# hjanime/recoup

Hardware: NVIDIA B200
Metric: reads/s through coverage + profileMatrix (reads -> per-base coverage -> regions x bins) (higher is better)
Workload: dtype int32 coverage / f64 matrix

## Files before the change

include/recoup_b200.h:

```cpp
#ifndef RECOUP_B200_H
#define RECOUP_B200_H

#include <stdint.h>

#ifdef __cplusplus
extern "C" {
#endif

#define RCP_ABI_VERSION 1

enum {
    RCP_OK = 0,
    RCP_ERR_CUDA = 1,
    RCP_ERR_ARG = 2,
    RCP_ERR_HANDLE = 3,
    RCP_ERR_NOGPU = 4,
    RCP_ERR_UNSUPPORTED = 5,
    RCP_ERR_DATA = 6
};

#define RCP_MEM_HOST 0
#define RCP_MEM_DEVICE 1

#define RCP_STRAND_ANY 2
// ... 35 lines not shown
#define RCP_PATH_BUCKETS 2
#define RCP_PATH_BLOCKS 3
#define RCP_PATH_SPLIT 4
int rcp_set_coverage_path(int path);
int rcp_coverage_path_info(int cov, int* path, int64_t* candidates);

int rcp_set_deferred_validation(int on);

int rcp_r_sample(int n, int k, int seed, int sample_kind, int* out );
int rcp_r_rank_table(int n, int seed, int sample_kind, int* rank_out );

int rcp_reads_load(int64_t n, const int32_t* chrom, const int32_t* start, const int32_t* end,
                   const int8_t* strand, int n_chrom, const int64_t* chrom_len, int frag_len,
                   int mem, int* reads_out);
int rcp_reads_load_rle(int64_t n, int64_t n_runs, const int32_t* run_chrom, const int32_t* run_len,
                       const int32_t* start, const int32_t* end, const int8_t* strand, int n_chrom,
                       const int64_t* chrom_len, int frag_len, int mem, int* reads_out);
int rcp_reads_load_width(int64_t n, const int32_t* chrom, int64_t n_runs, const int32_t* run_chrom,
                         const int32_t* run_len, const int32_t* start, int width, const int8_t* strand,
                         int n_chrom, const int64_t* chrom_len, int frag_len, int mem, int* reads_out);
int rcp_reads_width_quantile(int64_t n, const int32_t* start, const int32_t* end, double prob, int mem,
                             double* quantile_out , int64_t* n_le_out );
int rcp_r_sample_sorted(int seed, int sample_kind, int n_calls, const int64_t* n, const int64_t* k,
                        int32_t* out );
int rcp_reads_load_select(int64_t n, const int32_t* chrom, const int32_t* start, const int32_t* end,
                          const int8_t* strand, double max_width, int64_t k, const int32_t* idx,
                          int n_chrom, const int64_t* chrom_len, int frag_len, int mem,
                          int64_t* n_kept_out, int* reads_out);
int rcp_bgzf_size(const uint8_t* data , int64_t n_bytes, int64_t* inflated_bytes, int64_t* n_blocks);
int rcp_bgzf_inflate(const uint8_t* data , int64_t n_bytes, uint8_t* out , int64_t capacity,
                     int n_threads);
int rcp_bam_index(const uint8_t* rec , int64_t n_bytes, int64_t* n_records_out,
                  int64_t* offsets_out , int64_t capacity);
int rcp_bam_decode(const uint8_t* rec, int64_t n_bytes, const int64_t* offsets, int64_t n_records,
                   int n_ref, const int64_t* ref_len , int splice_split, int mem,
                   int* decoded_out, int64_t* n_out);
int rcp_bam_decode_param(const uint8_t* rec, int64_t n_bytes, const int64_t* offsets, int64_t n_records,
                         int n_ref, const int64_t* ref_len , int splice_split, int mem,
                         const int32_t* flag , int mapq_min , int simple_cigar,
                         int n_which, const int32_t* which_ref, const int32_t* which_start,
                         const int32_t* which_end, int n_tags, const char* tag_names, const int32_t* tag_ptr,
                         const int32_t* tag_type , const int64_t* int_values,
                         const char* const* str_values, int* decoded_out, int64_t* n_out);
int rcp_bed_decode(const char* text, int64_t n_bytes, int n_names, const char* const* names ,
                   int mem, int* decoded_out, int64_t* n_out);
int rcp_decoded_fetch(int decoded, int32_t* chrom, int32_t* start, int32_t* end, int8_t* strand,
                      int64_t capacity);
int rcp_decoded_free(int decoded);
int rcp_reads_load_decoded(int decoded, int n_chrom, const int64_t* chrom_len, int frag_len,
                           int* reads_out);
int rcp_decoded_width_quantile(int decoded, double prob, double* quantile_out, int64_t* n_le_out);
int rcp_reads_load_decoded_select(int decoded, double max_width, int64_t k, const int32_t* idx ,
                                  int n_chrom, const int64_t* chrom_len, int frag_len,
                                  int64_t* n_kept_out, int* reads_out);
int rcp_reads_info(int reads, int64_t* n, int* n_chrom, int64_t* device_bytes);
int rcp_reads_free(int reads);

int rcp_coverage(int reads, int64_t n_regions, const int32_t* chrom, const int32_t* start,
                 const int32_t* end, const int8_t* strand, int ignore_strand, int strand_filter,
                 int mem, int* cov_out);
int rcp_coverage_list(int reads, int64_t n_elements, const int64_t* ptr, const int32_t* chrom,
                      const int32_t* start, const int32_t* end, const int8_t* strand,
                      int ignore_strand, int strand_filter, int mem, int* cov_out);
int rcp_coverage_concat3(int left, int center, int right, int* cov_out);
int rcp_coverage_set_scale(int cov, double factor);
int rcp_coverage_info(int cov, int64_t* n_regions, int64_t* total_len, int64_t* n_null,
                      double* scale);
int rcp_coverage_lengths(int cov, int32_t* len_out );
int rcp_coverage_fetch(int cov, int64_t first, int64_t count, int32_t* out, int64_t capacity);
int rcp_coverage_rle(int cov, int64_t first, int64_t count, int64_t* run_ptr_out,
                     int32_t* values_out, int32_t* lengths_out, int64_t capacity);
int rcp_coverage_free(int cov);

#define RCP_VALUE_INT32 0
#define RCP_VALUE_FLOAT32 1
int rcp_bigwig_load(const uint8_t* data , int64_t n_bytes, int n_threads, int* signal_out);
int rcp_signal_info(int signal, int* n_chrom, int64_t* n_items, int64_t* names_bytes);
int rcp_signal_chroms(int signal, char* names , int64_t* chrom_len);
int rcp_signal_fetch(int signal, int32_t* chrom, int32_t* start, int32_t* end, float* value, int64_t capacity);
int rcp_signal_free(int signal);
int rcp_signal_coverage(int signal, int64_t n_elements, const int64_t* ptr, const int32_t* chrom,
                        const int32_t* start, const int32_t* end, const int8_t* strand, int mem, int* cov_out);
int rcp_coverage_value_type(int cov, int* type);
int rcp_coverage_fetch_f32(int cov, int64_t first, int64_t count, float* out, int64_t capacity);
int rcp_coverage_rle_f32(int cov, int64_t first, int64_t count, int64_t* run_ptr_out,
                         float* values_out, int32_t* lengths_out, int64_t capacity);

int rcp_bin_matrix(int cov, int where, int f1, int f2, int n_bins, int stat, int interp,
                   int seed, int sample_kind, double* out, int64_t ld, int mem);
int rcp_base_matrix(int cov, int where, int f1, int f2, int64_t n_cols, double* out, int64_t ld,
                    int mem);
int rcp_profile_ncols(int cov, int equal_lengths, int f1, int f2, int flank_bin_size,
                      int region_bin_size, int64_t* ncols_out);
int rcp_profile_matrix(int cov, int equal_lengths, int f1, int f2, int flank_bin_size,
                       int region_bin_size, int stat, int interp, int seed, int sample_kind,
                       double* out, int64_t ld, int mem);

int rcp_coverage_profile(int reads, int64_t n_regions, const int32_t* chrom,
                         const int32_t* start, const int32_t* end, const int8_t* strand,
                         int ignore_strand, int strand_filter, int n_bins, int seed,
                         int sample_kind, double scale, double* out, int64_t ld,
                         uint8_t* is_null_out, int mem);

int rcp_sort_keys_u32(uint32_t* keys, int64_t n, int key_bits, int mem);

#define RCP_ROW_SUM 0
#define RCP_ROW_MAX 1
#define RCP_ROW_MEAN 2
int rcp_matrix_col_profile(const double* m, int64_t n_rows, int64_t n_cols, int64_t ld, int stat,
                           int log2_scale, int mem, double* center ,
                           double* spread );
int rcp_matrix_row_stat(const double* m, int64_t n_rows, int64_t n_cols, int64_t ld, int what, int mem,
                        double* out );
int rcp_order(const double* v, int64_t n, int decreasing, int mem, int32_t* ix , int64_t* n_out);
int rcp_matrix_quantile(const double* m, int64_t n_rows, int64_t n_cols, int64_t ld, const double* probs,
                        int k, int mem, double* out );

int rcp_rows_scatter(const double* src, int64_t ld_src, int64_t n_rows, int64_t n_cols,
                     const int64_t* row_index, double* dst, int64_t ld_dst);

int rcp_rows_put(const double* src, int64_t ld_src, int64_t n_rows, int64_t n_cols, double* dst,
                 int64_t ld_dst, void* stream);

int rcp_reads_route_count(int64_t n, const int32_t* chrom, const int32_t* start, const int32_t* end, int world,
                          int n_chrom, const int32_t* spans, int64_t* counts_out );
int rcp_reads_route_pack(int64_t n, const int32_t* chrom, const int32_t* start, const int32_t* end,
                         const int8_t* strand, int world, int n_chrom, const int32_t* spans,
                         const int64_t* offsets , int32_t* chrom_out, int32_t* start_out,
                         int32_t* end_out, int8_t* strand_out);

#define RCP_IPC_HANDLE_BYTES 64
int rcp_shared_alloc(int64_t bytes, void** ptr_out, unsigned char* handle_out );
int rcp_shared_open(const unsigned char* handle , void** ptr_out);
int rcp_shared_close(void* ptr);
int rcp_shared_free(void* ptr);

#ifdef __cplusplus
}
#endif
#endif
```

recoup_b200/_lib.py:

```python
import ctypes as C
import os

_HERE = os.path.dirname(os.path.abspath(__file__))
LIB_PATH = os.environ.get("RCP_LIB_PATH") or os.path.join(_HERE, "librecoup_b200.so")

RCP_OK, RCP_ERR_CUDA, RCP_ERR_ARG, RCP_ERR_HANDLE, RCP_ERR_NOGPU, RCP_ERR_UNSUPPORTED, RCP_ERR_DATA = range(7)
MEM_HOST, MEM_DEVICE = 0, 1
STRAND_ANY = 2
WHERE = {"whole": 0, "center": 1, "upstream": 2, "downstream": 3}
STAT = {"mean": 0, "median": 1}
INTERP = {"auto": 0, "spline": 1, "linear": 2, "neighborhood": 3}
SAMPLE_KIND = {"Rejection": 0, "Rounding": 1}
COVERAGE_PATH = {"auto": 0, "index": 1, "buckets": 2, "blocks": 3, "split": 4}
VALUE_INT32, VALUE_FLOAT32 = 0, 1

_i32p = C.POINTER(C.c_int32)
_i64p = C.POINTER(C.c_int64)
_i8p = C.POINTER(C.c_int8)
_u8p = C.POINTER(C.c_uint8)
_f64p = C.POINTER(C.c_double)
_ip = C.POINTER(C.c_int)
_vp = C.c_void_p

SIGNATURES = {
    "rcp_last_error": (C.c_char_p, []),
    "rcp_abi_version": (C.c_int, []),
    "rcp_init": (C.c_int, [C.c_int]),
    "rcp_shutdown": (C.c_int, []),
    "rcp_device_info": (C.c_int, [_ip, _ip, _ip, _ip, _i64p]),
    "rcp_stream": (C.c_void_p, []),
    "rcp_sync": (C.c_int, []),
    "rcp_launch_count": (C.c_int64, [C.c_int]),
    "rcp_set_coverage_path": (C.c_int, [C.c_int]),
    "rcp_set_deferred_validation": (C.c_int, [C.c_int]),
    "rcp_host_alloc": (C.c_int, [C.c_int64, C.POINTER(C.c_void_p)]),
    "rcp_host_free": (C.c_int, [C.c_void_p]),
    "rcp_timing_enable": (C.c_int, [C.c_int]),
    "rcp_timing_read": (C.c_int, [C.c_int, C.c_int, _f64p, _i64p]),
    "rcp_timing_stage_name": (C.c_char_p, [C.c_int]),
    "rcp_r_sample": (C.c_int, [C.c_int, C.c_int, C.c_int, C.c_int, _ip]),
    "rcp_r_rank_table": (C.c_int, [C.c_int, C.c_int, C.c_int, _ip]),
    "rcp_reads_load": (C.c_int, [C.c_int64, _vp, _vp, _vp, _vp, C.c_int, _i64p, C.c_int, C.c_int, _ip]),
    "rcp_matrix_col_profile": (C.c_int, [_vp, C.c_int64, C.c_int64, C.c_int64, C.c_int, C.c_int, C.c_int,
                                         _vp, _vp]),
    "rcp_matrix_row_stat": (C.c_int, [_vp, C.c_int64, C.c_int64, C.c_int64, C.c_int, C.c_int, _vp]),
    "rcp_order": (C.c_int, [_vp, C.c_int64, C.c_int, C.c_int, _vp, _i64p]),
    "rcp_matrix_quantile": (C.c_int, [_vp, C.c_int64, C.c_int64, C.c_int64, _vp, C.c_int, C.c_int, _vp]),
    "rcp_reads_width_quantile": (C.c_int, [C.c_int64, _vp, _vp, C.c_double, C.c_int, _f64p, _i64p]),
    "rcp_r_sample_sorted": (C.c_int, [C.c_int, C.c_int, C.c_int, _i64p, _i64p, _vp]),
    "rcp_reads_load_select": (C.c_int, [C.c_int64, _vp, _vp, _vp, _vp, C.c_double, C.c_int64, _vp, C.c_int,
                                        _i64p, C.c_int, C.c_int, _i64p, _ip]),
    "rcp_coverage_path_info": (C.c_int, [C.c_int, _ip, _i64p]),
    "rcp_rows_put": (C.c_int, [_vp, C.c_int64, C.c_int64, C.c_int64, _vp, C.c_int64, _vp]),
    "rcp_reads_route_count": (C.c_int, [C.c_int64, _vp, _vp, _vp, C.c_int, C.c_int, _i32p, _i64p]),
    "rcp_reads_route_pack": (C.c_int, [C.c_int64, _vp, _vp, _vp, _vp, C.c_int, C.c_int, _i32p, _i64p, _vp, _vp, _vp,
                                       _vp]),
    "rcp_reads_load_width": (C.c_int, [C.c_int64, _vp, C.c_int64, _vp, _vp, _vp, C.c_int, _vp, C.c_int, _i64p,
                                       C.c_int, C.c_int, _ip]),
    "rcp_reads_load_rle": (C.c_int, [C.c_int64, C.c_int64, _vp, _vp, _vp, _vp, _vp, C.c_int, _i64p,
                                     C.c_int, C.c_int, _ip]),
    "rcp_bgzf_size": (C.c_int, [_vp, C.c_int64, _i64p, _i64p]),
    "rcp_bgzf_inflate": (C.c_int, [_vp, C.c_int64, _vp, C.c_int64, C.c_int]),
    "rcp_bam_index": (C.c_int, [_vp, C.c_int64, _i64p, _vp, C.c_int64]),
    "rcp_bam_decode": (C.c_int, [_vp, C.c_int64, _vp, C.c_int64, C.c_int, _i64p, C.c_int, C.c_int, _ip, _i64p]),
    "rcp_bam_decode_param": (C.c_int, [_vp, C.c_int64, _vp, C.c_int64, C.c_int, _i64p, C.c_int, C.c_int, _i32p,
                                       C.c_int, C.c_int, C.c_int, _i32p, _i32p, _i32p, C.c_int, C.c_char_p, _i32p,
                                       _i32p, _i64p, C.POINTER(C.c_char_p), _ip, _i64p]),
    "rcp_bed_decode": (C.c_int, [_vp, C.c_int64, C.c_int, C.POINTER(C.c_char_p), C.c_int, _ip, _i64p]),
    "rcp_decoded_fetch": (C.c_int, [C.c_int, _vp, _vp, _vp, _vp, C.c_int64]),
    "rcp_decoded_free": (C.c_int, [C.c_int]),
    "rcp_reads_load_decoded": (C.c_int, [C.c_int, C.c_int, _i64p, C.c_int, _ip]),
    "rcp_decoded_width_quantile": (C.c_int, [C.c_int, C.c_double, _f64p, _i64p]),
    "rcp_reads_load_decoded_select": (C.c_int, [C.c_int, C.c_double, C.c_int64, _vp, C.c_int, _i64p, C.c_int,
                                                _i64p, _ip]),
    "rcp_reads_info": (C.c_int, [C.c_int, _i64p, _ip, _i64p]),
    "rcp_reads_free": (C.c_int, [C.c_int]),
    "rcp_coverage": (C.c_int, [C.c_int, C.c_int64, _vp, _vp, _vp, _vp, C.c_int, C.c_int, C.c_int, _ip]),
    "rcp_coverage_list": (C.c_int, [C.c_int, C.c_int64, _i64p, _vp, _vp, _vp, _vp, C.c_int, C.c_int,
                                    C.c_int, _ip]),
    "rcp_coverage_concat3": (C.c_int, [C.c_int, C.c_int, C.c_int, _ip]),
    "rcp_coverage_set_scale": (C.c_int, [C.c_int, C.c_double]),
    "rcp_coverage_info": (C.c_int, [C.c_int, _i64p, _i64p, _i64p, _f64p]),
    "rcp_coverage_lengths": (C.c_int, [C.c_int, _i32p]),
    "rcp_coverage_fetch": (C.c_int, [C.c_int, C.c_int64, C.c_int64, _i32p, C.c_int64]),
    "rcp_coverage_rle": (C.c_int, [C.c_int, C.c_int64, C.c_int64, _i64p, _i32p, _i32p, C.c_int64]),
    "rcp_coverage_free": (C.c_int, [C.c_int]),
    "rcp_bigwig_load": (C.c_int, [_vp, C.c_int64, C.c_int, _ip]),
    "rcp_signal_info": (C.c_int, [C.c_int, _ip, _i64p, _i64p]),
    "rcp_signal_chroms": (C.c_int, [C.c_int, C.c_char_p, _i64p]),
    "rcp_signal_fetch": (C.c_int, [C.c_int, _vp, _vp, _vp, _vp, C.c_int64]),
    "rcp_signal_free": (C.c_int, [C.c_int]),
    "rcp_signal_coverage": (C.c_int, [C.c_int, C.c_int64, _i64p, _vp, _vp, _vp, _vp, C.c_int, _ip]),
    "rcp_coverage_value_type": (C.c_int, [C.c_int, _ip]),
    "rcp_coverage_fetch_f32": (C.c_int, [C.c_int, C.c_int64, C.c_int64, _vp, C.c_int64]),
    "rcp_coverage_rle_f32": (C.c_int, [C.c_int, C.c_int64, C.c_int64, _i64p, _vp, _i32p, C.c_int64]),
    "rcp_bin_matrix": (C.c_int, [C.c_int, C.c_int, C.c_int, C.c_int, C.c_int, C.c_int, C.c_int, C.c_int,
                                 C.c_int, _vp, C.c_int64, C.c_int]),
    "rcp_base_matrix": (C.c_int, [C.c_int, C.c_int, C.c_int, C.c_int, C.c_int64, _vp, C.c_int64, C.c_int]),
    "rcp_profile_ncols": (C.c_int, [C.c_int, C.c_int, C.c_int, C.c_int, C.c_int, C.c_int, _i64p]),
    "rcp_profile_matrix": (C.c_int, [C.c_int, C.c_int, C.c_int, C.c_int, C.c_int, C.c_int, C.c_int,
                                     C.c_int, C.c_int, C.c_int, _vp, C.c_int64, C.c_int]),
    "rcp_coverage_profile": (C.c_int, [C.c_int, C.c_int64, _vp, _vp, _vp, _vp, C.c_int, C.c_int, C.c_int,
                                       C.c_int, C.c_int, C.c_double, _vp, C.c_int64, _vp, C.c_int]),
    "rcp_sort_keys_u32": (C.c_int, [_vp, C.c_int64, C.c_int, C.c_int]),
    "rcp_shared_alloc": (C.c_int, [C.c_int64, C.POINTER(C.c_void_p), C.POINTER(C.c_ubyte)]),
    "rcp_shared_open": (C.c_int, [C.POINTER(C.c_ubyte), C.POINTER(C.c_void_p)]),
    "rcp_shared_close": (C.c_int, [C.c_void_p]),
    "rcp_shared_free": (C.c_int, [C.c_void_p]),
    "rcp_rows_scatter": (C.c_int, [_vp, C.c_int64, C.c_int64, C.c_int64, _vp, _vp, C.c_int64]),
}


class RecoupError(RuntimeError):
    def __init__(self, code, message):
        super().__init__("librecoup_b200 error %d: %s" % (code, message))
        self.code = code


def _load():
    if not os.path.exists(LIB_PATH):
        raise ImportError(
            "%s is missing: build it with `python -c 'import __graft_entry__ as g; g.build()'` "
            "(nvcc, sm_100a). recoup_b200 has no CPU fallback." % LIB_PATH)
    lib = C.CDLL(LIB_PATH)
    for name, (res, args) in SIGNATURES.items():
        fn = getattr(lib, name)
        fn.restype = res
        fn.argtypes = args
    return lib


lib = _load()
_initialised_device = None


def check(rc):
    if rc != RCP_OK:
        raise RecoupError(rc, lib.rcp_last_error().decode("utf-8", "replace"))


def init(device=None):
    global _initialised_device
    if device is None:
        device = int(os.environ.get("LOCAL_RANK", "0"))
    if _initialised_device == device:
        return
    check(lib.rcp_init(int(device)))
    _initialised_device = device


def shutdown():
    global _initialised_device
    lib.rcp_shutdown()
    _initialised_device = None


def set_coverage_path(path):
    ensure_init()
    check(lib.rcp_set_coverage_path(COVERAGE_PATH[path]))


def ensure_init():
    if _initialised_device is None:
        init()
```

recoup_b200/csrc/api.cu:

```cuda
#include <climits>
#include <algorithm>
#include <cstdarg>
#include <cstdio>
#include <cstdlib>
#include <cstring>
#include <map>
#include <memory>

#include "r_rng.cuh"
#include "rcp_internal.cuh"

namespace rcp {

Ctx g_ctx;
static thread_local std::string g_error;
static std::map<int, std::unique_ptr<ReadsIdx>> g_reads;
static std::map<int, std::unique_ptr<Coverage>> g_covs;
static int g_next_handle = 1;

int fail(int code, const char* fmt, ...) {
    char buf[1024];
    va_list ap;
    va_start(ap, fmt);
    vsnprintf(buf, sizeof(buf), fmt, ap);
// ... 912 lines not shown
    Coverage *a = get_coverage(left), *b = get_coverage(center), *c = get_coverage(right);
    if (!a || !b || !c) return fail(RCP_ERR_HANDLE, "unknown coverage handle");
    if (cov_out == nullptr) return fail(RCP_ERR_ARG, "cov_out is NULL");
    if (a->value_type != b->value_type || b->value_type != c->value_type)
        return fail(RCP_ERR_ARG, "concat3: the three coverages have different value types");
    Coverage* cv;
    int h;
    RCP_TRY(new_coverage(&cv, &h));
    cv->value_type = b->value_type;
    int rc = coverage_concat3(*a, *b, *c, cv);
    if (rc != RCP_OK) {
        drop_coverage(h);
        return rc;
    }
    cv->scale = b->scale;
    *cov_out = h;
    return RCP_OK;
}

int rcp_coverage_set_scale(int cov, double factor) {
    Coverage* cv = get_coverage(cov);
    if (!cv) return fail(RCP_ERR_HANDLE, "unknown coverage handle %d", cov);
    cv->scale = factor;
    return RCP_OK;
}

int rcp_coverage_info(int cov, int64_t* n_regions, int64_t* total_len, int64_t* n_null,
                      double* scale) {
    Coverage* cv = get_coverage(cov);
    if (!cv) return fail(RCP_ERR_HANDLE, "unknown coverage handle %d", cov);
    if (total_len || n_null) RCP_TRY(coverage_resolve_stats(*cv));
    if (n_regions) *n_regions = cv->n_regions;
    if (total_len) *total_len = cv->total_len;
    if (n_null) *n_null = cv->n_null;
    if (scale) *scale = cv->scale;
    return RCP_OK;
}

int rcp_coverage_path_info(int cov, int* path, int64_t* candidates) {
    Coverage* cv = get_coverage(cov);
    if (!cv) return fail(RCP_ERR_HANDLE, "unknown coverage handle %d", cov);
    if (candidates) RCP_TRY(coverage_resolve_stats(*cv));
    if (path) *path = cv->path;
    if (candidates) *candidates = cv->candidates;
    return RCP_OK;
}

int rcp_coverage_lengths(int cov, int32_t* len_out) {
    RCP_TRY(require_ready());
    Coverage* cv = get_coverage(cov);
    if (!cv) return fail(RCP_ERR_HANDLE, "unknown coverage handle %d", cov);
    if (cv->n_regions == 0) return RCP_OK;
    if (!len_out) return fail(RCP_ERR_ARG, "len_out is NULL");
    RCP_CUDA(cudaMemcpyAsync(len_out, cv->len, (size_t)cv->n_regions * 4, cudaMemcpyDeviceToHost,
                             g_ctx.stream));
    RCP_CUDA(cudaStreamSynchronize(g_ctx.stream));
    return RCP_OK;
}

int rcp_coverage_fetch(int cov, int64_t first, int64_t count, int32_t* out, int64_t capacity) {
    RCP_TRY(require_ready());
    Coverage* cv = get_coverage(cov);
    if (!cv) return fail(RCP_ERR_HANDLE, "unknown coverage handle %d", cov);
    if (cv->value_type != RCP_VALUE_INT32) return fail(RCP_ERR_ARG, "rcp_coverage_fetch: a FLOAT32 coverage (use _f32)");
    return coverage_fetch(*cv, first, count, out, capacity);
}

int rcp_coverage_fetch_f32(int cov, int64_t first, int64_t count, float* out, int64_t capacity) {
    RCP_TRY(require_ready());
    Coverage* cv = get_coverage(cov);
    if (!cv) return fail(RCP_ERR_HANDLE, "unknown coverage handle %d", cov);
    if (cv->value_type != RCP_VALUE_FLOAT32) return fail(RCP_ERR_ARG, "rcp_coverage_fetch_f32: an INT32 coverage");
    return coverage_fetch(*cv, first, count, reinterpret_cast<int32_t*>(out), capacity);
}

int rcp_coverage_value_type(int cov, int* type) {
    Coverage* cv = get_coverage(cov);
    if (!cv) return fail(RCP_ERR_HANDLE, "unknown coverage handle %d", cov);
    if (type == nullptr) return fail(RCP_ERR_ARG, "type is NULL");
    *type = cv->value_type;
    return RCP_OK;
}

int rcp_coverage_rle(int cov, int64_t first, int64_t count, int64_t* run_ptr_out,
                     int32_t* values_out, int32_t* lengths_out, int64_t capacity) {
    RCP_TRY(require_ready());
    Coverage* cv = get_coverage(cov);
    if (!cv) return fail(RCP_ERR_HANDLE, "unknown coverage handle %d", cov);
    if (cv->value_type != RCP_VALUE_INT32) return fail(RCP_ERR_ARG, "rcp_coverage_rle: a FLOAT32 coverage (use _f32)");
    return coverage_rle(*cv, first, count, run_ptr_out, values_out, lengths_out, capacity);
}

int rcp_coverage_rle_f32(int cov, int64_t first, int64_t count, int64_t* run_ptr_out, float* values_out,
                         int32_t* lengths_out, int64_t capacity) {
    RCP_TRY(require_ready());
    Coverage* cv = get_coverage(cov);
    if (!cv) return fail(RCP_ERR_HANDLE, "unknown coverage handle %d", cov);
    if (cv->value_type != RCP_VALUE_FLOAT32) return fail(RCP_ERR_ARG, "rcp_coverage_rle_f32: an INT32 coverage");
    return coverage_rle(*cv, first, count, run_ptr_out, reinterpret_cast<int32_t*>(values_out), lengths_out,
                        capacity);
}

int rcp_coverage_free(int cov) {
    if (!get_coverage(cov)) return fail(RCP_ERR_HANDLE, "unknown coverage handle %d", cov);
    drop_coverage(cov);
    return RCP_OK;
}

int rcp_bin_matrix(int cov, int where, int f1, int f2, int n_bins, int stat, int interp, int seed,
                   int sample_kind, double* out, int64_t ld, int mem) {
    RCP_TRY(require_ready());
    Coverage* cv = get_coverage(cov);
    if (!cv) return fail(RCP_ERR_HANDLE, "unknown coverage handle %d", cov);
    RCP_TRY(check_bins(n_bins, stat, interp));
    if (where < RCP_WHERE_WHOLE || where > RCP_WHERE_DOWNSTREAM) return fail(RCP_ERR_ARG, "bad where");
    if (f1 < 0 || f2 < 0) return fail(RCP_ERR_ARG, "negative flank");
    if (ld < cv->n_regions || out == nullptr) return fail(RCP_ERR_ARG, "bad output matrix");
    MatrixOut m;
    RCP_TRY(m.init(out, ld, cv->n_regions, n_bins, mem));
    RCP_TRY(bin_matrix_device(*cv, where, f1, f2, n_bins, stat, interp, seed, sample_kind, m.dev,
                              m.ld_dev));
    return m.finish(out, ld, cv->n_regions, n_bins);
}

int rcp_base_matrix(int cov, int where, int f1, int f2, int64_t n_cols, double* out, int64_t ld,
                    int mem) {
    RCP_TRY(require_ready());
    Coverage* cv = get_coverage(cov);
    if (!cv) return fail(RCP_ERR_HANDLE, "unknown coverage handle %d", cov);
    if (where < RCP_WHERE_WHOLE || where > RCP_WHERE_DOWNSTREAM || where == RCP_WHERE_CENTER)
        return fail(RCP_ERR_ARG, "baseCoverageMatrix takes where = whole / upstream / downstream");
    if (f1 < 0 || f2 < 0 || n_cols < 0) return fail(RCP_ERR_ARG, "negative size");
    if (where == RCP_WHERE_UPSTREAM && n_cols != f1) return fail(RCP_ERR_ARG, "n_cols must equal flank[1]");
    if (where == RCP_WHERE_DOWNSTREAM && n_cols != f2) return fail(RCP_ERR_ARG, "n_cols must equal flank[2]");
    if (ld < cv->n_regions || out == nullptr) return fail(RCP_ERR_ARG, "bad output matrix");
    MatrixOut m;
    RCP_TRY(m.init(out, ld, cv->n_regions, n_cols, mem));
    RCP_TRY(base_matrix_device(*cv, where, f1, f2, n_cols, m.dev, m.ld_dev));
    return m.finish(out, ld, cv->n_regions, n_cols);
}

int rcp_profile_ncols(int cov, int equal_lengths, int f1, int f2, int flank_bin_size,
                      int region_bin_size, int64_t* ncols_out) {
    RCP_TRY(require_ready());
    Coverage* cv = get_coverage(cov);
    if (!cv) return fail(RCP_ERR_HANDLE, "unknown coverage handle %d", cov);
    int64_t common = 0;
    if (equal_lengths && region_bin_size == 0) RCP_TRY(common_length(*cv, &common));
    Blocks b;
    RCP_TRY(profile_blocks(*cv, equal_lengths, f1, f2, flank_bin_size, region_bin_size, common, &b));
    *ncols_out = b.left + b.center + b.right;
    return RCP_OK;
}

int rcp_profile_matrix(int cov, int equal_lengths, int f1, int f2, int flank_bin_size,
                       int region_bin_size, int stat, int interp, int seed, int sample_kind,
                       double* out, int64_t ld, int mem) {
    RCP_TRY(require_ready());
    Coverage* cv = get_coverage(cov);
    if (!cv) return fail(RCP_ERR_HANDLE, "unknown coverage handle %d", cov);
    if (ld < cv->n_regions || out == nullptr) return fail(RCP_ERR_ARG, "bad output matrix");
    int64_t common = 0;
    if (equal_lengths && region_bin_size == 0) RCP_TRY(common_length(*cv, &common));
    Blocks b;
    RCP_TRY(profile_blocks(*cv, equal_lengths, f1, f2, flank_bin_size, region_bin_size, common, &b));
    const int64_t ncols = b.left + b.center + b.right;
// ... 260 lines not shown
```

recoup_b200/csrc/coverage.cu:

```cuda
#include "cov_common.cuh"
#include "rcp_internal.cuh"

namespace rcp {

using namespace covk;

namespace {

template <int NS>
struct Sources {
    const uint32_t* xs[NS];
    const uint32_t* ye[NS];
    uint32_t n[NS];
    uint32_t yshift[NS];
    uint8_t cls_bit[NS];
    uint8_t corr[NS];
};

struct RegionArrays {
    uint32_t* gs;
    int32_t* len;
    uint8_t* flags;
    uint8_t* is_null;
    uint32_t* ix0;
// ... 381 lines not shown
                int32_t* __restrict__ cov) {
    __shared__ __align__(16) int diff[TILE];
    __shared__ int rowpre[MAX_ROWS + 1];
    const int tid = threadIdx.x;
    const int64_t g = tile_region[blockIdx.x];
    const int j = (int)((int64_t)blockIdx.x - tile_off[g]);
    const int L = la.len[g];
    const int m = (L + TILE - 1) / TILE;
    const int tile_len = (((L + m - 1) / m) + ROW - 1) / ROW * ROW;
    const int o_lo = j * tile_len;
    const int tlen = min(tile_len, L - o_lo);
    const bool rev = (la.flags[g] & 1u) != 0;
    const int t0 = rev ? (L - o_lo - tlen) : o_lo;
    const int t1 = t0 + tlen - 1;
    const int nrows = (tlen + ROW - 1) / ROW;
    for (int i = tid; i < nrows * (ROW / 4); i += CTA)
        reinterpret_cast<int4*>(diff)[i] = make_int4(0, 0, 0, 0);
    __syncthreads();
    const int64_t a = ptr[g], b = ptr[g + 1];
    const uint32_t clo = la.clo[g], chi = la.chi[g], span_lo = la.span_lo[g];
    for (uint32_t i = clo + tid; i < chi; i += CTA) {
        const uint32_t rs = __ldg(xs + i), re1 = __ldg(p_end1 + i);
        if (re1 <= span_lo) continue;
        const int rst = p_strand ? (int)__ldg(p_strand + i) : 0;
        if (strand_filter != RCP_STRAND_ANY && rst != strand_filter) continue;
        int mult = 0;
        for (int64_t q = a; q < b; q++) {
            const uint32_t s = __ldg(la.xgs + q), e = __ldg(la.xge + q);
            if (e + 1u == s) continue;
            if (rs <= e && re1 > s &&
                strand_ok(rst, strand ? (int)__ldg(strand + q) : 0, ignore_strand, strand_filter))
                mult++;
        }
        if (mult == 0) continue;
        for (int64_t q = a; q < b; q++) {
            const uint32_t s = __ldg(la.xgs + q), e = __ldg(la.xge + q);
            if (e + 1u == s) continue;
            if (!(rs <= e && re1 > s)) continue;
            const int xo = __ldg(la.xoff + q);
            const int pa = xo + (int)(max(rs, s) - s);
            const int pb = xo + (int)(min(re1 - 1u, e) - s);
            if (pb < t0 || pa > t1) continue;
            const int ka = max(pa, t0) - t0, kb1 = pb + 1 - t0;
            if (!rev) {
                atomicAdd(diff + ka, mult);
                if (kb1 < tlen) atomicSub(diff + kb1, mult);
            } else {
                atomicAdd(diff + (tlen - 1 - ka), mult);
                if (kb1 < tlen) atomicSub(diff + (tlen - 1 - kb1), mult);
            }
        }
    }
    __syncthreads();
    block_scan_store(diff, tlen, 0, rev, rowpre, cov + off[g] + o_lo);
}

__global__ void __launch_bounds__(CTA)
concat_plan_kernel(int64_t R, const uint8_t* __restrict__ n0, const uint8_t* __restrict__ n1,
                   const uint8_t* __restrict__ n2, const int32_t* __restrict__ l0,
                   const int32_t* __restrict__ l1, const int32_t* __restrict__ l2,
                   int32_t* __restrict__ len, uint8_t* __restrict__ is_null,
                   int64_t* __restrict__ padded, unsigned long long* __restrict__ stats) {
    const int64_t r = (int64_t)blockIdx.x * CTA + threadIdx.x;
    if (r >= R) return;
    const bool null = n0[r] || n1[r] || n2[r];
    const int64_t L = null ? 0 : (int64_t)l0[r] + l1[r] + l2[r];
    len[r] = (int32_t)L;
    is_null[r] = null ? 1 : 0;
    padded[r] = (L + PAD - 1) / PAD * PAD;
    if (null) {
        atomicAdd(&stats[0], 1ull);
    } else {
        atomicAdd(&stats[1], (unsigned long long)L);
        atomicMax(&stats[2], (unsigned long long)L);
    }
}

__global__ void __launch_bounds__(CTA)
concat_copy_kernel(const int32_t* __restrict__ c0, const int64_t* __restrict__ o0,
                   const int32_t* __restrict__ l0, const int32_t* __restrict__ c1,
                   const int64_t* __restrict__ o1, const int32_t* __restrict__ l1,
                   const int32_t* __restrict__ c2, const int64_t* __restrict__ o2,
                   const int32_t* __restrict__ l2, const int32_t* __restrict__ len,
                   const int64_t* __restrict__ off, int32_t* __restrict__ cov) {
    const int64_t r = blockIdx.x;
    if (len[r] == 0) return;
    int32_t* dst = cov + off[r];
    const int a = l0[r], b = l1[r], c = l2[r];
    for (int i = threadIdx.x; i < a; i += CTA) dst[i] = c0[o0[r] + i];
    for (int i = threadIdx.x; i < b; i += CTA) dst[a + i] = c1[o1[r] + i];
    for (int i = threadIdx.x; i < c; i += CTA) dst[a + b + i] = c2[o2[r] + i];
}

__global__ void __launch_bounds__(CTA)
pack_kernel(const int32_t* __restrict__ cov, const int64_t* __restrict__ off,
            const int32_t* __restrict__ len, const int64_t* __restrict__ packed_off,
            int64_t first, int32_t* __restrict__ out) {
    const int64_t r = first + blockIdx.x;
    const int L = len[r];
    const int32_t* src = cov + off[r];
    int32_t* dst = out + packed_off[blockIdx.x];
    for (int i = threadIdx.x; i < L; i += CTA) dst[i] = src[i];
}

__global__ void __launch_bounds__(CTA)
len_to_i64_kernel(int64_t n, const int32_t* __restrict__ len, int64_t* __restrict__ out) {
    const int64_t i = (int64_t)blockIdx.x * CTA + threadIdx.x;
    if (i < n) out[i] = len[i];
}


__global__ void __launch_bounds__(CTA)
rle_count_kernel(const int32_t* __restrict__ cov, const int64_t* __restrict__ off,
                 const int32_t* __restrict__ len, int64_t first, int64_t* __restrict__ n_runs) {
    __shared__ int wsum[WARPS];
    const int64_t r = first + blockIdx.x;
    const int L = len[r];
    const int32_t* x = cov + off[r];
    int c = 0;
    for (int i = threadIdx.x; i < L; i += CTA) c += (i == 0) || (x[i] != x[i - 1]);
    for (int d = 16; d > 0; d >>= 1) c += __shfl_xor_sync(0xffffffffu, c, d);
    if ((threadIdx.x & 31) == 0) wsum[threadIdx.x >> 5] = c;
    __syncthreads();
    if (threadIdx.x == 0) {
        int t = 0;
        for (int w = 0; w < WARPS; w++) t += wsum[w];
        n_runs[blockIdx.x] = t;
    }
}

__global__ void __launch_bounds__(CTA)
rle_write_kernel(const int32_t* __restrict__ cov, const int64_t* __restrict__ off,
                 const int32_t* __restrict__ len, int64_t first,
                 const int64_t* __restrict__ run_ptr, int32_t* __restrict__ values,
                 int32_t* __restrict__ starts) {
    __shared__ int wsum[WARPS];
    __shared__ int carry_s;
    const int64_t r = first + blockIdx.x;
    const int L = len[r];
    const int32_t* x = cov + off[r];
    const int64_t base = run_ptr[blockIdx.x];
    const int lane = threadIdx.x & 31, warp = threadIdx.x >> 5;
    if (threadIdx.x == 0) carry_s = 0;
    __syncthreads();
    for (int i0 = 0; i0 < L; i0 += CTA) {
        const int i = i0 + threadIdx.x;
        int v = 0;
        bool head = false;
        if (i < L) {
            v = x[i];
            head = (i == 0) || (v != x[i - 1]);
        }
        const unsigned bal = __ballot_sync(0xffffffffu, head);
        if (lane == 0) wsum[warp] = __popc(bal);
        __syncthreads();
        int pre = carry_s;
        for (int w = 0; w < warp; w++) pre += wsum[w];
        if (head) {
            const int64_t o = base + pre + __popc(bal & ((1u << lane) - 1u));
            values[o] = v;
            starts[o] = i;
        }
        __syncthreads();
        if (threadIdx.x == CTA - 1) carry_s = pre + __popc(bal);
        __syncthreads();
    }
}

__global__ void __launch_bounds__(CTA)
rle_lengths_kernel(const int32_t* __restrict__ len, int64_t first,
                   const int64_t* __restrict__ run_ptr, const int32_t* __restrict__ starts,
                   int32_t* __restrict__ lengths) {
    const int64_t r = first + blockIdx.x;
    const int L = len[r];
    const int64_t a = run_ptr[blockIdx.x], b = run_ptr[blockIdx.x + 1];
    for (int64_t j = a + threadIdx.x; j < b; j += CTA)
        lengths[j] = (j + 1 < b ? starts[j + 1] : L) - starts[j];
}

int alloc_coverage_arrays(Coverage* cv, int64_t R) {
    cv->n_regions = R;
    RCP_TRY(dalloc(&cv->off, (size_t)R + 1));
    RCP_TRY(dalloc(&cv->len, (size_t)R));
    RCP_TRY(dalloc(&cv->is_null, (size_t)R));
    return RCP_OK;
}

template <int NS>
int coverage_ranges_impl(ReadsIdx& rd, Sources<NS> src, int64_t R, const int32_t* chrom,
                         const int32_t* start, const int32_t* end, const int8_t* strand,
                         int ignore_strand, int strand_filter, Coverage* cv) {
    RCP_TRY(alloc_coverage_arrays(cv, R));
    RegionArrays ra;
    RCP_TRY(dalloc(&ra.gs, (size_t)R));
    ra.len = cv->len;
    RCP_TRY(dalloc(&ra.flags, (size_t)R));
    ra.is_null = cv->is_null;
    RCP_TRY(dalloc(&ra.ix0, (size_t)R * NS));
    RCP_TRY(dalloc(&ra.ix1, (size_t)R * NS));
    RCP_TRY(dalloc(&ra.iy0, (size_t)R * NS));
    RCP_TRY(dalloc(&ra.iy1, (size_t)R * NS));
    RCP_TRY(dalloc(&ra.padded, (size_t)R));
    RCP_TRY(dalloc(&ra.ntiles, (size_t)R));
    int64_t* tile_off = nullptr;
    RCP_TRY(dalloc(&tile_off, (size_t)R + 1));
    unsigned int* d_err = nullptr;
    unsigned long long* d_stats = nullptr;
    RCP_TRY(dalloc(&d_err, 1));
    RCP_TRY(dalloc(&d_stats, 3));
    RCP_CUDA(cudaMemsetAsync(d_err, 0, sizeof(unsigned int), g_ctx.stream));
    RCP_CUDA(cudaMemsetAsync(d_stats, 0, 3 * sizeof(unsigned long long), g_ctx.stream));

    struct Host {
        int64_t total_padded, total_tiles;
        unsigned long long stats[3];
        unsigned int err;
    } h = {0, 0, {0, 0, 0}, 0};
    {
        StageTimer t(ST_COV_PLAN);
        if (R > 0) {
            region_plan_kernel<NS><<<blocks_for(R, CTA), CTA, 0, g_ctx.stream>>>(
                R, chrom, start, end, strand, rd.d_chrom_off, rd.d_chrom_len, rd.n_chrom, src,
                ignore_strand, strand_filter, ra, d_err, d_stats);
            RCP_LAUNCHED();
        }
        RCP_TRY(exclusive_scan2_i64(ra.padded, cv->off, cv->off + R, ra.ntiles, tile_off,
                                    tile_off + R, R));
    }
    {
        const FetchItem items[4] = {{cv->off + R, &h.total_padded, 8}, {tile_off + R, &h.total_tiles, 8},
                                    {d_stats, h.stats, 24}, {d_err, &h.err, 4}};
        RCP_TRY(fetch_and_sync(items, 4));
    }
    int rc = RCP_OK;
    if (h.err & 1u) rc = fail(RCP_ERR_DATA, "a region has a chromosome id outside [0, n_chrom)");
    else if (h.err & 2u) rc = fail(RCP_ERR_DATA, "a region has end < start - 1");
    if (rc == RCP_OK) {
        cv->path = RCP_PATH_INDEX;
        cv->total_padded = h.total_padded;
        cv->n_null = (int64_t)h.stats[0];
        cv->total_len = (int64_t)h.stats[1];
        cv->max_len = (int32_t)h.stats[2];
        rc = dalloc(&cv->cov, (size_t)h.total_padded);
    }
    int32_t* tile_region = nullptr;
    if (rc == RCP_OK && h.total_tiles > 0) {
        rc = dalloc(&tile_region, (size_t)h.total_tiles);
        if (rc == RCP_OK) {
            {
                StageTimer t(ST_COV_PLAN);
                fill_tiles_kernel<<<blocks_for(R, CTA), CTA, 0, g_ctx.stream>>>(R, ra.ntiles,
                                                                                tile_off, tile_region);
                g_ctx.launches++;
            }
            StageTimer t(ST_COV_TILE);
            cov_tile_kernel<NS><<<(unsigned)h.total_tiles, CTA, 0, g_ctx.stream>>>(
                tile_region, tile_off, ra, src, cv->off, cv->cov);
            g_ctx.launches++;
        }
    }
    if (rc == RCP_OK && R > 0) {
        StageTimer t(ST_COV_SMALL);
        cov_small_kernel<NS><<<blocks_for(R, WARPS), CTA, 0, g_ctx.stream>>>(R, ra, src, cv->off,
                                                                             cv->cov);
        g_ctx.launches++;
    }
    if (rc == RCP_OK && cudaGetLastError() != cudaSuccess)
        rc = fail(RCP_ERR_CUDA, "coverage kernel launch failed");
    dfree(tile_region);
    dfree(ra.gs);
    dfree(ra.flags);
    dfree(ra.ix0);
    dfree(ra.ix1);
    dfree(ra.iy0);
    dfree(ra.iy1);
    dfree(ra.padded);
    dfree(ra.ntiles);
    dfree(tile_off);
    dfree(d_err);
    dfree(d_stats);
    return rc;
}

}

void coverage_release(Coverage& c) {
    dfree(c.cov);
    dfree(c.off);
    dfree(c.len);
    dfree(c.is_null);
    dfree(c.d_stats);
    c.stats_pending = false;
}

namespace {
__global__ void __launch_bounds__(CTA)
na_rule_kernel(int64_t R, const int32_t* __restrict__ chrom, const int8_t* __restrict__ strand,
               const uint8_t* __restrict__ len_na, int n_chrom, const int64_t* __restrict__ off,
               int32_t* __restrict__ len, uint8_t* __restrict__ is_null, const int32_t* __restrict__ cov,
               const int64_t* __restrict__ end_pos) {
    const int64_t r = (int64_t)blockIdx.x * CTA + threadIdx.x;
    if (r >= R) return;
    const int32_t L = len[r];
    const int c = chrom[r];
    if (L <= 0 || c < 0 || c >= n_chrom || !len_na[c]) return;
    const int64_t idx = end_pos ? end_pos[r] : ((strand && strand[r] < 0) ? 0 : (int64_t)L - 1);
    if (idx < 0 || idx >= L || cov[off[r] + idx] == 0) {
        len[r] = 0;
        is_null[r] = 1;
    }
}

__global__ void __launch_bounds__(CTA)
len_stats_kernel(int64_t R, const int32_t* __restrict__ len, unsigned long long* __restrict__ stats) {
    const int64_t r = (int64_t)blockIdx.x * CTA + threadIdx.x;
    unsigned long long my_null = 0, my_len = 0;
    if (r < R) {
        my_len = (unsigned long long)len[r];
        my_null = my_len == 0 ? 1 : 0;
    }
    unsigned long long my_max = my_len;
    for (int d = 16; d > 0; d >>= 1) {
        my_null += __shfl_xor_sync(0xffffffffu, my_null, d);
        my_len += __shfl_xor_sync(0xffffffffu, my_len, d);
        my_max = max(my_max, __shfl_xor_sync(0xffffffffu, my_max, d));
    }
    if ((threadIdx.x & 31) == 0) {
        if (my_null) atomicAdd(&stats[0], my_null);
        if (my_len) atomicAdd(&stats[1], my_len);
        if (my_max) atomicMax(&stats[2], my_max);
    }
}
}

int coverage_na_rule(const ReadsIdx& rd, Coverage& cv, int64_t R, const int32_t* d_chrom, const int8_t* d_strand,
                     const int64_t* d_end_pos) {
    if (!rd.any_na || R <= 0) return RCP_OK;
    RCP_TRY(coverage_resolve_stats(cv));
    if (!cv.d_stats) RCP_TRY(dalloc(&cv.d_stats, 4));
    const unsigned long long h[4] = {0ull, 0ull, 0ull, (unsigned long long)cv.candidates};
    RCP_CUDA(cudaMemcpyAsync(cv.d_stats, h, 32, cudaMemcpyHostToDevice, g_ctx.stream));
    na_rule_kernel<<<blocks_for(R, CTA), CTA, 0, g_ctx.stream>>>(R, d_chrom, d_strand, rd.d_len_na, rd.n_chrom, cv.off,
                                                               cv.len, cv.is_null, cv.cov, d_end_pos);
    RCP_LAUNCHED();
    len_stats_kernel<<<blocks_for(R, CTA), CTA, 0, g_ctx.stream>>>(R, cv.len, cv.d_stats);
    RCP_LAUNCHED();
    cv.stats_pending = true;
    return coverage_resolve_stats(cv);
}

int coverage_resolve_stats(Coverage& c) {
    if (!c.stats_pending) return RCP_OK;
    unsigned long long h[4] = {0, 0, 0, 0};
    const FetchItem items[1] = {{c.d_stats, h, 32}};
    RCP_TRY(fetch_and_sync(items, 1));
    c.n_null = (int64_t)h[0];
    c.total_len = (int64_t)h[1];
    c.max_len = (int32_t)h[2];
    c.candidates = (int64_t)h[3];
    c.stats_pending = false;
    return RCP_OK;
}

int coverage_ranges(ReadsIdx& rd, int64_t R, const int32_t* chrom, const int32_t* start,
                    const int32_t* end, const int8_t* strand, int ignore_strand,
                    int strand_filter, int mem, Coverage* cv) {
    DevIn<int32_t> d_chrom, d_start, d_end;
    DevIn<int8_t> d_strand;
    RCP_TRY(d_chrom.init(chrom, (size_t)R, mem));
    RCP_TRY(d_start.init(start, (size_t)R, mem));
    RCP_TRY(d_end.init(end, (size_t)R, mem));
    RCP_TRY(d_strand.init(strand, (size_t)R, mem));
    const bool unstranded = (strand_filter == RCP_STRAND_ANY) && (ignore_strand || strand == nullptr);
    const bool uni = rd.uniform_w != 0;
    auto fill = [&](auto& src, int slot, int cls, int bit) {
        const SortedClass& sc = rd.cls[cls];
        src.xs[slot] = sc.xs;
        src.ye[slot] = uni ? sc.xs : sc.ye;
        src.yshift[slot] = rd.uniform_w;
        src.n[slot] = (uint32_t)sc.n;
        src.cls_bit[slot] = (uint8_t)bit;
        src.corr[slot] = 0;
    };
    auto fill_corr = [&](auto& src, int slot, int cls, int bit) {
        const SortedClass& sc = rd.cls[cls];
        src.xs[slot] = sc.cxs;
        src.ye[slot] = sc.cye;
        src.yshift[slot] = 0;
        src.n[slot] = (uint32_t)sc.cn;
        src.cls_bit[slot] = (uint8_t)bit;
        src.corr[slot] = 1;
    };
    if (unstranded) {
        RCP_TRY(reads_build_class(rd, CLS_ALL));
        if (!uni) {
            Sources<1> src;
            fill(src, 0, CLS_ALL, 0);
            return coverage_ranges_impl<1>(rd, src, R, d_chrom.ptr, d_start.ptr, d_end.ptr,
                                           d_strand.ptr, ignore_strand, strand_filter, cv);
        }
        Sources<2> src;
        fill(src, 0, CLS_ALL, 0);
        fill_corr(src, 1, CLS_ALL, 0);
        return coverage_ranges_impl<2>(rd, src, R, d_chrom.ptr, d_start.ptr, d_end.ptr,
                                       d_strand.ptr, ignore_strand, strand_filter, cv);
    }
    for (int k = 0; k < 3; k++) RCP_TRY(reads_build_class(rd, CLS_PLUS + k));
    if (!uni) {
        Sources<3> src;
        for (int k = 0; k < 3; k++) fill(src, k, CLS_PLUS + k, k);
        return coverage_ranges_impl<3>(rd, src, R, d_chrom.ptr, d_start.ptr, d_end.ptr,
                                       d_strand.ptr, ignore_strand, strand_filter, cv);
    }
    Sources<6> src;
    for (int k = 0; k < 3; k++) {
        fill(src, k, CLS_PLUS + k, k);
        fill_corr(src, 3 + k, CLS_PLUS + k, k);
    }
    return coverage_ranges_impl<6>(rd, src, R, d_chrom.ptr, d_start.ptr, d_end.ptr, d_strand.ptr,
                                   ignore_strand, strand_filter, cv);
}

int coverage_list(ReadsIdx& rd, int64_t G, const int64_t* ptr, const int64_t n_ranges,
                  const int32_t* chrom, const int32_t* start, const int32_t* end,
                  const int8_t* strand, int ignore_strand, int strand_filter, int mem,
                  Coverage* cv) {
// ... 41 lines not shown
        RCP_LAUNCHED();
    }
    RCP_TRY(exclusive_scan2_i64(la.padded, cv->off, cv->off + G, la.ntiles, tile_off,
                                tile_off + G, G));
    {
        const FetchItem items[4] = {{cv->off + G, &h.total_padded, 8}, {tile_off + G, &h.total_tiles, 8},
                                    {d_stats, h.stats, 24}, {d_err, &h.err, 4}};
        RCP_TRY(fetch_and_sync(items, 4));
    }
    int rc = RCP_OK;
    if (h.err & 1u) rc = fail(RCP_ERR_DATA, "a range has a chromosome id outside [0, n_chrom)");
    else if (h.err & 2u) rc = fail(RCP_ERR_DATA, "a range has end < start - 1");
    else if (h.err & 4u)
        rc = fail(RCP_ERR_DATA, "the ranges of one list element lie on different chromosomes");
    if (rc == RCP_OK) {
        cv->total_padded = h.total_padded;
        cv->n_null = (int64_t)h.stats[0];
        cv->total_len = (int64_t)h.stats[1];
        cv->max_len = (int32_t)h.stats[2];
        rc = dalloc(&cv->cov, (size_t)h.total_padded);
    }
    int32_t* tile_region = nullptr;
    if (rc == RCP_OK && h.total_tiles > 0) {
        rc = dalloc(&tile_region, (size_t)h.total_tiles);
        if (rc == RCP_OK) {
            fill_tiles_kernel<<<blocks_for(G, CTA), CTA, 0, g_ctx.stream>>>(G, la.ntiles, tile_off,
                                                                            tile_region);
            g_ctx.launches++;
            cov_list_kernel<<<(unsigned)h.total_tiles, CTA, 0, g_ctx.stream>>>(
                tile_region, tile_off, d_ptr.ptr, d_strand.ptr, la, rd.cls[CLS_ALL].xs, rd.p_end1,
                rd.p_strand, ignore_strand, strand_filter, cv->off, cv->cov);
            g_ctx.launches++;
            if (cudaGetLastError() != cudaSuccess)
                rc = fail(RCP_ERR_CUDA, "list coverage kernel launch failed");
        }
    }
    dfree(tile_region);
    dfree(la.xgs);
    dfree(la.xge);
    dfree(la.xoff);
    dfree(la.flags);
    dfree(la.clo);
    dfree(la.chi);
    dfree(la.span_lo);
    dfree(la.padded);
    dfree(la.ntiles);
    dfree(tile_off);
    dfree(d_err);
    dfree(d_stats);
    return rc;
}

int coverage_concat3(const Coverage& a, const Coverage& b, const Coverage& c, Coverage* cv) {
    const int64_t R = a.n_regions;
    if (b.n_regions != R || c.n_regions != R)
        return fail(RCP_ERR_ARG, "concat3: the three coverages have different lengths");
    RCP_TRY(alloc_coverage_arrays(cv, R));
    int64_t* padded = nullptr;
    unsigned long long* d_stats = nullptr;
    RCP_TRY(dalloc(&padded, (size_t)R));
    RCP_TRY(dalloc(&d_stats, 3));
    RCP_CUDA(cudaMemsetAsync(d_stats, 0, 24, g_ctx.stream));
    if (R > 0) {
        concat_plan_kernel<<<blocks_for(R, CTA), CTA, 0, g_ctx.stream>>>(
            R, a.is_null, b.is_null, c.is_null, a.len, b.len, c.len, cv->len, cv->is_null, padded,
            d_stats);
        RCP_LAUNCHED();
    }
    RCP_TRY(exclusive_scan_i64(padded, cv->off, R, cv->off + R));
    int64_t total = 0;
    unsigned long long stats[3] = {0, 0, 0};
    StageTimer concat_timer(ST_COV_CONCAT);
    RCP_CUDA(cudaMemcpyAsync(&total, cv->off + R, 8, cudaMemcpyDeviceToHost, g_ctx.stream));
    RCP_CUDA(cudaMemcpyAsync(stats, d_stats, 24, cudaMemcpyDeviceToHost, g_ctx.stream));
    RCP_CUDA(cudaStreamSynchronize(g_ctx.stream));
    cv->total_padded = total;
    cv->n_null = (int64_t)stats[0];
    cv->total_len = (int64_t)stats[1];
    cv->max_len = (int32_t)stats[2];
    RCP_TRY(dalloc(&cv->cov, (size_t)total));
    if (R > 0) {
        concat_copy_kernel<<<(unsigned)R, CTA, 0, g_ctx.stream>>>(a.cov, a.off, a.len, b.cov, b.off,
                                                                 b.len, c.cov, c.off, c.len,
                                                                 cv->len, cv->off, cv->cov);
        RCP_LAUNCHED();
    }
    dfree(padded);
    dfree(d_stats);
    return RCP_OK;
}

int coverage_fetch(const Coverage& cv, int64_t first, int64_t count, int32_t* out,
                   int64_t capacity) {
    if (first < 0 || count < 0 || first + count > cv.n_regions)
        return fail(RCP_ERR_ARG, "fetch: region range [%lld, %lld) outside [0, %lld)",
                    (long long)first, (long long)(first + count), (long long)cv.n_regions);
    if (count == 0) return RCP_OK;
    int64_t *len64 = nullptr, *poff = nullptr;
    RCP_TRY(dalloc(&len64, (size_t)count));
    RCP_TRY(dalloc(&poff, (size_t)count + 1));
    len_to_i64_kernel<<<blocks_for(count, CTA), CTA, 0, g_ctx.stream>>>(count, cv.len + first, len64);
    RCP_LAUNCHED();
    RCP_TRY(exclusive_scan_i64(len64, poff, count, poff + count));
    int64_t total = 0;
    RCP_CUDA(cudaMemcpyAsync(&total, poff + count, 8, cudaMemcpyDeviceToHost, g_ctx.stream));
    RCP_CUDA(cudaStreamSynchronize(g_ctx.stream));
    int rc = RCP_OK;
    if (total > capacity) {
        rc = fail(RCP_ERR_ARG, "fetch: %lld ints needed, capacity %lld", (long long)total,
                  (long long)capacity);
    } else if (total > 0) {
        int32_t* packed = nullptr;
        rc = dalloc(&packed, (size_t)total);
        if (rc == RCP_OK) {
            pack_kernel<<<(unsigned)count, CTA, 0, g_ctx.stream>>>(cv.cov, cv.off, cv.len, poff,
                                                                  first, packed);
            g_ctx.launches++;
            cudaError_t e = cudaMemcpyAsync(out, packed, (size_t)total * 4, cudaMemcpyDeviceToHost,
                                            g_ctx.stream);
            if (e == cudaSuccess) e = cudaStreamSynchronize(g_ctx.stream);
            if (e != cudaSuccess) rc = fail(RCP_ERR_CUDA, "fetch copy failed: %s", cudaGetErrorString(e));
            dfree(packed);
        }
    }
    dfree(len64);
    dfree(poff);
    return rc;
}

int coverage_rle(const Coverage& cv, int64_t first, int64_t count, int64_t* run_ptr,
                 int32_t* values, int32_t* lengths, int64_t capacity) {
    if (first < 0 || count < 0 || first + count > cv.n_regions)
        return fail(RCP_ERR_ARG, "rle: region range [%lld, %lld) outside [0, %lld)", (long long)first,
                    (long long)(first + count), (long long)cv.n_regions);
    if (run_ptr == nullptr) return fail(RCP_ERR_ARG, "rle: run_ptr is NULL");
    run_ptr[0] = 0;
    if (count == 0) return RCP_OK;
    int64_t *n_runs = nullptr, *d_ptr = nullptr;
    RCP_TRY(dalloc(&n_runs, (size_t)count));
    RCP_TRY(dalloc(&d_ptr, (size_t)count + 1));
    rle_count_kernel<<<(unsigned)count, CTA, 0, g_ctx.stream>>>(cv.cov, cv.off, cv.len, first, n_runs);
    RCP_LAUNCHED();
    RCP_TRY(exclusive_scan_i64(n_runs, d_ptr, count, d_ptr + count));
    RCP_CUDA(cudaMemcpyAsync(run_ptr, d_ptr, ((size_t)count + 1) * 8, cudaMemcpyDeviceToHost,
                             g_ctx.stream));
    RCP_CUDA(cudaStreamSynchronize(g_ctx.stream));
    const int64_t total = run_ptr[count];
    int rc = RCP_OK;
    if (values != nullptr || lengths != nullptr) {
        if (values == nullptr || lengths == nullptr)
            rc = fail(RCP_ERR_ARG, "rle: values and lengths must be given together");
        else if (total > capacity)
            rc = fail(RCP_ERR_ARG, "rle: %lld runs, capacity %lld", (long long)total, (long long)capacity);
        else if (total > 0) {
            int32_t *d_val = nullptr, *d_start = nullptr, *d_len = nullptr;
            rc = dalloc(&d_val, (size_t)total);
            if (rc == RCP_OK) rc = dalloc(&d_start, (size_t)total);
            if (rc == RCP_OK) rc = dalloc(&d_len, (size_t)total);
            if (rc == RCP_OK) {
                rle_write_kernel<<<(unsigned)count, CTA, 0, g_ctx.stream>>>(cv.cov, cv.off, cv.len, first,
                                                                           d_ptr, d_val, d_start);
                g_ctx.launches++;
                rle_lengths_kernel<<<(unsigned)count, CTA, 0, g_ctx.stream>>>(cv.len, first, d_ptr,
                                                                             d_start, d_len);
                g_ctx.launches++;
                cudaError_t e = cudaMemcpyAsync(values, d_val, (size_t)total * 4, cudaMemcpyDeviceToHost,
                                                g_ctx.stream);
                if (e == cudaSuccess)
                    e = cudaMemcpyAsync(lengths, d_len, (size_t)total * 4, cudaMemcpyDeviceToHost,
                                        g_ctx.stream);
                if (e == cudaSuccess) e = cudaStreamSynchronize(g_ctx.stream);
                if (e != cudaSuccess) rc = fail(RCP_ERR_CUDA, "rle copy failed: %s", cudaGetErrorString(e));
            }
            dfree(d_val);
            dfree(d_start);
            dfree(d_len);
        }
    }
    dfree(n_runs);
    dfree(d_ptr);
    return rc;
}

}
```

recoup_b200/csrc/coverage_split.cu:

```cuda
#include <algorithm>
#include <cstdlib>
#include <chrono>
#include <cstdio>

#include <type_traits>
#include <vector>

#include <cooperative_groups.h>

#include "cov_common.cuh"
#include "r_rng.cuh"
#include "rcp_internal.cuh"

namespace rcp {

using namespace covk;

namespace {

constexpr int BLK_SHIFT = 14;
#ifndef RCP_SUB_SHIFT
#define RCP_SUB_SHIFT 10
#endif
constexpr int SUB_SHIFT = RCP_SUB_SHIFT;
constexpr int NG = 1024;
constexpr int RING = 32;
constexpr int CH = 16;
#ifndef RCP_SPLIT_ST
#define RCP_SPLIT_ST 1024
#endif
constexpr int ST = RCP_SPLIT_ST;
constexpr int ROUND_VEC = 2048;
constexpr int VPT = ROUND_VEC / ST;
constexpr int SLAB = 64;
constexpr int MIN_P = 16, MAX_P = 22;
constexpr int GT = 1024;
constexpr int CS = 1024;
constexpr int WT = 7 * ROW;
constexpr int WT_ONE = SMALL_MAX;
static_assert(NG % ST == 0 && ROUND_VEC % ST == 0, "the flush phase maps thread t to the groups t, t + ST, ...");
static_assert(RING == 2 * CH, "a ring holds two chunks");
static_assert(SLAB >= 64, "one flush phase of a warp needs up to 64 chunks");

__device__ __forceinline__ void sp_mark_block(uint32_t* __restrict__ tab, uint32_t b) {
    atomicOr(tab + (b >> 4), 1u << (b & 15u));
    if (b > 0) atomicOr(tab + ((b - 1u) >> 4), 0x10000u << ((b - 1u) & 15u));
}

__global__ void __launch_bounds__(CTA)
sp_plan_kernel(int64_t R, const int32_t* __restrict__ chrom, const int32_t* __restrict__ start,
               const int32_t* __restrict__ end, const int8_t* __restrict__ strand,
               const uint32_t* __restrict__ chrom_off, const int64_t* __restrict__ chrom_len,
               int n_chrom, int ignore_strand, int strand_filter, uint32_t* __restrict__ gs_out,
               int32_t* __restrict__ plen, uint8_t* __restrict__ flags, int64_t* __restrict__ ntile,
               int64_t* __restrict__ padded, uint32_t* __restrict__ tab, unsigned int* __restrict__ err,
               unsigned long long* __restrict__ pstats ,
               unsigned long long* __restrict__ zero4 ) {
    const int64_t r = (int64_t)blockIdx.x * CTA + threadIdx.x;
    if (r < 4) zero4[r] = 0ull;
    unsigned long long my_len = 0;
    if (r < R) {
        const int st = strand ? (int)strand[r] : 0;
        uint32_t gs;
        int64_t L;
        const bool null = window_geometry(chrom[r], start[r], end[r], n_chrom, chrom_off, chrom_len,
                                          err, &gs, &L);
        const int32_t len = null ? 0 : (int32_t)L;
        gs_out[r] = gs;
        plen[r] = len;
        flags[r] = (uint8_t)((st < 0 ? 1u : 0u) | (class_mask(st, ignore_strand, strand_filter) << 1));
        ntile[r] = len > WT_ONE ? ((int64_t)len + WT - 1) / WT : (len > 0 ? 1 : 0);
        padded[r] = ((int64_t)len + PAD - 1) / PAD * PAD;
        my_len = (unsigned long long)len;
        if (len > 0) {
            const uint32_t b1 = (gs + (uint32_t)len - 1u) >> BLK_SHIFT;
            for (uint32_t b = gs >> BLK_SHIFT; b <= b1; b++) sp_mark_block(tab, b);
        }
    }
    unsigned long long my_max = my_len, my_inv = my_len ? 0x100000000ull - my_len : 0ull;
    for (int d = 16; d > 0; d >>= 1) {
        my_len += __shfl_xor_sync(0xffffffffu, my_len, d);
        my_max = max(my_max, __shfl_xor_sync(0xffffffffu, my_max, d));
        my_inv = max(my_inv, __shfl_xor_sync(0xffffffffu, my_inv, d));
    }
    if ((threadIdx.x & 31) == 0 && my_len) {
        atomicAdd(&pstats[0], my_len);
        atomicMax(&pstats[1], my_max);
        atomicMax(&pstats[2], my_inv);
    }
}

__device__ __forceinline__ int64_t sp_owner_of(const int64_t* __restrict__ off, int64_t R, int64_t t) {
    int64_t lo = 0, hi = R;
    while (hi - lo > 1) {
        const int64_t mid = lo + ((hi - lo) >> 1);
        if (__ldg(off + mid) <= t) lo = mid;
        else hi = mid;
    }
    return lo;
}

struct __align__(16) SpDesc {
    int64_t out;
    uint32_t c0;
    uint32_t n;
    int32_t tlen;
    uint32_t cts;
    uint32_t flags;
    uint32_t region;
};

__global__ void __launch_bounds__(CTA)
sp_tiles_kernel(int64_t R, int64_t T, const int64_t* __restrict__ off_tile, const uint32_t* __restrict__ gs,
                const int32_t* __restrict__ plen, const uint8_t* __restrict__ flags,
                const int64_t* __restrict__ cov_off ,
                const int32_t* __restrict__ edge, int n_bins,
                uint32_t max_w, uint32_t pmask, const uint32_t* __restrict__ boff, SpDesc* __restrict__ desc,
                uint32_t* __restrict__ tabs,
                const uint32_t* __restrict__ lxs, const uint32_t* __restrict__ lmax, uint32_t ln,
                uint2* __restrict__ lrange) {
    const int64_t t = (int64_t)blockIdx.x * CTA + threadIdx.x;
    if (t >= T) return;
    const int64_t r = sp_owner_of(off_tile, R, t);
    const int L = plen[r];
    uint32_t o_lo = 0, tlen = (uint32_t)L;
    if (L > WT_ONE) {
        o_lo = (uint32_t)(t - off_tile[r]) * WT;
        tlen = (uint32_t)min(WT, L - (int)o_lo);
    }
    const uint32_t q0 = (flags[r] & 1u) ? (uint32_t)L - o_lo - tlen : o_lo;
    const uint32_t tstart = gs[r] + q0;
    const uint32_t first = tstart >= max_w ? tstart - max_w + 1u : 0u;
    SpDesc d;
    d.out = cov_off ? cov_off[r] + o_lo : (int64_t)o_lo;
    if (!cov_off) {
        int a = 0, b = n_bins;
        while (b - a > 1) {
            const int mid = (a + b) >> 1;
            if (__ldg(edge + mid) <= (int)o_lo) a = mid;
            else b = mid;
        }
        d.out |= (int64_t)a << 32;
    }
    d.c0 = __ldg(boff + (first >> SUB_SHIFT));
    d.n = __ldg(boff + ((tstart + tlen - 1u) >> SUB_SHIFT) + 1u) - d.c0;
    d.tlen = (int32_t)tlen;
    d.cts = tstart & pmask;
    d.flags = flags[r];
    d.region = (uint32_t)r;
    desc[t] = d;
    if (ln) {
        tabs[t] = tstart;
        const uint32_t hi = tstart + tlen - 1u;
        uint32_t a = 0, b = ln;
        while (a < b) {
            const uint32_t mid = a + ((b - a) >> 1);
            if (__ldg(lxs + mid) < hi + 1u) a = mid + 1;
            else b = mid;
        }
        const uint32_t c1 = a;
        a = 0;
        b = c1;
        while (a < b) {
            const uint32_t mid = a + ((b - a) >> 1);
            if (__ldg(lmax + mid) < tstart + 1u) a = mid + 1;
            else b = mid;
        }
        lrange[t] = make_uint2(a, c1);
    }
}

__device__ __forceinline__ uint2 lds64(uint32_t a) {
    uint2 v;
    asm volatile("ld.shared.v2.u32 {%0, %1}, [%2];" : "=r"(v.x), "=r"(v.y) : "r"(a));
    return v;
}
__device__ __forceinline__ uint32_t lds32(uint32_t a) {
    uint32_t v;
    asm volatile("ld.shared.u32 %0, [%1];" : "=r"(v) : "r"(a));
    return v;
}
__device__ __forceinline__ uint4 lds128(uint32_t a) {
    uint4 v;
    asm volatile("ld.shared.v4.u32 {%0, %1, %2, %3}, [%4];" : "=r"(v.x), "=r"(v.y), "=r"(v.z), "=r"(v.w) : "r"(a));
    return v;
}
__device__ __forceinline__ void sts32(uint32_t a, uint32_t v) {
    asm volatile("st.shared.u32 [%0], %1;" ::"r"(a), "r"(v) : "memory");
}
__device__ __forceinline__ void sts64(uint32_t a, uint32_t x, uint32_t y) {
    asm volatile("st.shared.v2.u32 [%0], {%1, %2};" ::"r"(a), "r"(x), "r"(y) : "memory");
}
__device__ __forceinline__ int lds_s8(uint32_t a) {
    int v;
    asm volatile("ld.shared.s8 %0, [%1];" : "=r"(v) : "r"(a));
    return v;
}
__device__ __forceinline__ void sts8(uint32_t a, int v) {
    asm volatile("st.shared.u8 [%0], %1;" ::"r"(a), "r"(v) : "memory");
}
__device__ __forceinline__ uint32_t atoms_add(uint32_t a, uint32_t v) {
    uint32_t old;
    asm volatile("atom.shared.add.u32 %0, [%1], %2;" : "=r"(old) : "r"(a), "r"(v) : "memory");
    return old;
}

struct SplitOut {
    uint32_t* pool;
    uint16_t* meta;
    uint32_t* pool_next;
};

constexpr size_t sp_split_smem(int words) {
    return (size_t)NG * RING * 4 + (size_t)NG * 4 + (size_t)words * 4;
}
constexpr size_t SP_SMEM_MAX = 232448;

template <bool STRANDED>
__global__ void __launch_bounds__(ST, 1)
sp_split_kernel(int64_t n, const uint32_t* __restrict__ g_start, const uint32_t* __restrict__ g_end1,
                const int8_t* __restrict__ strand, const uint32_t* __restrict__ tab_g, int words, int P,
                uint32_t max_pack_w, SplitOut out) {
    extern __shared__ __align__(16) unsigned char sp_smem[];
    const int tid = threadIdx.x;
    const unsigned lane = tid & 31, lt = (1u << lane) - 1u;
    const uint32_t ring_a = (uint32_t)__cvta_generic_to_shared(sp_smem);
    const uint32_t cnt_a = ring_a + NG * RING * 4;
    const uint32_t tab_a = cnt_a + NG * 4;
    for (int i = tid; i < words; i += ST) sts32(tab_a + i * 4, tab_g[i]);
    for (int i = tid; i < NG; i += ST) sts32(cnt_a + i * 4, 0u);
    __syncthreads();
    const uint32_t pmask = (1u << P) - 1u;
    const int wsh = STRANDED ? P + 2 : P;
    uint32_t slab_next = 0, slab_end = 0;
    uint32_t spare = 0;
    bool have_spare = false;
    bool hot = false;

    uint32_t a_rem = 0, a_old = 0, a_new = 0;
    auto alloc = [&](uint32_t total) {
        a_rem = slab_end - slab_next;
        a_old = slab_next;
        a_new = 0;
        if (total > a_rem) {
            if (!have_spare && lane == 0) spare = atomicAdd(out.pool_next, (uint32_t)SLAB);
            a_new = __shfl_sync(0xffffffffu, spare, 0);
            have_spare = false;
            slab_next = a_new + (total - a_rem);
            slab_end = a_new + SLAB;
        } else {
            slab_next += total;
// ... 361 lines not shown
            keys[k] = s[i];
            idx[k] = (uint32_t)i;
        }
    }
}

__global__ void __launch_bounds__(CTA)
sp_long_gather_kernel(uint32_t n, const uint32_t* __restrict__ idx, const uint32_t* __restrict__ e1,
                      const int8_t* __restrict__ st, uint32_t* __restrict__ o_e1, int8_t* __restrict__ o_st) {
    const uint32_t i = blockIdx.x * CTA + threadIdx.x;
    if (i >= n) return;
    o_e1[i] = e1[idx[i]];
    if (st) o_st[i] = st[idx[i]];
}

__device__ __forceinline__ uint32_t sp_lower_bound(const uint32_t* __restrict__ a, uint32_t lo, uint32_t hi, uint32_t v) {
    while (lo < hi) {
        const uint32_t mid = lo + ((hi - lo) >> 1);
        if (__ldg(a + mid) < v) lo = mid + 1;
        else hi = mid;
    }
    return lo;
}
__device__ __forceinline__ uint2 sp_long_range(const LongIdx& lg, uint32_t lo, uint32_t hi) {
    const uint32_t c1 = sp_lower_bound(lg.xs, 0, lg.n, hi + 1u);
    const uint32_t c0 = sp_lower_bound(lg.maxe1, 0, c1, lo + 1u);
    return make_uint2(c0, c1);
}

__device__ __forceinline__ SpDesc sp_load_desc(const SpDesc* __restrict__ p) {
    const int4 a = __ldg(reinterpret_cast<const int4*>(p));
    const int4 b = __ldg(reinterpret_cast<const int4*>(p) + 1);
    SpDesc d;
    d.out = (int64_t)(((uint64_t)(uint32_t)a.y << 32) | (uint32_t)a.x);
    d.c0 = (uint32_t)a.z;
    d.n = (uint32_t)a.w;
    d.tlen = b.x;
    d.cts = (uint32_t)b.y;
    d.flags = (uint32_t)b.z;
    d.region = (uint32_t)b.w;
    return d;
}

template <bool STRANDED>
__device__ __forceinline__ bool sp_apply(uint32_t e, const SpDesc& d, int P, int* diff) {
    const int sh = 32 - P;
    const int rel = ((int)((e - d.cts) << sh)) >> sh;
    uint32_t w = e >> (STRANDED ? P + 2 : P);
    if (STRANDED && !((d.flags >> (1u + ((e >> P) & 3u))) & 1u)) w = 0;
    int lo = max(rel, 0), hi = min(rel + (int)w, d.tlen);
    if (lo >= hi) return false;
    if (d.flags & 1u) {
        const int l2 = d.tlen - hi;
        hi = d.tlen - lo;
        lo = l2;
    }
    atomicAdd(diff + lo, 1);
    if (hi < d.tlen) atomicSub(diff + hi, 1);
    return true;
}

template <bool STRANDED, bool REV>
__device__ __forceinline__ bool sp_apply_fast(uint32_t e, uint32_t cts, int tlen, uint32_t cls, int P,
                                              uint32_t diff_a) {
    const int sh = 32 - P;
    const int rel = ((int)((e - cts) << sh)) >> sh;
    int w = (int)(e >> (STRANDED ? P + 2 : P));
    if (STRANDED) w = ((cls >> ((e >> P) & 3u)) & 1u) ? w : 0;
    const int lo = max(rel, 0), hi = min(rel + w, tlen);
    const int a = REV ? tlen - hi : lo;
    const int b = REV ? tlen - lo : hi;
    asm volatile(
        "{\n\t"
        ".reg .pred p, q;\n\t"
        "setp.lt.s32 p, %0, %1;\n\t"
        "setp.lt.and.s32 q, %2, %3, p;\n\t"
        "@p red.shared.add.s32 [%4], 1;\n\t"
        "@q red.shared.add.s32 [%5], -1;\n\t"
        "}" ::"r"(lo), "r"(hi), "r"(b), "r"(tlen), "r"(diff_a + (uint32_t)a * 4u), "r"(diff_a + (uint32_t)b * 4u)
        : "memory");
    return lo < hi;
}

template <int RPW, bool STORE = true>
__device__ __forceinline__ void warp_scan_store_fwd(int* diff, int tlen, int32_t* __restrict__ dst) {
    const int lane = threadIdx.x & 31;
    int* mine = diff + lane * 4 * RPW;
    int4 v[RPW];
    int sum = 0;
#pragma unroll
    for (int k = 0; k < RPW; k++) {
        v[k] = *(reinterpret_cast<const int4*>(mine) + k);
        sum += (v[k].x + v[k].y) + (v[k].z + v[k].w);
    }
    const int inc = warp_inclusive_scan(sum);
    int run = inc - sum;
#pragma unroll
    for (int k = 0; k < RPW; k++) {
        int4 o;
        o.x = (run += v[k].x);
        o.y = (run += v[k].y);
        o.z = (run += v[k].z);
        o.w = (run += v[k].w);
        *(reinterpret_cast<int4*>(mine) + k) = o;
    }
    __syncwarp();
    if (STORE && lane == 0) {
        fence_proxy_async_smem();
        tma_store_1d(dst, diff, (uint32_t)((tlen + 3) & ~3) * 4u);
        tma_store_commit();
    }
}

struct FusedBins {
    const int32_t* edge;
    int n;
    int64_t R;
    unsigned long long* acc;
};

template <int RPW>
__device__ __forceinline__ bool warp_scan_prefix2(int* diff) {
    const int lane = threadIdx.x & 31;
    int* mine = diff + lane * 4 * RPW;
    int4 v[RPW];
    int sum = 0;
#pragma unroll
    for (int k = 0; k < RPW; k++) {
        v[k] = *(reinterpret_cast<const int4*>(mine) + k);
        sum += (v[k].x + v[k].y) + (v[k].z + v[k].w);
    }
    const int inc = warp_inclusive_scan(sum);
    const int run0 = inc - sum;
    int run = run0, cmax = 0;
    uint32_t tot = 0;
#pragma unroll
    for (int k = 0; k < RPW; k++) {
        run += v[k].x; tot += (uint32_t)run; cmax = max(cmax, run);
        run += v[k].y; tot += (uint32_t)run; cmax = max(cmax, run);
        run += v[k].z; tot += (uint32_t)run; cmax = max(cmax, run);
        run += v[k].w; tot += (uint32_t)run; cmax = max(cmax, run);
    }
    const bool small = __reduce_max_sync(0xffffffffu, cmax) < (1 << 22);
    uint32_t acc = 0;
    if (small) {
        uint32_t incs = tot;
#pragma unroll
        for (int d = 1; d < 32; d <<= 1) {
            const uint32_t o = __shfl_up_sync(0xffffffffu, incs, d);
            if (lane >= d) incs += o;
        }
        acc = incs - tot;
    }
    run = run0;
#pragma unroll
    for (int k = 0; k < RPW; k++) {
        int4 o;
        run += v[k].x; acc += (uint32_t)run; o.x = small ? (int)acc : run;
        run += v[k].y; acc += (uint32_t)run; o.y = small ? (int)acc : run;
        run += v[k].z; acc += (uint32_t)run; o.z = small ? (int)acc : run;
        run += v[k].w; acc += (uint32_t)run; o.w = small ? (int)acc : run;
        *(reinterpret_cast<int4*>(mine) + k) = o;
    }
    __syncwarp();
    return small;
}

__device__ __forceinline__ void tile_to_bins(const int* tile, const SpDesc& d, const FusedBins& fb, bool prefixed) {
    const int lane = threadIdx.x & 31;
    const int o_lo = (int)(uint32_t)d.out, o_hi = o_lo + d.tlen;
    const int a = (int)(d.out >> 32);
    for (int i = a + lane; i < fb.n; i += 32) {
        const int e0 = __ldg(fb.edge + i);
        if (e0 >= o_hi) break;
        const int lo = max(e0, o_lo) - o_lo, hi = min(__ldg(fb.edge + i + 1), o_hi) - o_lo;
        unsigned long long s = 0;
        if (prefixed) {
            if (hi > lo) s = (uint32_t)tile[hi - 1] - (lo > 0 ? (uint32_t)tile[lo - 1] : 0u);
        } else {
            for (int k = lo; k < hi; k++) s += (unsigned long long)(unsigned int)tile[k];
        }
        if (s) atomicAdd(fb.acc + (size_t)i * fb.R + d.region, s);
    }
}

__global__ void __launch_bounds__(CTA)
sp_bins_finish_kernel(FusedBins fb, const int32_t* __restrict__ plen, const uint8_t* __restrict__ region_hit,
                      double scale, double* __restrict__ out, int64_t ld, uint8_t* __restrict__ is_null) {
    const int64_t r = (int64_t)blockIdx.x * CTA + threadIdx.x;
    if (r >= fb.R) return;
    const int i = blockIdx.y;
    const bool null = plen[r] == 0 || region_hit[r] == 0;
    double v = 0.0;
    if (!null) {
        const int w = __ldg(fb.edge + i + 1) - __ldg(fb.edge + i);
        v = scale * ((double)(long long)fb.acc[(size_t)i * fb.R + r] / (double)w);
    }
    out[(size_t)i * ld + r] = v;
    if (i == 0 && is_null) is_null[r] = null ? 1 : 0;
}

__device__ __forceinline__ void cp_async16(uint32_t smem_dst, const void* gmem_src) {
    asm volatile("cp.async.cg.shared.global [%0], [%1], 16;" ::"r"(smem_dst), "l"(gmem_src) : "memory");
}
__device__ __forceinline__ void cp_async_commit() { asm volatile("cp.async.commit_group;" ::: "memory"); }
template <int N>
__device__ __forceinline__ void cp_async_wait() { asm volatile("cp.async.wait_group %0;" ::"n"(N) : "memory"); }

#ifndef RCP_WTILE_OCC
#define RCP_WTILE_OCC 4
#endif
constexpr int CBUF = 256;
constexpr size_t WTILE_SMEM = (size_t)WARPS * (WT_ONE * 4 + 2 * CBUF * 4 + 4 * sizeof(SpDesc));
template <bool STRANDED, bool FUSED>
__global__ void __launch_bounds__(CTA, RCP_WTILE_OCC)
sp_wtile_kernel(int64_t T, const SpDesc* __restrict__ desc, const uint32_t* __restrict__ cand, int P,
                int32_t* __restrict__ cov, uint8_t* __restrict__ region_hit, FusedBins fb, LongIdx lg,
                const uint32_t* __restrict__ tabs, const uint2* __restrict__ lrange) {
    extern __shared__ __align__(16) unsigned char wt_smem[];
    const int warp = threadIdx.x >> 5;
    const uint32_t lane = threadIdx.x & 31;
    int* diff = reinterpret_cast<int*>(wt_smem) + warp * WT_ONE;
    const uint32_t* cs = reinterpret_cast<const uint32_t*>(wt_smem + (size_t)WARPS * WT_ONE * 4) + warp * 2 * CBUF;
    const SpDesc* ring = reinterpret_cast<const SpDesc*>(wt_smem + (size_t)WARPS * (WT_ONE * 4 + 2 * CBUF * 4)) + warp * 4;
    const uint32_t cs_a = (uint32_t)__cvta_generic_to_shared(cs);
    const uint32_t ring_a = (uint32_t)__cvta_generic_to_shared(ring);
    const int64_t step = (int64_t)gridDim.x * WARPS;
    int64_t t = (int64_t)blockIdx.x * WARPS + warp;
    if (t >= T) return;
    auto stage_desc = [&](int64_t tile, int j) {
        if (lane < 2 && tile < T)
            cp_async16(ring_a + (uint32_t)(j & 3) * (uint32_t)sizeof(SpDesc) + lane * 16u,
                       reinterpret_cast<const int4*>(desc + tile) + lane);
    };
    auto stage_cands = [&](uint32_t c0, uint32_t n, int buf) {
        const uint32_t a0 = c0 & ~3u;
        const uint32_t units = min(((c0 - a0) + n + 3u) >> 2, (uint32_t)(CBUF / 4));
#pragma unroll
        for (int k = 0; k < CBUF / 128; k++) {
            const uint32_t u = (uint32_t)k * 32u + lane;
            if (u < units) cp_async16(cs_a + (uint32_t)buf * (CBUF * 4) + u * 16u, cand + a0 + u * 4u);
        }
    };
    stage_desc(t, 0);
    stage_desc(t + step, 1);
    cp_async_commit();
    cp_async_wait<0>();
    __syncwarp();
    stage_cands(ring[0].c0, ring[0].n, 0);
    cp_async_commit();
    int buf = 0;
    constexpr int B = 4;
    for (int j = 0;; j++) {
        cp_async_wait<0>();
        __syncwarp();
        const SpDesc d = ring[j & 3];
        const bool more = t + step < T;
        if (more) {
            const SpDesc* nx = ring + ((j + 1) & 3);
            stage_cands(nx->c0, nx->n, buf ^ 1);
        }
        stage_desc(t + 2 * step, j + 2);
        cp_async_commit();
        const int rows = (d.tlen + ROW - 1) / ROW;
        for (int k = 0; k < rows; k++) reinterpret_cast<int4*>(diff)[k * 32 + lane] = make_int4(0, 0, 0, 0);
        __syncwarp();
        bool hit = false;
        const uint32_t a0 = d.c0 & ~3u;
        const uint32_t words = (d.c0 - a0) + d.n;
        const uint32_t staged = min((words + 3u) & ~3u, (uint32_t)CBUF);
        const uint32_t mine_a = cs_a + (uint32_t)buf * (CBUF * 4) + lane * 4u;
        const uint32_t diff_a = (uint32_t)__cvta_generic_to_shared(diff);
        const uint32_t cls = d.flags >> 1;
        auto apply_all = [&](auto rev_tag) {
            constexpr bool REV = decltype(rev_tag)::value;
#pragma unroll 4
            for (uint32_t i = lane; i < staged; i += 32)
                hit |= sp_apply_fast<STRANDED, REV>(lds32(mine_a + (i - lane) * 4u), d.cts, d.tlen, cls, P, diff_a);
#if defined(RCP_EXP_MODE) && RCP_EXP_MODE == 2
            if (d.tlen >= 0) return;
#endif
            for (uint32_t i0 = CBUF; i0 < words; i0 += B * 32) {
                uint32_t e[B];
#pragma unroll
                for (int k = 0; k < B; k++) {
                    const uint32_t i = i0 + (uint32_t)k * 32u + lane;
                    e[k] = i < words ? __ldg(cand + a0 + i) : 0u;
                }
#pragma unroll
                for (int k = 0; k < B; k++) hit |= sp_apply_fast<STRANDED, REV>(e[k], d.cts, d.tlen, cls, P, diff_a);
            }
        };
#if defined(RCP_EXP_MODE) && RCP_EXP_MODE == 1
        if (d.tlen < 0) apply_all(std::true_type{});
#else
        if (d.flags & 1u) apply_all(std::true_type{});
        else apply_all(std::false_type{});
#endif
        if (lg.n) {
            const uint2 lr = lrange[t];
            const uint32_t ts = tabs[t];
            for (uint32_t i = lr.x + lane; i < lr.y; i += 32) {
                const uint32_t rs = __ldg(lg.xs + i), re1 = __ldg(lg.e1 + i);
                const int st = lg.st ? (int)__ldg(lg.st + i) : 0;
                const uint32_t cls = st > 0 ? 0u : (st < 0 ? 1u : 2u);
                if (!((d.flags >> (1u + cls)) & 1u)) continue;
                if (rs >= ts + (uint32_t)d.tlen || re1 <= ts) continue;
                int lo = (int)(max(rs, ts) - ts), hi = (int)(min(re1, ts + (uint32_t)d.tlen) - ts);
                if (d.flags & 1u) {
                    const int l2 = d.tlen - hi;
                    hi = d.tlen - lo;
                    lo = l2;
                }
                atomicAdd(diff + lo, 1);
                if (hi < d.tlen) atomicSub(diff + hi, 1);
                hit = true;
            }
        }
        hit = __any_sync(0xffffffffu, hit);
        __syncwarp();
        if (FUSED) {
            if (hit) {
                bool prefixed = false;
                switch (rows) {
                    case 1: prefixed = warp_scan_prefix2<1>(diff); break;
                    case 2: prefixed = warp_scan_prefix2<2>(diff); break;
                    case 3: prefixed = warp_scan_prefix2<3>(diff); break;
                    case 4: prefixed = warp_scan_prefix2<4>(diff); break;
                    case 5: prefixed = warp_scan_prefix2<5>(diff); break;
                    case 6: prefixed = warp_scan_prefix2<6>(diff); break;
                    case 7: prefixed = warp_scan_prefix2<7>(diff); break;
                    default: prefixed = warp_scan_prefix2<8>(diff); break;
                }
                tile_to_bins(diff, d, fb, prefixed);
            }
        } else {
            int32_t* dst = cov + d.out;
            switch (rows) {
                case 1: warp_scan_store_fwd<1>(diff, d.tlen, dst); break;
                case 2: warp_scan_store_fwd<2>(diff, d.tlen, dst); break;
                case 3: warp_scan_store_fwd<3>(diff, d.tlen, dst); break;
                case 4: warp_scan_store_fwd<4>(diff, d.tlen, dst); break;
                case 5: warp_scan_store_fwd<5>(diff, d.tlen, dst); break;
                case 6: warp_scan_store_fwd<6>(diff, d.tlen, dst); break;
                case 7: warp_scan_store_fwd<7>(diff, d.tlen, dst); break;
                default: {
                    int pre = 0;
                    for (int row = 0; row < rows; row++)
                        pre += warp_row_scan_store(diff + row * ROW, pre, 0, false, d.tlen - row * ROW, dst + row * ROW);
                }
            }
        }
        if (hit && lane == 0) region_hit[d.region] = 1;
        t += step;
        if (!FUSED && lane == 0) tma_store_wait_read();
        if (!more) break;
        __syncwarp();
        buf ^= 1;
    }
}

struct ListPlan {
    const int64_t* ptr;
    const int8_t* rstrand;
    uint32_t* xgs;
    uint32_t* xge;
    int32_t* xoff;
    uint2* lrange;
};

__global__ void __launch_bounds__(CTA)
sp_list_plan_kernel(int64_t G, ListPlan lp, const int32_t* __restrict__ chrom, const int32_t* __restrict__ start,
                    const int32_t* __restrict__ end, const uint32_t* __restrict__ chrom_off,
                    const int64_t* __restrict__ chrom_len, int n_chrom, int32_t* __restrict__ plen,
                    uint8_t* __restrict__ flags, int64_t* __restrict__ ntile, int64_t* __restrict__ padded,
                    unsigned int* __restrict__ err, unsigned long long* __restrict__ pstats, LongIdx lg) {
    const int64_t g = (int64_t)blockIdx.x * CTA + threadIdx.x;
    unsigned long long my_len = 0;
    if (g < G) {
        const int64_t a = lp.ptr[g], b = lp.ptr[g + 1];
        bool null = (b <= a);
        bool simple = true;
        int64_t L = 0;
        int st0 = 0;
        uint32_t lo = 0xffffffffu, hi = 0;
        if (!null) {
            const int c = chrom[a];
            st0 = lp.rstrand ? (int)lp.rstrand[a] : 0;
            if (c < 0 || c >= n_chrom) {
                atomicOr(err, 1u);
                null = true;
            } else {
                const int64_t clen = chrom_len[c];
                const uint32_t coff = chrom_off[c];
                int64_t prev_end = -1;
                for (int64_t i = a; i < b; i++) {
                    int64_t s = start[i], e = end[i];
                    if (s <= prev_end || e < s || (lp.rstrand && lp.rstrand[i] != lp.rstrand[a])) simple = false;
                    prev_end = e;
                    if (chrom[i] != c) atomicOr(err, 4u);
                    if (e < s - 1) { atomicOr(err, 2u); null = true; }
                    if (s < 0 || e > clen) null = true;
                    if (s == 0) s = 1;
                    int64_t w = e - s + 1;
                    if (w < 0) w = 0;
                    const uint32_t gs = coff + (uint32_t)(s > 0 ? s : 0);
                    lp.xgs[i] = gs;
                    lp.xge[i] = gs + (uint32_t)w - 1u;
                    lp.xoff[i] = (int32_t)L;
                    L += w;
                    if (w > 0) {
                        lo = min(lo, gs);
                        hi = max(hi, gs + (uint32_t)w - 1u);
                    }
                }
                if (L == 0 || L > 0x7fffffff) null = true;
            }
// ... 370 lines not shown
        RCP_TRY(sort_pairs_u32(rd.ln_xs, idx, (int64_t)n, rd.key_bits));
        dbg.lap("  long: sort");
        if (n > 0) {
            sp_long_gather_kernel<<<blocks_for((int64_t)n, CTA), CTA, 0, g_ctx.stream>>>((uint32_t)n, idx, rd.g_end1,
                                                                                        rd.d_strand, rd.ln_e1, rd.ln_st);
            RCP_LAUNCHED();
        }
        RCP_TRY(running_max_u32_device(rd.ln_e1, rd.ln_maxe1, (int64_t)n));
        rd.ln_n = (int64_t)n;
        dfree(idx);
        dbg.lap("binned: long-read list");
    }
    Arena K, B, Tb;
    RCP_TRY(Tb.reserve(Arena::pad((size_t)g.words * 4)));
    uint32_t* tab = Tb.take<uint32_t>((size_t)g.words);
    RCP_CUDA(cudaMemsetAsync(tab, 0xff, (size_t)g.words * 4, g_ctx.stream));
    SortedCands sc;
    RCP_TRY(split_and_sort(rd, tab, g.words, g.P, g.n_groups, stranded, stranded, max_pack_w, K, B, &sc));
    rd.bn_base = K.base;
    K.base = nullptr;
    rd.bn_cand = sc.cand;
    rd.bn_boff = sc.boff;
    rd.bn_cb = sc.cb;
    rd.bn_P = g.P;
    rd.bn_stranded = stranded;
    dbg.lap("binned: split + sort");
    return RCP_OK;
}

struct FusedReq {
    int n_bins, seed, sample_kind;
    double scale;
    double* d_out;
    int64_t ld;
    uint8_t* d_is_null;
};

static int split_impl(ReadsIdx& rd, int64_t R, const int32_t* chrom, const int32_t* start,
                      const int32_t* end, const int8_t* strand, int ignore_strand,
                      int strand_filter, int mem, Coverage* cv, const FusedReq* fz) {
    const bool stranded = !((strand_filter == RCP_STRAND_ANY) && (ignore_strand || strand == nullptr));
    const bool st_arr = stranded && rd.d_strand != nullptr;
    const int64_t span = (int64_t)rd.chrom_off[(size_t)rd.n_chrom];
    const int words = (int)((span >> (BLK_SHIFT + 4)) + 2);
    int P = MIN_P;
    while (P < MAX_P && ((span + (1ll << P) - 1) >> P) > NG) P++;
    const int n_groups = (int)std::max<int64_t>(1, (span + (1ll << P) - 1) >> P);
    const int wbits = 32 - P - (stranded ? 2 : 0);
    if (n_groups > NG || rd.n >= 0x7ffffff0ll || sp_split_smem(words) > SP_SMEM_MAX)
        return RCP_SPLIT_NOT_APPLICABLE;
    const bool have_index = rd.bn_cand && rd.bn_P == P && (rd.bn_stranded || !stranded);
    if (!have_index && !rd.pending && (rd.max_width > 8191u || rd.max_width >= (1u << wbits)))
        return RCP_SPLIT_NOT_APPLICABLE;
    const uint32_t pmask = (1u << P) - 1u;

    DevIn<int32_t> d_chrom, d_start, d_end;
    DevIn<int8_t> d_strand;
    RCP_TRY(d_chrom.init(chrom, (size_t)R, mem));
    RCP_TRY(d_start.init(start, (size_t)R, mem));
    RCP_TRY(d_end.init(end, (size_t)R, mem));
    RCP_TRY(d_strand.init(strand, (size_t)R, mem));

    Arena A;
    const size_t r = (size_t)R;
    RCP_TRY(A.reserve(Arena::pad(64) + Arena::pad((size_t)words * 4) + Arena::pad(r * 4) * 2 + Arena::pad(r) * 2 +
                      Arena::pad(r * 8) * 2 + Arena::pad((r + 1) * 8)));
    unsigned int* err = A.take<unsigned int>(16);
    unsigned long long* pstats = reinterpret_cast<unsigned long long*>(err + 4);
    uint32_t* tab = A.take<uint32_t>((size_t)words);
    uint8_t* region_hit = A.take<uint8_t>(r);
    const size_t zero_bytes = A.used;
    uint32_t* gs = A.take<uint32_t>(r);
    int32_t* plen = A.take<int32_t>(r);
    uint8_t* flags = A.take<uint8_t>(r);
    int64_t* ntile = A.take<int64_t>(r);
    int64_t* padded = A.take<int64_t>(r);
    int64_t* off_tile = A.take<int64_t>(r + 1);
    if (A.used > A.cap) return fail(RCP_ERR_CUDA, "internal: split plan arena overrun");

    cv->n_regions = R;
    RCP_TRY(dalloc(&cv->off, r + 1));
    RCP_TRY(dalloc(&cv->len, r));
    RCP_TRY(dalloc(&cv->is_null, r));
    RCP_TRY(dalloc(&cv->d_stats, 4));
    auto give_up = [&]() {
        dfree(cv->off);
        dfree(cv->len);
        dfree(cv->is_null);
        dfree(cv->d_stats);
        return RCP_SPLIT_NOT_APPLICABLE;
    };
    {
        StageTimer t(ST_SP_PLAN);
        RCP_CUDA(cudaMemsetAsync(A.base, 0, zero_bytes, g_ctx.stream));
        if (R == 0) RCP_CUDA(cudaMemsetAsync(cv->d_stats, 0, 32, g_ctx.stream));
        if (R > 0) {
            sp_plan_kernel<<<blocks_for(R, CTA), CTA, 0, g_ctx.stream>>>(
                R, d_chrom.ptr, d_start.ptr, d_end.ptr, d_strand.ptr, rd.d_chrom_off, rd.d_chrom_len,
                rd.n_chrom, ignore_strand, strand_filter, gs, plen, flags, ntile, padded, tab, err,
                pstats, cv->d_stats);
            RCP_LAUNCHED();
        }
        RCP_TRY(exclusive_scan2_i64(ntile, off_tile, off_tile + R, padded, cv->off, cv->off + R, R));
    }
    struct Host {
        int64_t T, total_padded;
        unsigned long long pstats[3];
        unsigned int err;
    } h = {0, 0, {0, 0, 0}, 0};
    Arena K, B;
    SortedCands sc;
    {
        FetchItem items[8] = {{off_tile + R, &h.T, 8}, {cv->off + R, &h.total_padded, 8}, {pstats, h.pstats, 24},
                              {err, &h.err, 4}};
        int n_items = 4;
        reads_pending_items(rd, items, &n_items);
        RCP_TRY(fetch_begin(items, n_items));
        if (!have_index) RCP_TRY(split_and_sort(rd, tab, words, P, n_groups, stranded, st_arr, 0xffffffffu, K, B, &sc));
        RCP_TRY(fetch_end(items, n_items));
        RCP_TRY(reads_finish(rd));
    }
    if (h.err & 1u) return fail(RCP_ERR_DATA, "a region has a chromosome id outside [0, n_chrom)");
    if (h.err & 2u) return fail(RCP_ERR_DATA, "a region has end < start - 1");
    const int64_t T = h.T;
    if (T > 0x7fffffff) return fail(RCP_ERR_UNSUPPORTED, "more than 2^31-1 coverage tiles");
    const uint32_t max_w = have_index ? std::max(1u, std::min(rd.max_width, rd.bn_max_pack_w))
                                      : (rd.max_width > 0 ? rd.max_width : 1u);
    if (!have_index && (max_w > 8191u || max_w >= (1u << wbits))) return give_up();

    FusedBins fb = {nullptr, 0, R, nullptr};
    Arena F;
    if (fz) {
        const int64_t max_len = (int64_t)h.pstats[1];
        const int64_t min_len = h.pstats[2] ? 0x100000000ll - (int64_t)h.pstats[2] : 0;
        const int n = fz->n_bins;
        if (max_len != min_len || (max_len > 0 && max_len < n)) return give_up();
        const int64_t Lc = max_len > 0 ? max_len : n;
        std::vector<int32_t> edge((size_t)n + 1);
        {
            std::vector<int> perm((size_t)n), scratch((size_t)n), rank((size_t)n);
            RRng* rng = new RRng;
            rng->seed((uint32_t)fz->seed, fz->sample_kind);
            rng->sample(n, n, scratch.data(), perm.data());
            delete rng;
            for (int pos = 0; pos < n; pos++) rank[(size_t)perm[(size_t)pos] - 1] = pos + 1;
            const int64_t b = Lc / n, d = Lc - b * n;
            int64_t at = 0;
            for (int i = 0; i < n; i++) {
                edge[(size_t)i] = (int32_t)at;
                at += b + (rank[(size_t)i] <= d ? 1 : 0);
            }
            edge[(size_t)n] = (int32_t)at;
        }
        RCP_TRY(F.reserve(Arena::pad(((size_t)n + 1) * 4) + Arena::pad((size_t)n * r * 8)));
        int32_t* d_edge = F.take<int32_t>((size_t)n + 1);
        fb.acc = F.take<unsigned long long>((size_t)n * r);
        RCP_CUDA(cudaMemcpyAsync(d_edge, edge.data(), ((size_t)n + 1) * 4, cudaMemcpyHostToDevice, g_ctx.stream));
        RCP_CUDA(cudaMemsetAsync(fb.acc, 0, (size_t)n * r * 8, g_ctx.stream));
        fb.edge = d_edge;
        fb.n = n;
    } else {
        cv->path = RCP_PATH_SPLIT;
        cv->total_padded = h.total_padded;
        cv->total_len = (int64_t)h.pstats[0];
        cv->max_len = (int32_t)h.pstats[1];
        cv->n_null = 0;
        cv->stats_pending = true;
        RCP_TRY(dalloc(&cv->cov, (size_t)h.total_padded));
    }

    bool words_stranded = stranded;
    if (have_index) {
        sc.cand = rd.bn_cand;
        sc.boff = rd.bn_boff;
        sc.cb = rd.bn_cb;
        words_stranded = rd.bn_stranded;
    }
    uint32_t* cand = sc.cand;
    uint32_t* boff = sc.boff;
    uint32_t* cb = sc.cb;
    LongIdx lg = long_index(rd);
    if (!have_index) lg.n = 0;
    Arena D;
    RCP_TRY(D.reserve(Arena::pad((size_t)(T + 1) * sizeof(SpDesc)) + (lg.n ? Arena::pad((size_t)(T + 1) * 4) +
                                                                            Arena::pad((size_t)(T + 1) * 8) : 0)));
    SpDesc* desc = D.take<SpDesc>((size_t)T + 1);
    uint32_t* tabs = lg.n ? D.take<uint32_t>((size_t)T + 1) : nullptr;
    uint2* lrange = lg.n ? D.take<uint2>((size_t)T + 1) : nullptr;
    if (T > 0) {
        StageTimer t(ST_SP_PLAN);
        sp_tiles_kernel<<<blocks_for(T, CTA), CTA, 0, g_ctx.stream>>>(R, T, off_tile, gs, plen, flags,
                                                                     fz ? nullptr : cv->off, fb.edge, fb.n, max_w, pmask, boff,
                                                                     desc, tabs,
                                                                     lg.xs, lg.maxe1, lg.n, lrange);
        RCP_LAUNCHED();
    }
    if (T > 0) {
        {
            StageTimer t(fz ? ST_FUSED : ST_SP_TILE);
            const int64_t want = blocks_for(T, WARPS);
            auto launch = [&](auto kern) -> int {
                int per_sm = 0;
                RCP_CUDA(cudaFuncSetAttribute(kern, cudaFuncAttributeMaxDynamicSharedMemorySize, (int)WTILE_SMEM));
                RCP_CUDA(cudaOccupancyMaxActiveBlocksPerMultiprocessor(&per_sm, kern, CTA, WTILE_SMEM));
                per_sm = std::max(per_sm, 1);
                kern<<<(unsigned)std::min<int64_t>(want, (int64_t)g_ctx.sm_count * per_sm), CTA, WTILE_SMEM,
                       g_ctx.stream>>>(
                    T, desc, cand, P, cv->cov, region_hit, fb, lg, tabs, lrange);
                RCP_LAUNCHED();
                return RCP_OK;
            };
            if (fz) RCP_TRY(words_stranded ? launch(sp_wtile_kernel<true, true>) : launch(sp_wtile_kernel<false, true>));
            else RCP_TRY(words_stranded ? launch(sp_wtile_kernel<true, false>) : launch(sp_wtile_kernel<false, false>));
        }
    }
    if (fz) {
        if (R > 0) {
            StageTimer t(ST_FUSED);
            sp_bins_finish_kernel<<<dim3(blocks_for(R, CTA), (unsigned)fb.n), CTA, 0, g_ctx.stream>>>(
                fb, plen, region_hit, fz->scale, fz->d_out, fz->ld, fz->d_is_null);
            RCP_LAUNCHED();
        }
        return RCP_OK;
    }
    if (R > 0) {
        StageTimer t(ST_SP_PLAN);
        sp_null_kernel<<<blocks_for(R, CTA), CTA, 0, g_ctx.stream>>>(R, plen, region_hit, cb, cv->len, cv->is_null,
                                                                    cv->d_stats);
        RCP_LAUNCHED();
    }
    return RCP_OK;
}

int coverage_ranges_split(ReadsIdx& rd, int64_t R, const int32_t* chrom, const int32_t* start,
                          const int32_t* end, const int8_t* strand, int ignore_strand,
                          int strand_filter, int mem, Coverage* cv) {
    return split_impl(rd, R, chrom, start, end, strand, ignore_strand, strand_filter, mem, cv, nullptr);
}

int coverage_profile_split(ReadsIdx& rd, int64_t R, const int32_t* chrom, const int32_t* start,
                           const int32_t* end, const int8_t* strand, int ignore_strand,
                           int strand_filter, int mem, int n_bins, int seed, int sample_kind,
                           double scale, double* d_out, int64_t ld, uint8_t* d_is_null) {
    if (n_bins < 1 || n_bins > 30000) return RCP_SPLIT_NOT_APPLICABLE;
    Coverage scratch;
    const FusedReq fz = {n_bins, seed, sample_kind, scale, d_out, ld, d_is_null};
    const int rc = split_impl(rd, R, chrom, start, end, strand, ignore_strand, strand_filter, mem, &scratch, &fz);
    coverage_release(scratch);
    return rc;
}

int coverage_list_split(ReadsIdx& rd, int64_t G, const int64_t* ptr, int64_t n_ranges, const int32_t* chrom,
                        const int32_t* start, const int32_t* end, const int8_t* strand, int ignore_strand,
                        int strand_filter, int mem, Coverage* cv) {
    DebugLap dbg;
    {
        const int rc = reads_build_binned(rd);
        if (rc != RCP_OK) return rc;
    }
    dbg.lap("list: binned index");
    const SplitGeom g = split_geometry(rd);
    const uint32_t max_w = std::max(1u, std::min(rd.max_width, rd.bn_max_pack_w));
    const LongIdx lg = long_index(rd);
    DevIn<int64_t> d_ptr;
    DevIn<int32_t> d_chrom, d_start, d_end;
    DevIn<int8_t> d_strand;
    RCP_TRY(d_ptr.init(ptr, (size_t)G + 1, mem));
    RCP_TRY(d_chrom.init(chrom, (size_t)n_ranges, mem));
    RCP_TRY(d_start.init(start, (size_t)n_ranges, mem));
    RCP_TRY(d_end.init(end, (size_t)n_ranges, mem));
    RCP_TRY(d_strand.init(strand, (size_t)n_ranges, mem));
    Arena A;
    const size_t r = (size_t)G, nr = (size_t)n_ranges;
    RCP_TRY(A.reserve(Arena::pad(64) + Arena::pad(r) * 2 + Arena::pad(r * 4) + Arena::pad(r * 8) * 3 +
                      Arena::pad((r + 1) * 8) + Arena::pad(nr * 4) * 3));
    unsigned int* err = A.take<unsigned int>(16);
    unsigned long long* pstats = reinterpret_cast<unsigned long long*>(err + 4);
    uint8_t* region_hit = A.take<uint8_t>(r);
    const size_t zero_bytes = A.used;
    uint8_t* flags = A.take<uint8_t>(r);
    int32_t* plen = A.take<int32_t>(r);
    int64_t* ntile = A.take<int64_t>(r);
    int64_t* padded = A.take<int64_t>(r);
    int64_t* off_tile = A.take<int64_t>(r + 1);
    ListPlan lp;
    lp.ptr = d_ptr.ptr;
    lp.rstrand = d_strand.ptr;
    lp.xgs = A.take<uint32_t>(nr);
    lp.xge = A.take<uint32_t>(nr);
    lp.xoff = A.take<int32_t>(nr);
    lp.lrange = A.take<uint2>(r);
// ... 66 lines not shown
```

recoup_b200/csrc/profile.cu:

```cuda

#include <algorithm>
#include <cstdlib>
#include <type_traits>

#include "r_rng.cuh"
#include "rcp_internal.cuh"

namespace rcp {

namespace {

constexpr int CTA = 256;
constexpr int WARPS = CTA / 32;

template <class V>
struct Val;
template <>
struct Val<int32_t> {
    using Sum = long long;
    using Key = int;
    static constexpr int KEY_MIN = -0x7fffffff - 1, KEY_MAX = 0x7fffffff;
};
template <>
struct Val<float> {
    using Sum = double;
    using Key = unsigned;
    static constexpr unsigned KEY_MIN = 0u, KEY_MAX = 0xffffffffu;
};
template <class V>
__device__ __forceinline__ typename Val<V>::Sum word_sum(uint32_t w) {
    if constexpr (std::is_same<V, float>::value) return (double)__uint_as_float(w);
    else return (long long)w;
}
template <class V>
__device__ __forceinline__ auto word_val(int w) {
    if constexpr (std::is_same<V, float>::value) return (double)__int_as_float(w);
    else return w;
}
template <class V>
__device__ __forceinline__ double word_double(int w) {
    if constexpr (std::is_same<V, float>::value) return (double)__int_as_float(w);
    else return (double)w;
}
template <class V>
__device__ __forceinline__ typename Val<V>::Key word_key(int w) {
    if constexpr (std::is_same<V, float>::value) {
        const unsigned u = (unsigned)w;
        return (u & 0x80000000u) ? ~u : (u | 0x80000000u);
    } else {
        return w;
    }
}
template <class V>
__device__ __forceinline__ double key_double(typename Val<V>::Key k) {
    if constexpr (std::is_same<V, float>::value)
        return (double)__uint_as_float((k & 0x80000000u) ? (k & 0x7fffffffu) : ~k);
    else return (double)k;
}

struct Seg {
    int a, b;
};

__device__ __forceinline__ Seg segment_of(int L, int where, int f1, int f2) {
    Seg s;
    switch (where) {
        case RCP_WHERE_CENTER: s.a = f1; s.b = L - f2; break;
        case RCP_WHERE_UPSTREAM: s.a = 0; s.b = f1; break;
        case RCP_WHERE_DOWNSTREAM: s.a = L - f2; s.b = L; break;
        default: s.a = 0; s.b = L; break;
    }
    if (s.a < 0) s.a = 0;
    if (s.b > L) s.b = L;
    if (s.b < s.a) s.b = s.a;
    return s;
}

struct BinArgs {
    const int32_t* cov;
    const int64_t* off;
    const int32_t* len;
    const uint8_t* is_null;
    const int* rank;
    int where, f1, f2, n;
    double scale;
    double* out;
    int64_t ld;
    int32_t* short_list;
    unsigned int* short_count;
};

constexpr int STAGE_INTS = 12288;
constexpr int STAGE_MAX_BIN = 128;
constexpr int LONG_REGION_MIN = 16384;

__device__ __forceinline__ long long warp_range_sum(const int32_t* __restrict__ src, int lo, int hi) {
    const int lane = threadIdx.x & 31;
    long long s = 0;
    const int a4 = (lo + 3) & ~3, b4 = hi & ~3;
    if (a4 >= b4) {
        for (int q = lo + lane; q < hi; q += 32) s += __ldg(src + q);
    } else {
        if (lo + lane < a4) s += __ldg(src + lo + lane);
        const int4* v = reinterpret_cast<const int4*>(src + a4);
        const int nv = (b4 - a4) >> 2;
        for (int q = lane; q < nv; q += 32) {
            const int4 x = __ldg(v + q);
            s += (long long)x.x + x.y + x.z + x.w;
        }
        if (b4 + lane < hi) s += __ldg(src + b4 + lane);
    }
#pragma unroll
    for (int d = 16; d > 0; d >>= 1) s += __shfl_xor_sync(0xffffffffu, s, d);
    return s;
}

template <class V>
__global__ void __launch_bounds__(CTA) bin_median_kernel(BinArgs p) {
    using K = typename Val<V>::Key;
    extern __shared__ __align__(16) int sh[];
    int* edges = sh;
    __shared__ int wcount[WARPS];
    __shared__ int chunk_carry;
    const int tid = threadIdx.x, warp = tid >> 5, lane = tid & 31;
    const int64_t r = blockIdx.x;
    const int n = p.n;
    double* out = p.out + r;
    if (p.is_null[r]) {
        for (int i = tid; i < n; i += CTA) out[(int64_t)i * p.ld] = 0.0;
        return;
    }
    const int L = p.len[r];
    const Seg sg = segment_of(L, p.where, p.f1, p.f2);
    const int Ls = sg.b - sg.a;
    if (Ls < n) {
        if (tid == 0) {
            if (Ls <= 0) {
                for (int i = 0; i < n; i++) out[(int64_t)i * p.ld] = 0.0;
            } else {
                p.short_list[atomicAdd(p.short_count, 1u)] = (int32_t)r;
            }
        }
        return;
    }
    const int bsz = Ls / n, dif = Ls - bsz * n;
    if (dif == 0) {
        for (int i = tid; i <= n; i += CTA) edges[i] = sg.a + i * bsz;
        __syncthreads();
    } else {
        if (tid == 0) chunk_carry = 0;
        __syncthreads();
        for (int c0 = 0; c0 < n; c0 += CTA) {
            const int i = c0 + tid;
            const bool extra = (i < n) && (p.rank[i] <= dif);
            const unsigned bal = __ballot_sync(0xffffffffu, extra);
            if (lane == 0) wcount[warp] = __popc(bal);
            __syncthreads();
            int pre = chunk_carry;
            for (int w = 0; w < warp; w++) pre += wcount[w];
            pre += __popc(bal & ((1u << lane) - 1u));
            if (i < n) edges[i] = sg.a + i * bsz + pre;
            __syncthreads();
            if (tid == CTA - 1) chunk_carry = pre + (extra ? 1 : 0);
            __syncthreads();
        }
        if (tid == 0) edges[n] = sg.b;
        __syncthreads();
    }
    const int32_t* src = p.cov + p.off[r];
    int g = 1;
    while (g < 32 && g < bsz) g <<= 1;
    const int per_warp = 32 / g;
    const int sub = lane / g, li = lane % g;
    for (int b0 = warp * per_warp; b0 < n; b0 += WARPS * per_warp) {
        const int i = b0 + sub;
        const bool ok = i < n;
        const int lo = ok ? edges[i] : 0, hi = ok ? edges[i + 1] : 0;
        const int cnt = hi - lo;
        K vmin = Val<V>::KEY_MAX, vmax = Val<V>::KEY_MIN;
        for (int q = lo + li; q < hi; q += g) {
            const K v = word_key<V>(__ldg(src + q));
            vmin = min(vmin, v);
            vmax = max(vmax, v);
        }
        for (int d = g >> 1; d > 0; d >>= 1) {
            vmin = min(vmin, __shfl_xor_sync(0xffffffffu, vmin, d));
            vmax = max(vmax, __shfl_xor_sync(0xffffffffu, vmax, d));
        }
        const int k1 = (cnt - 1) / 2, k2 = cnt / 2;
        K res[2];
#pragma unroll
        for (int t = 0; t < 2; t++) {
            const int k = t == 0 ? k1 : k2;
            K a = vmin, b = vmax;
            K span = ok ? (b - a) : 0;
            for (int d = 16; d > 0; d >>= 1) span = max(span, __shfl_xor_sync(0xffffffffu, span, d));
            while (span > 0) {
                const K mid = a + ((b - a) >> 1);
                int c = 0;
                for (int q = lo + li; q < hi; q += g) c += (word_key<V>(__ldg(src + q)) <= mid);
                for (int d = g >> 1; d > 0; d >>= 1) c += __shfl_xor_sync(0xffffffffu, c, d);
                if (a < b) {
                    if (c >= k + 1) b = mid;
                    else a = mid + 1;
                }
                span >>= 1;
            }
            res[t] = a;
        }
        if (ok && li == 0)
            out[(int64_t)i * p.ld] = p.scale * ((key_double<V>(res[0]) + key_double<V>(res[1])) * 0.5);
    }
}

__device__ __forceinline__ uint32_t smem_u32(const void* p) {
    return (uint32_t)__cvta_generic_to_shared(p);
}
__device__ __forceinline__ void mbar_init(uint64_t* bar, uint32_t count) {
    asm volatile("mbarrier.init.shared::cta.b64 [%0], %1;" ::"r"(smem_u32(bar)), "r"(count) : "memory");
}
__device__ __forceinline__ void mbar_arrive(uint64_t* bar) {
    asm volatile("mbarrier.arrive.shared::cta.b64 _, [%0];" ::"r"(smem_u32(bar)) : "memory");
}
__device__ __forceinline__ void mbar_arrive_expect_tx(uint64_t* bar, uint32_t bytes) {
    asm volatile("mbarrier.arrive.expect_tx.shared::cta.b64 _, [%0], %1;" ::"r"(smem_u32(bar)), "r"(bytes)
                 : "memory");
}
__device__ __forceinline__ void mbar_wait(uint64_t* bar, uint32_t parity) {
    asm volatile(
        "{\n\t"
        ".reg .pred P1;\n\t"
        "WAIT_LOOP:\n\t"
        "mbarrier.try_wait.parity.shared::cta.b64 P1, [%0], %1;\n\t"
        "@P1 bra WAIT_DONE;\n\t"
        "bra WAIT_LOOP;\n\t"
        "WAIT_DONE:\n\t"
        "}" ::"r"(smem_u32(bar)), "r"(parity)
        : "memory");
}
__device__ __forceinline__ void tma_load_1d(void* smem_dst, const void* gmem_src, uint32_t bytes,
                                            uint64_t* bar) {
    asm volatile("cp.async.bulk.shared::cluster.global.mbarrier::complete_tx::bytes [%0], [%1], %2, [%3];"
                 ::"r"(smem_u32(smem_dst)), "l"(gmem_src), "r"(bytes), "r"(smem_u32(bar))
                 : "memory");
}
__device__ __forceinline__ void fence_proxy_async() {
    asm volatile("fence.proxy.async.shared::cta;" ::: "memory");
}

struct __align__(16) BinDesc {
    int off_lo, off_hi, a, b;
    int bsz, dif, lo_al, nvec;
};

constexpr int BT = 256;
constexpr int BWARPS = BT / 32;

__global__ void __launch_bounds__(CTA)
bin_desc_kernel(int64_t R, const int64_t* __restrict__ off, const int32_t* __restrict__ len,
                const uint8_t* __restrict__ is_null, int where, int f1, int f2, int n,
                int buf_ints, BinDesc* __restrict__ desc, int32_t* __restrict__ long_list,
                unsigned int* __restrict__ long_count) {
    const int64_t r = (int64_t)blockIdx.x * CTA + threadIdx.x;
    if (r >= R) return;
    Seg sg;
    sg.a = sg.b = 0;
    if (!is_null[r]) sg = segment_of(len[r], where, f1, f2);
    const uint64_t o = (uint64_t)off[r];
    BinDesc d;
    d.off_lo = (int)(uint32_t)o;
    d.off_hi = (int)(uint32_t)(o >> 32);
    d.a = sg.a;
    d.b = sg.b;
    const int Ls = sg.b - sg.a;
    d.bsz = Ls >= n ? Ls / n : 0;
    d.dif = Ls >= n ? Ls - d.bsz * n : 0;
    d.lo_al = sg.a & ~3;
    d.nvec = 0;
    if (d.bsz > 0 && d.bsz < STAGE_MAX_BIN) {
        const int nvec = (sg.b - d.lo_al + 3) >> 2;
        if (nvec * 4 <= buf_ints) d.nvec = nvec;
    }
    if (d.bsz >= STAGE_MAX_BIN && Ls >= LONG_REGION_MIN) {
        d.nvec = -1;
        long_list[atomicAdd(long_count, 1u)] = (int32_t)r;
    }
    desc[r] = d;
}

__device__ __forceinline__ BinDesc load_bin_desc(const BinDesc* __restrict__ p) {
    const int4 u = __ldg(reinterpret_cast<const int4*>(p));
    const int4 v = __ldg(reinterpret_cast<const int4*>(p) + 1);
    BinDesc d;
    d.off_lo = u.x; d.off_hi = u.y; d.a = u.z; d.b = u.w;
    d.bsz = v.x; d.dif = v.y; d.lo_al = v.z; d.nvec = v.w;
    return d;
}

constexpr int NBUF_MAX = 8;

template <class V>
__global__ void __launch_bounds__(BT)
bin_mean_kernel(BinArgs p, const BinDesc* __restrict__ desc, int64_t R, int buf_ints, int nbuf) {
    using S = typename Val<V>::Sum;
    extern __shared__ __align__(16) int sh[];
    int* edges = sh;
    uint32_t* bufs = reinterpret_cast<uint32_t*>(sh + ((p.n + 1 + 3) & ~3));
    __shared__ int wcount[BWARPS];
    __shared__ int chunk_carry;
    __shared__ __align__(8) uint64_t full_bar[NBUF_MAX];
    __shared__ BinDesc ring[NBUF_MAX];
    const int tid = threadIdx.x, warp = tid >> 5, lane = tid & 31;
    const int n = p.n;
    const int64_t step = gridDim.x;
    int64_t r = blockIdx.x;
    if (r >= R) return;
    if (tid == 0) {
        for (int k = 0; k < nbuf; k++) mbar_init(&full_bar[k], 1);
        fence_proxy_async();
    }
    __syncthreads();
    BinDesc none;
    none.off_lo = none.off_hi = none.a = none.b = none.bsz = none.dif = none.lo_al = none.nvec = 0;

    auto src_of = [&](const BinDesc& d) {
        return p.cov + (int64_t)(((uint64_t)(uint32_t)d.off_hi << 32) | (uint32_t)d.off_lo);
    };
    auto issue = [&](const BinDesc& d, int which) {
        if (tid != 0) return;
        ring[which] = d;
        uint64_t* bar = &full_bar[which];
        if (d.nvec > 0) {
            const uint32_t bytes = (uint32_t)d.nvec * 16u;
            fence_proxy_async();
            mbar_arrive_expect_tx(bar, bytes);
            tma_load_1d(bufs + (size_t)which * buf_ints, src_of(d) + d.lo_al, bytes, bar);
        } else {
            mbar_arrive(bar);
        }
    };

    auto desc_at = [&](int64_t k) {
        const int64_t rr = blockIdx.x + k * step;
        return rr < R ? load_bin_desc(desc + rr) : none;
    };
    for (int k = 0; k < nbuf - 1; k++) issue(desc_at(k), k);
    BinDesc dq = desc_at(nbuf - 1);
    uint32_t parity = 0;
    for (int64_t it = 0;; it++) {
        const int cur = (int)(it % nbuf);
        issue(dq, (int)((it + nbuf - 1) % nbuf));
        dq = desc_at(it + nbuf);
        uint32_t* stage = bufs + (size_t)cur * buf_ints;
        mbar_wait(&full_bar[cur], (parity >> cur) & 1u);
        parity ^= 1u << cur;
        const BinDesc d = ring[cur];
        double* out = p.out + r;
        const int Ls = d.b - d.a;
        if (Ls <= 0) {
            for (int i = tid; i < n; i += BT) out[(int64_t)i * p.ld] = 0.0;
        } else if (d.bsz == 0) {
            if (tid == 0) p.short_list[atomicAdd(p.short_count, 1u)] = (int32_t)r;
        } else if (d.nvec < 0) {
        } else {
            const int bsz = d.bsz, dif = d.dif;
            const bool equal = dif == 0;
            if (!equal) {
                if (tid == 0) chunk_carry = 0;
                __syncthreads();
                for (int c0 = 0; c0 < n; c0 += BT) {
                    const int i = c0 + tid;
                    const bool extra = (i < n) && (p.rank[i] <= dif);
                    const unsigned bal = __ballot_sync(0xffffffffu, extra);
                    if (lane == 0) wcount[warp] = __popc(bal);
                    __syncthreads();
                    int pre = chunk_carry;
                    for (int w = 0; w < warp; w++) pre += wcount[w];
                    pre += __popc(bal & ((1u << lane) - 1u));
                    if (i < n) edges[i] = d.a + i * bsz + pre;
                    __syncthreads();
                    if (tid == BT - 1) chunk_carry = pre + (extra ? 1 : 0);
                    __syncthreads();
                }
                if (tid == 0) edges[n] = d.b;
                __syncthreads();
            }
            auto edge = [&](int i) { return equal ? d.a + i * bsz : edges[i]; };
            const int32_t* src = src_of(d);
            if (bsz < STAGE_MAX_BIN) {
                const bool preloaded = d.nvec > 0;
                const int bins_per_chunk = preloaded ? n : max(1, (buf_ints - 4) / (bsz + 1));
                for (int bin0 = 0; bin0 < n; bin0 += bins_per_chunk) {
                    const int bin1 = min(n, bin0 + bins_per_chunk);
                    const int lo_al = preloaded ? d.lo_al : (edge(bin0) & ~3);
                    const int nvec = preloaded ? d.nvec : ((edge(bin1) - lo_al + 3) >> 2);
                    if (!preloaded) {
                        __syncthreads();
                        const int4* gsrc = reinterpret_cast<const int4*>(src + lo_al);
                        for (int i = tid; i < nvec; i += BT)
                            reinterpret_cast<int4*>(stage)[i] = __ldg(gsrc + i);
                        __syncthreads();
                    }
                    const int nb = bin1 - bin0;
                    int g = 1;
                    while (g < 32 && 2 * g * nb <= BT) g <<= 1;
                    const int part = tid & (g - 1);
                    for (int b0 = bin0; b0 < bin1; b0 += BT / g) {
                        const int b = b0 + tid / g;
                        S s64 = 0;
                        int eb0 = 0, eb1 = 1;
                        if (b < bin1) {
                            eb0 = edge(b);
                            eb1 = edge(b + 1);
                            const int blen = eb1 - eb0;
                            const int share = (blen + g - 1) / g;
                            int q = eb0 - lo_al + part * share;
                            const int qe = min(q + share, eb1 - lo_al);
                            while (q < qe && (q & 3)) s64 += word_sum<V>(stage[q++]);
                            for (; q + 4 <= qe; q += 4) {
                                const uint4 x = *reinterpret_cast<const uint4*>(stage + q);
                                s64 += (word_sum<V>(x.x) + word_sum<V>(x.y)) + (word_sum<V>(x.z) + word_sum<V>(x.w));
                            }
                            while (q < qe) s64 += word_sum<V>(stage[q++]);
                        }
                        for (int dd = g >> 1; dd > 0; dd >>= 1) s64 += __shfl_xor_sync(0xffffffffu, s64, dd);
                        if (b < bin1 && part == 0)
                            out[(int64_t)b * p.ld] = p.scale * ((double)s64 / (double)(eb1 - eb0));
                    }
                }
            } else {
                const int per = (n + BWARPS - 1) / BWARPS;
                const int i0 = warp * per, i1 = min(n, i0 + per);
                if (i0 < i1) {
                    const int lo = edge(i0), hi = edge(i1);
                    int k = i0, nxt = edge(i0 + 1);
                    S acc = 0;
                    constexpr int UW = 4;
                    for (int q0 = lo & ~3; q0 < hi; q0 += 128 * UW) {
                        int4 x[UW];
#pragma unroll
                        for (int u = 0; u < UW; u++) {
                            const int q = q0 + u * 128 + lane * 4;
                            x[u] = make_int4(0, 0, 0, 0);
                            if (q < hi) x[u] = __ldcs(reinterpret_cast<const int4*>(src + q));
                        }
#pragma unroll
                        for (int u = 0; u < UW; u++) {
                            const int row = q0 + u * 128;
                            if (row >= hi) break;
                            const int q = row + lane * 4;
                            auto a0 = word_val<V>(x[u].x), a1 = word_val<V>(x[u].y), a2 = word_val<V>(x[u].z),
                                 a3 = word_val<V>(x[u].w);
                            if (row < lo || row + 128 > hi) {
                                a0 = (q >= lo && q < hi) ? a0 : 0;
                                a1 = (q + 1 >= lo && q + 1 < hi) ? a1 : 0;
                                a2 = (q + 2 >= lo && q + 2 < hi) ? a2 : 0;
                                a3 = (q + 3 >= lo && q + 3 < hi) ? a3 : 0;
                            }
                            const S tot = ((S)a0 + a1) + ((S)a2 + a3);
                            if (row + 128 >= nxt) {
                                const int c = nxt - q;
                                const S before = (S)(c > 0 ? a0 : 0) + (c > 1 ? a1 : 0) +
                                                 (c > 2 ? a2 : 0) + (c > 3 ? a3 : 0);
                                S t = acc + before;
#pragma unroll
                                for (int dd = 16; dd > 0; dd >>= 1) t += __shfl_xor_sync(0xffffffffu, t, dd);
                                const int b0 = edge(k);
                                if (lane == 0) out[(int64_t)k * p.ld] = p.scale * ((double)t / (double)(nxt - b0));
                                acc = tot - before;
                                k++;
                                nxt = k < i1 ? edge(k + 1) : 0x7fffffff;
                            } else {
                                acc += tot;
                            }
                        }
                    }
                }
            }
        }
        r += step;
        if (r >= R) break;
        __syncthreads();
    }
}

constexpr int WIDE_RUN = 16;

template <class V>
__global__ void __launch_bounds__(BT, 3)
bin_wide_kernel(BinArgs p, const BinDesc* __restrict__ desc, const int32_t* __restrict__ long_list,
                unsigned int* __restrict__ long_count) {
    using S = typename Val<V>::Sum;
    const int lane = threadIdx.x & 31;
    const int n = p.n;
    const int runs = (n + WIDE_RUN - 1) / WIDE_RUN;
    const int64_t units = (int64_t)(*long_count) * runs;
    if (units == 0) return;
    for (;;) {
        unsigned long long u = 0;
        if (lane == 0) u = atomicAdd(reinterpret_cast<unsigned long long*>(long_count + 2), 1ull);
        u = __shfl_sync(0xffffffffu, u, 0);
        if ((int64_t)u >= units) break;
        const int64_t r = long_list[u / runs];
        const int i0 = (int)(u % runs) * WIDE_RUN, i1 = min(n, i0 + WIDE_RUN);
        const BinDesc d = load_bin_desc(desc + r);
        const int bsz = d.bsz, dif = d.dif;
        int pre = 0;
        unsigned extra = 0;
        if (dif > 0) {
            for (int j = lane; j < i0; j += 32) pre += (__ldg(p.rank + j) <= dif);
#pragma unroll
            for (int dd = 16; dd > 0; dd >>= 1) pre += __shfl_xor_sync(0xffffffffu, pre, dd);
            extra = __ballot_sync(0xffffffffu, i0 + lane < i1 && __ldg(p.rank + i0 + lane) <= dif);
        }
        const int lo = d.a + i0 * bsz + pre;
        const int hi = lo + (i1 - i0) * bsz + __popc(extra);
        const int32_t* src = p.cov + (int64_t)(((uint64_t)(uint32_t)d.off_hi << 32) | (uint32_t)d.off_lo);
        double* out = p.out + r;
        int k = i0, b0 = lo, nxt = lo + bsz + (int)(extra & 1u);
        S acc = 0;
        constexpr int UW = 4;
        auto fetch = [&](int q0, int4* x) {
#pragma unroll
            for (int v = 0; v < UW; v++) {
                const int q = q0 + v * 128 + lane * 4;
                x[v] = make_int4(0, 0, 0, 0);
                if (q < hi) x[v] = __ldcs(reinterpret_cast<const int4*>(src + q));
            }
        };
        int4 x[UW], y[UW];
        fetch(lo & ~3, x);
        for (int q0 = lo & ~3; q0 < hi; q0 += 128 * UW) {
            if (q0 + 128 * UW < hi) fetch(q0 + 128 * UW, y);
#pragma unroll
            for (int v = 0; v < UW; v++) {
                const int row = q0 + v * 128;
                if (row >= hi) break;
                const int q = row + lane * 4;
                auto a0 = word_val<V>(x[v].x), a1 = word_val<V>(x[v].y), a2 = word_val<V>(x[v].z),
                     a3 = word_val<V>(x[v].w);
                if (row < lo || row + 128 > hi) {
                    a0 = (q >= lo && q < hi) ? a0 : 0;
                    a1 = (q + 1 >= lo && q + 1 < hi) ? a1 : 0;
                    a2 = (q + 2 >= lo && q + 2 < hi) ? a2 : 0;
                    a3 = (q + 3 >= lo && q + 3 < hi) ? a3 : 0;
                }
                const S tot = ((S)a0 + a1) + ((S)a2 + a3);
                if (row + 128 >= nxt) {
                    const int c = nxt - q;
                    const S before = (S)(c > 0 ? a0 : 0) + (c > 1 ? a1 : 0) +
                                     (c > 2 ? a2 : 0) + (c > 3 ? a3 : 0);
                    S t = acc + before;
#pragma unroll
                    for (int dd = 16; dd > 0; dd >>= 1) t += __shfl_xor_sync(0xffffffffu, t, dd);
                    if (lane == 0) out[(int64_t)k * p.ld] = p.scale * ((double)t / (double)(nxt - b0));
                    acc = tot - before;
                    k++;
                    b0 = nxt;
                    nxt = k < i1 ? nxt + bsz + (int)((extra >> (k - i0)) & 1u) : 0x7fffffff;
                } else {
                    acc += tot;
                }
            }
#pragma unroll
            for (int v = 0; v < UW; v++) x[v] = y[v];
        }
    }
}

struct InterpArgs {
    const int32_t* cov;
    const int64_t* off;
    const int32_t* len;
    int where, f1, f2, n;
    int interp, seed, sample_kind;
    double scale;
    double* out;
    int64_t ld;
    const int32_t* short_list;
    const unsigned int* short_count;
};

template <class V>
__global__ void __launch_bounds__(32) interp_kernel(InterpArgs p) {
    extern __shared__ double shd[];
    const int n = p.n;
    double* y = shd;
    double* cb = shd + n;
    double* cc = shd + 2 * n;
    double* cd = shd + 3 * n;
    int* ia = reinterpret_cast<int*>(shd + 4 * n);
    int* ib = ia + n;
    RRng* rng = reinterpret_cast<RRng*>(ib + n);
    const int lane = threadIdx.x;
    const unsigned int count = *p.short_count;
    for (unsigned int w = blockIdx.x; w < count; w += gridDim.x) {
        const int64_t r = p.short_list[w];
        const int L_all = p.len[r];
        const Seg sg = segment_of(L_all, p.where, p.f1, p.f2);
        const int L = sg.b - sg.a;
        const V* src = reinterpret_cast<const V*>(p.cov) + p.off[r] + sg.a;
        double* out = p.out + r;
        __syncwarp();
        bool neighborhood = p.interp == RCP_INTERP_NEIGHBORHOOD;
        if (p.interp == RCP_INTERP_AUTO) neighborhood = ((double)(n - L) / (double)n) < 0.2;
        if (neighborhood && (L < 4 || n < 6)) {
            for (int i = lane; i < n; i += 32) out[(int64_t)i * p.ld] = nan("");
            continue;
        }
        if (!neighborhood) {
            for (int i = lane; i < L; i += 32) y[i] = (double)src[i];
            __syncwarp();
            if (lane == 0) {
                double *b = cb, *c = cc, *d = cd;
                for (int i = 0; i < L; i++) b[i] = c[i] = d[i] = 0.0;
                if (L == 2) {
                    b[0] = b[1] = y[1] - y[0];
                } else if (L >= 3) {
                    const int nm1 = L - 1;
                    d[0] = 1.0;
                    c[1] = (y[1] - y[0]) / d[0];
                    for (int i = 1; i < nm1; i++) {
                        d[i] = 1.0;
                        b[i] = 2.0 * (d[i - 1] + d[i]);
                        c[i + 1] = (y[i + 1] - y[i]) / d[i];
                        c[i] = c[i + 1] - c[i];
                    }
                    b[0] = -d[0];
                    b[L - 1] = -d[L - 2];
                    c[0] = c[L - 1] = 0.0;
                    if (L > 3) {
                        c[0] = c[2] / 2.0 - c[1] / 2.0;
                        c[L - 1] = c[L - 2] / 2.0 - c[L - 3] / 2.0;
                        c[0] = c[0] * d[0] * d[0] / 3.0;
                        c[L - 1] = -c[L - 1] * d[L - 2] * d[L - 2] / 3.0;
                    }
                    for (int i = 1; i < L; i++) {
                        const double t = d[i - 1] / b[i - 1];
                        b[i] = b[i] - t * d[i - 1];
                        c[i] = c[i] - t * c[i - 1];
                    }
                    c[L - 1] = c[L - 1] / b[L - 1];
                    for (int i = L - 2; i >= 0; i--) c[i] = (c[i] - d[i] * c[i + 1]) / b[i];
                    b[L - 1] = (y[L - 1] - y[L - 2]) / d[L - 2] + d[L - 2] * (c[L - 2] + 2.0 * c[L - 1]);
                    for (int i = 0; i < nm1; i++) {
                        b[i] = (y[i + 1] - y[i]) / d[i] - d[i] * (c[i + 1] + 2.0 * c[i]);
                        d[i] = (c[i + 1] - c[i]) / d[i];
                        c[i] = 3.0 * c[i];
                    }
                    c[L - 1] = 3.0 * c[L - 1];
                    d[L - 1] = d[L - 2];
                }
            }
            __syncwarp();
            const double by = n > 2 ? ((double)L - 1.0) / (double)(n - 1) : 0.0;
            for (int l = lane; l < n; l += 32) {
                double ul = 1.0 + (double)l * by;
                if (l == 0) ul = 1.0;
                if (l == n - 1 && n > 1) ul = (double)L;
                int i = (int)floor(ul) - 1;
                if (i > L - 2) i = L - 2;
                if (i < 0) i = 0;
                const double dx = ul - (double)(i + 1);
                double v = y[i] + dx * (cb[i] + dx * (cc[i] + dx * cd[i]));
                if (v < 0.0) v = 0.0;
                out[(int64_t)l * p.ld] = p.scale * v;
            }
        } else {
            for (int i = lane; i < n; i += 32) {
                y[i] = nan("");
                ia[i] = 0;
            }
            __syncwarp();
            if (lane == 0) {
                y[0] = (double)src[0];
                y[1] = (double)src[1];
                y[n - 2] = (double)src[L - 2];
                y[n - 1] = (double)src[L - 1];
                rng->seed((uint32_t)p.seed, p.sample_kind);
                const int pool = n - 4, k = L - 4;
                int* x = ib;
                for (int i = 0; i < pool; i++) x[i] = i;
                int m = pool;
                for (int i = 0; i < k; i++) {
                    const int j = (int)rng->index((uint32_t)m);
                    ia[x[j]] = 1;
                    x[j] = x[--m];
                }
                int q = 2;
                for (int i = 0; i < pool; i++)
                    if (ia[i]) y[2 + i] = (double)src[q++];
            }
            __syncwarp();
            for (int i = lane; i < n; i += 32) cb[i] = y[i];
            __syncwarp();
            for (int z = lane; z < n; z += 32) {
                double v = cb[z];
                if (isnan(v)) {
                    double s = 0.0;
                    int c = 0;
                    const int nb[4] = {z - 2, z - 1, z + 1, z + 2};
#pragma unroll
                    for (int t = 0; t < 4; t++) {
                        const double u = cb[nb[t]];
                        if (!isnan(u)) { s += u; c++; }
                    }
                    v = c ? s / (double)c : nan("");
                }
                out[(int64_t)z * p.ld] = p.scale * v;
            }
        }
    }
}

struct BaseArgs {
    const int32_t* cov;
    const int64_t* off;
    const int32_t* len;
    const uint8_t* is_null;
    int where, f1, f2;
    int64_t R, n_cols;
    double scale;
    double* out;
    int64_t ld;
};

template <class V>
__global__ void __launch_bounds__(256) base_matrix_kernel(BaseArgs p) {
    __shared__ int tile[32][33];
    __shared__ int64_t r_off[32];
    __shared__ int r_a[32], r_b[32];
    const int tx = threadIdx.x, ty = threadIdx.y;
    const int64_t r0 = (int64_t)blockIdx.y * 32, k0 = (int64_t)blockIdx.x * 32;
    if (ty == 0) {
        const int64_t r = r0 + tx;
        int a = 0, b = 0;
        int64_t o = 0;
        if (r < p.R && !p.is_null[r]) {
            const Seg sg = segment_of(p.len[r], p.where, p.f1, p.f2);
            a = sg.a;
            b = sg.b;
            o = p.off[r];
        }
        r_off[tx] = o;
        r_a[tx] = a;
        r_b[tx] = b;
    }
    __syncthreads();
    for (int jj = ty; jj < 32; jj += 8) {
        const int64_t k = k0 + tx;
        const int q = r_a[jj] + (int)k;
        int v = 0;
        if (k < p.n_cols && q < r_b[jj]) v = __ldg(p.cov + r_off[jj] + q);
        tile[jj][tx] = v;
    }
    __syncthreads();
    for (int jj = ty; jj < 32; jj += 8) {
        const int64_t k = k0 + jj, r = r0 + tx;
        if (r < p.R && k < p.n_cols) p.out[k * p.ld + r] = p.scale * word_double<V>(tile[tx][jj]);
    }
}

constexpr int BW_ROWS = 32, BW_COLS = 256;

template <class V>
__global__ void __launch_bounds__(256) base_matrix_wide_kernel(BaseArgs p, int64_t col_tiles,
                                                               int vec_store) {
    __shared__ int tile[BW_ROWS][BW_COLS + 1];
    __shared__ int64_t r_off[BW_ROWS];
    __shared__ int r_a[BW_ROWS], r_b[BW_ROWS];
    const int tid = threadIdx.x, warp = tid >> 5, lane = tid & 31;
    const int64_t r0 = ((int64_t)blockIdx.x / col_tiles) * BW_ROWS;
    const int64_t k0 = ((int64_t)blockIdx.x % col_tiles) * BW_COLS;
    if (tid < BW_ROWS) {
        const int64_t r = r0 + tid;
        int a = 0, b = 0;
        int64_t o = 0;
        if (r < p.R && !p.is_null[r]) {
            const Seg sg = segment_of(p.len[r], p.where, p.f1, p.f2);
            a = sg.a;
            b = sg.b;
            o = p.off[r];
        }
        r_off[tid] = o;
        r_a[tid] = a;
        r_b[tid] = b;
    }
    __syncthreads();
    for (int jj = warp; jj < BW_ROWS; jj += 8) {
        const int a = r_a[jj], b = r_b[jj];
        const int32_t* src = p.cov + r_off[jj] + a + k0;
        const int avail = (int)min((int64_t)(b - a) - k0, (int64_t)BW_COLS);
#pragma unroll
        for (int h = 0; h < BW_COLS / 128; h++) {
            const int c = h * 128 + lane * 4;
            int4 v = make_int4(0, 0, 0, 0);
            if ((a & 3) == 0 && c + 3 < avail) {
                v = __ldg(reinterpret_cast<const int4*>(src + c));
            } else {
                if (c < avail) v.x = __ldg(src + c);
                if (c + 1 < avail) v.y = __ldg(src + c + 1);
                if (c + 2 < avail) v.z = __ldg(src + c + 2);
                if (c + 3 < avail) v.w = __ldg(src + c + 3);
            }
            tile[jj][c] = v.x;
            tile[jj][c + 1] = v.y;
            tile[jj][c + 2] = v.z;
            tile[jj][c + 3] = v.w;
        }
    }
    __syncthreads();
    const int ncol = (int)min((int64_t)BW_COLS, p.n_cols - k0);
    if (vec_store && r0 + BW_ROWS <= p.R) {
        const int rr = (lane & 15) * 2, dc = lane >> 4;
        for (int c = warp * 2 + dc; c < ncol; c += 16) {
            const double2 v = make_double2(p.scale * word_double<V>(tile[rr][c]), p.scale * word_double<V>(tile[rr + 1][c]));
            *reinterpret_cast<double2*>(p.out + (k0 + c) * p.ld + r0 + rr) = v;
        }
    } else {
        const int64_t r = r0 + lane;
        if (r < p.R)
            for (int c = warp; c < ncol; c += 8) p.out[(k0 + c) * p.ld + r] = p.scale * word_double<V>(tile[lane][c]);
    }
}

template <class V>
int bin_matrix_impl(const Coverage& cv, int where, int f1, int f2, int n_bins, int stat,
                    int interp, int seed, int sample_kind, double* d_out, int64_t ld) {
    const int64_t R = cv.n_regions;
    if (R == 0) return RCP_OK;
    std::vector<int> rank((size_t)n_bins), perm((size_t)n_bins), scratch((size_t)n_bins);
    {
        RRng* rng = new RRng;
        rng->seed((uint32_t)seed, sample_kind);
        rng->sample(n_bins, n_bins, scratch.data(), perm.data());
        delete rng;
        for (int pos = 0; pos < n_bins; pos++) rank[(size_t)perm[(size_t)pos] - 1] = pos + 1;
    }
    int* d_rank = nullptr;
    int32_t* short_list = nullptr;
    unsigned int* short_count = nullptr;
    RCP_TRY(dalloc(&d_rank, (size_t)n_bins));
    RCP_TRY(dalloc(&short_list, (size_t)R));
    RCP_TRY(dalloc(&short_count, 1));
    RCP_CUDA(cudaMemcpyAsync(d_rank, rank.data(), (size_t)n_bins * sizeof(int),
                             cudaMemcpyHostToDevice, g_ctx.stream));
    RCP_CUDA(cudaMemsetAsync(short_count, 0, sizeof(unsigned int), g_ctx.stream));
    BinArgs a;
    a.cov = cv.cov;
    a.off = cv.off;
    a.len = cv.len;
    a.is_null = cv.is_null;
    a.rank = d_rank;
    a.where = where;
    a.f1 = f1;
    a.f2 = f2;
    a.n = n_bins;
    a.scale = cv.scale;
    a.out = d_out;
    a.ld = ld;
    a.short_list = short_list;
    a.short_count = short_count;
    const size_t edge_bytes = (((size_t)n_bins + 1 + 3) & ~(size_t)3) * sizeof(int);
    if (edge_bytes > 150 * 1024) return fail(RCP_ERR_UNSUPPORTED, "more than ~38000 bins per segment");
    BinDesc* d_desc = nullptr;
    int32_t* long_list = nullptr;
    unsigned int* long_count = nullptr;
    if (stat == RCP_STAT_MEDIAN) {
        StageTimer t(ST_PROF_BIN);
        const size_t smem = edge_bytes;
        if (smem > 48 * 1024)
            RCP_CUDA(cudaFuncSetAttribute(bin_median_kernel<V>,
                                          cudaFuncAttributeMaxDynamicSharedMemorySize, (int)smem));
        bin_median_kernel<V><<<(unsigned)R, CTA, smem, g_ctx.stream>>>(a);
        RCP_LAUNCHED();
    } else {
        RCP_TRY(dalloc(&d_desc, (size_t)R));
        StageTimer t(ST_PROF_BIN);
        int64_t seg_max = cv.max_len;
        if (where == RCP_WHERE_UPSTREAM) seg_max = std::min<int64_t>(seg_max, f1);
        else if (where == RCP_WHERE_DOWNSTREAM) seg_max = std::min<int64_t>(seg_max, f2);
        else if (where == RCP_WHERE_CENTER) seg_max = std::max<int64_t>(seg_max - f1 - f2, 0);
        int buf_ints = (int)std::min<int64_t>(STAGE_INTS, ((seg_max + 10) & ~(int64_t)3));
        int per_sm = 4;
        {
            const int64_t live = std::max<int64_t>(R - cv.n_null, 1);
            int64_t seg_mean = cv.total_len / live;
            if (where == RCP_WHERE_UPSTREAM) seg_mean = std::min<int64_t>(seg_mean, f1);
            else if (where == RCP_WHERE_DOWNSTREAM) seg_mean = std::min<int64_t>(seg_mean, f2);
            else if (where == RCP_WHERE_CENTER) seg_mean = std::max<int64_t>(seg_mean - f1 - f2, 0);
            if (seg_mean / n_bins >= 128) {
                per_sm = 8;
                buf_ints = std::min(buf_ints, 6144);
            }
        }
        RCP_TRY(dalloc(&long_list, (size_t)R));
        RCP_TRY(dalloc(&long_count, 4));
        RCP_CUDA(cudaMemsetAsync(long_count, 0, 4 * sizeof(unsigned int), g_ctx.stream));
        bin_desc_kernel<<<(unsigned)((R + CTA - 1) / CTA), CTA, 0, g_ctx.stream>>>(
            R, cv.off, cv.len, cv.is_null, where, f1, f2, n_bins, buf_ints, d_desc, long_list, long_count);
        RCP_LAUNCHED();
        int nbuf = 2;
        if (const char* e = getenv("RCP_BIN_CTAS")) per_sm = std::max(1, atoi(e));
        const size_t budget = 220u * 1024u / (size_t)per_sm - 1024u;
        nbuf = (int)((budget - edge_bytes) / ((size_t)buf_ints * sizeof(int)));
        nbuf = std::max(1, std::min(nbuf, NBUF_MAX));
        const size_t smem = edge_bytes + (size_t)nbuf * buf_ints * sizeof(int);
        RCP_CUDA(cudaFuncSetAttribute(bin_mean_kernel<V>, cudaFuncAttributeMaxDynamicSharedMemorySize,
                                      (int)smem));
        int fit = 0;
        RCP_CUDA(cudaOccupancyMaxActiveBlocksPerMultiprocessor(&fit, bin_mean_kernel<V>, BT, smem));
        if (fit < 1) return fail(RCP_ERR_UNSUPPORTED, "bin kernel does not fit (%zu bytes of shared memory)", smem);
        const int64_t grid = std::min<int64_t>(R, (int64_t)g_ctx.sm_count * std::min(fit, per_sm));
        bin_mean_kernel<V><<<(unsigned)grid, BT, smem, g_ctx.stream>>>(a, d_desc, R, buf_ints, nbuf);
        RCP_LAUNCHED();
        bin_wide_kernel<V><<<(unsigned)(g_ctx.sm_count * 8), BT, 0, g_ctx.stream>>>(a, d_desc, long_list, long_count);
        RCP_LAUNCHED();
    }
    InterpArgs ia;
    ia.cov = cv.cov;
    ia.off = cv.off;
    ia.len = cv.len;
    ia.where = where;
    ia.f1 = f1;
    ia.f2 = f2;
    ia.n = n_bins;
    ia.interp = interp;
    ia.seed = seed;
    ia.sample_kind = sample_kind;
    ia.scale = cv.scale;
    ia.out = d_out;
    ia.ld = ld;
    ia.short_list = short_list;
    ia.short_count = short_count;
    const size_t ismem = (size_t)n_bins * (4 * sizeof(double) + 2 * sizeof(int)) + 8 + sizeof(RRng);
    if (ismem > 220 * 1024)
        return fail(RCP_ERR_UNSUPPORTED, "interpolation supports at most ~5500 bins per segment");
    if (ismem > 48 * 1024)
        RCP_CUDA(cudaFuncSetAttribute(interp_kernel<V>, cudaFuncAttributeMaxDynamicSharedMemorySize,
                                      (int)ismem));
    int iblocks = g_ctx.sm_count * 8;
    if ((int64_t)iblocks > R) iblocks = (int)R;
    {
        StageTimer t(ST_PROF_INTERP);
        interp_kernel<V><<<(unsigned)iblocks, 32, ismem, g_ctx.stream>>>(ia);
        RCP_LAUNCHED();
    }
    dfree(d_desc);
    dfree(long_list);
    dfree(long_count);
    dfree(d_rank);
    dfree(short_list);
    dfree(short_count);
    return RCP_OK;
}

template <class V>
int base_matrix_impl(const Coverage& cv, int where, int f1, int f2, int64_t n_cols,
                     double* d_out, int64_t ld) {
    const int64_t R = cv.n_regions;
    if (R == 0 || n_cols == 0) return RCP_OK;
    BaseArgs a;
    a.cov = cv.cov;
    a.off = cv.off;
    a.len = cv.len;
    a.is_null = cv.is_null;
    a.where = where;
    a.f1 = f1;
    a.f2 = f2;
    a.R = R;
    a.n_cols = n_cols;
    a.scale = cv.scale;
    a.out = d_out;
    a.ld = ld;
    StageTimer t(ST_PROF_BASE);
    if (n_cols >= 128) {
        const int64_t col_tiles = (n_cols + BW_COLS - 1) / BW_COLS, row_tiles = (R + BW_ROWS - 1) / BW_ROWS;
        if (col_tiles * row_tiles <= 0x7fffffff) {
            const int vec = ((ld & 1) == 0) && ((reinterpret_cast<uintptr_t>(d_out) & 15u) == 0);
            base_matrix_wide_kernel<V><<<(unsigned)(col_tiles * row_tiles), 256, 0, g_ctx.stream>>>(
                a, col_tiles, vec);
            RCP_LAUNCHED();
            return RCP_OK;
        }
    }
    const int64_t gy = (R + 31) / 32, gx = (n_cols + 31) / 32;
    if (gy > 65535) {
        for (int64_t y0 = 0; y0 < gy; y0 += 65535) {
            BaseArgs s = a;
            const int64_t rows0 = y0 * 32;
            s.off = a.off + rows0;
            s.len = a.len + rows0;
            s.is_null = a.is_null + rows0;
            s.R = (R - rows0) < 65535 * 32 ? (R - rows0) : 65535 * 32;
            s.out = a.out + rows0;
            const int64_t gys = (s.R + 31) / 32;
            base_matrix_kernel<V><<<dim3((unsigned)gx, (unsigned)gys), dim3(32, 8), 0, g_ctx.stream>>>(s);
            RCP_LAUNCHED();
        }
    } else {
        base_matrix_kernel<V><<<dim3((unsigned)gx, (unsigned)gy), dim3(32, 8), 0, g_ctx.stream>>>(a);
        RCP_LAUNCHED();
    }
    return RCP_OK;
}

}

int bin_matrix_device(const Coverage& cv, int where, int f1, int f2, int n_bins, int stat,
                      int interp, int seed, int sample_kind, double* d_out, int64_t ld) {
    if (cv.value_type == RCP_VALUE_FLOAT32)
        return bin_matrix_impl<float>(cv, where, f1, f2, n_bins, stat, interp, seed, sample_kind, d_out, ld);
    return bin_matrix_impl<int32_t>(cv, where, f1, f2, n_bins, stat, interp, seed, sample_kind, d_out, ld);
}

int base_matrix_device(const Coverage& cv, int where, int f1, int f2, int64_t n_cols,
                       double* d_out, int64_t ld) {
    if (cv.value_type == RCP_VALUE_FLOAT32) return base_matrix_impl<float>(cv, where, f1, f2, n_cols, d_out, ld);
    return base_matrix_impl<int32_t>(cv, where, f1, f2, n_cols, d_out, ld);
}

}
```

recoup_b200/csrc/rcp_internal.cuh:

```cuda
#pragma once
#include <cuda_runtime.h>
#include <stdint.h>

#include <string>
#include <vector>

#include "recoup_b200.h"

namespace rcp {

struct Ctx {
    bool ready = false;
    int device = -1;
    int sm_count = 0;
    int cc_major = 0, cc_minor = 0;
    size_t mem_bytes = 0;
    cudaStream_t stream = nullptr;
    int64_t launches = 0;
    int coverage_path = RCP_PATH_AUTO;
    bool deferred_validation = false;
};
extern Ctx g_ctx;

int fail(int code, const char* fmt, ...);
// ... 143 lines not shown
    uint32_t* cye = nullptr;
};

struct ReadsIdx {
    int64_t n = 0;
    int n_chrom = 0;
    bool has_strand = false;
    uint32_t max_width = 0;
    uint32_t uniform_w = 0;
    int64_t n_exc = 0;
    uint32_t* exc_xw = nullptr;
    uint32_t* exc_e1 = nullptr;
    int8_t* exc_st = nullptr;
    int key_bits = 32;
    std::vector<int64_t> chrom_len;
    std::vector<uint32_t> chrom_off;
    int64_t* d_chrom_len = nullptr;
    uint32_t* d_chrom_off = nullptr;
    bool any_na = false;
    std::vector<uint8_t> len_na;
    uint8_t* d_len_na = nullptr;
    uint32_t* g_start = nullptr;
    uint32_t* g_end1 = nullptr;
    int8_t* d_strand = nullptr;
    SortedClass cls[CLS_N];
    bool pairs_built = false;
    uint32_t* p_end1 = nullptr;
    int8_t* p_strand = nullptr;
    uint32_t* p_maxend1 = nullptr;
    size_t device_bytes = 0;
    char* bn_base = nullptr;
    uint32_t* bn_cand = nullptr;
    uint32_t* bn_boff = nullptr;
    uint32_t* bn_cb = nullptr;
    int bn_P = 0;
    bool bn_stranded = false;
    int64_t ln_n = 0;
    uint32_t bn_max_pack_w = 0;
    uint32_t* ln_xs = nullptr;
    uint32_t* ln_e1 = nullptr;
    int8_t* ln_st = nullptr;
    uint32_t* ln_maxe1 = nullptr;
    bool pending = false;
    bool pd_rle = false;
    unsigned int* pd_err = nullptr;
    unsigned long long* pd_cnt = nullptr;
    unsigned int* pd_w = nullptr;
    uint32_t* pd_run_total = nullptr;
    uint32_t* pd_run_first = nullptr;
    uint32_t pd_exc_cap = 0;
    bool pd_eager_index = false;
    unsigned int h_err = 0, h_w[4] = {0, 0, 0, 0}, h_total = 0;
    uint32_t long_thr = 0;
    int64_t n_long = 0;
    unsigned long long h_cnt[4] = {0, 0, 0, 0};
};

inline int split_position_bits(int64_t span) {
    int P = 16;
    while (P < 22 && ((span + (1ll << P) - 1) >> P) > 1024) P++;
    return P;
}

int reads_pending_items(ReadsIdx& r, FetchItem* items, int* n);
int reads_finish(ReadsIdx& r);
int reads_resolve(ReadsIdx& r);

int reads_build_class(ReadsIdx& r, int cls);
int reads_build_pairs(ReadsIdx& r);
void reads_release(ReadsIdx& r);

struct Coverage {
    int64_t n_regions = 0;
    int64_t total_padded = 0;
    int64_t total_len = 0;
    int64_t n_null = 0;
    int32_t max_len = 0;
    int path = 0;
    int64_t candidates = 0;
    unsigned long long* d_stats = nullptr;
    bool stats_pending = false;
    double scale = 1.0;
    int value_type = RCP_VALUE_INT32;
    int32_t* cov = nullptr;
    int64_t* off = nullptr;
    int32_t* len = nullptr;
    uint8_t* is_null = nullptr;
};
void coverage_release(Coverage& c);
int coverage_resolve_stats(Coverage& c);
int coverage_na_rule(const ReadsIdx& rd, Coverage& cv, int64_t R, const int32_t* d_chrom, const int8_t* d_strand,
                     const int64_t* d_end_pos);

ReadsIdx* get_reads(int h);
Coverage* get_coverage(int h);
int new_coverage(Coverage** out, int* handle);

int sort_keys_u32(uint32_t* keys_in_out, int64_t n, int end_bit);
int sort_pairs_u32(uint32_t* keys_in_out, uint32_t* vals_in_out, int64_t n, int end_bit);
int running_max_u32_device(const uint32_t* in, uint32_t* out, int64_t n);
int exclusive_scan_i64(const int64_t* in, int64_t* out, int64_t n, int64_t* d_total);
int exclusive_scan_u32(const uint32_t* in, uint32_t* out, int64_t n, uint32_t* d_total);
int exclusive_scan_u32_bounded(const uint32_t* in, uint32_t* out, int64_t n_upper, const uint32_t* n_dev,
                               uint32_t* d_total);
int exclusive_scan2_i64(const int64_t* in0, int64_t* out0, int64_t* d_total0, const int64_t* in1,
                        int64_t* out1, int64_t* d_total1, int64_t n);

}
```

Before: 48.89 billion.

## Store coverage as uint16 when device-computed bound fits, halving coverage traffic

Adds a device-side upper bound on per-tile coverage depth, computed with warp max-reductions and an atomicMax during split descriptor setup. When the bound fits in 16 bits, the split coverage kernel writes coverage as packed uint16, and every consumer (bin, interp, base matrix, RLE, pack, concat, NA rule) reads through a narrow-aware accessor chosen at runtime from that bound. This targets the memory bandwidth spent writing and rereading the int32 coverage buffer. In exchange it adds a templated code path in every reader, an extra device read of the bound in each kernel, and wider staging buffers.

```diff
diff --git a/include/recoup_b200.h b/include/recoup_b200.h
--- a/include/recoup_b200.h
+++ b/include/recoup_b200.h
@@ -141,6 +141,7 @@
 int rcp_signal_coverage(int signal, int64_t n_elements, const int64_t* ptr, const int32_t* chrom,
                         const int32_t* start, const int32_t* end, const int8_t* strand, int mem, int* cov_out);
 int rcp_coverage_value_type(int cov, int* type);
+int rcp_coverage_storage_bytes(int cov, int* bytes);
 int rcp_coverage_fetch_f32(int cov, int64_t first, int64_t count, float* out, int64_t capacity);
 int rcp_coverage_rle_f32(int cov, int64_t first, int64_t count, int64_t* run_ptr_out,
                          float* values_out, int32_t* lengths_out, int64_t capacity);
diff --git a/recoup_b200/_lib.py b/recoup_b200/_lib.py
--- a/recoup_b200/_lib.py
+++ b/recoup_b200/_lib.py
@@ -92,6 +92,7 @@
     "rcp_signal_free": (C.c_int, [C.c_int]),
     "rcp_signal_coverage": (C.c_int, [C.c_int, C.c_int64, _i64p, _vp, _vp, _vp, _vp, C.c_int, _ip]),
     "rcp_coverage_value_type": (C.c_int, [C.c_int, _ip]),
+    "rcp_coverage_storage_bytes": (C.c_int, [C.c_int, _ip]),
     "rcp_coverage_fetch_f32": (C.c_int, [C.c_int, C.c_int64, C.c_int64, _vp, C.c_int64]),
     "rcp_coverage_rle_f32": (C.c_int, [C.c_int, C.c_int64, C.c_int64, _i64p, _vp, _i32p, C.c_int64]),
     "rcp_bin_matrix": (C.c_int, [C.c_int, C.c_int, C.c_int, C.c_int, C.c_int, C.c_int, C.c_int, C.c_int,
diff --git a/recoup_b200/csrc/api.cu b/recoup_b200/csrc/api.cu
--- a/recoup_b200/csrc/api.cu
+++ b/recoup_b200/csrc/api.cu
@@ -1018,6 +1018,21 @@
     return RCP_OK;
 }
 
+int rcp_coverage_storage_bytes(int cov, int* bytes) {
+    RCP_TRY(require_ready());
+    Coverage* cv = get_coverage(cov);
+    if (!cv) return fail(RCP_ERR_HANDLE, "unknown coverage handle %d", cov);
+    if (bytes == nullptr) return fail(RCP_ERR_ARG, "bytes is NULL");
+    *bytes = 4;
+    if (cv->d_bound) {
+        unsigned long long bound = 0;
+        const FetchItem items[1] = {{cv->d_bound, &bound, 8}};
+        RCP_TRY(fetch_and_sync(items, 1));
+        if (bound <= NARROW_MAX) *bytes = 2;
+    }
+    return RCP_OK;
+}
+
 int rcp_coverage_rle(int cov, int64_t first, int64_t count, int64_t* run_ptr_out,
                      int32_t* values_out, int32_t* lengths_out, int64_t capacity) {
     RCP_TRY(require_ready());
diff --git a/recoup_b200/csrc/coverage.cu b/recoup_b200/csrc/coverage.cu
--- a/recoup_b200/csrc/coverage.cu
+++ b/recoup_b200/csrc/coverage.cu
@@ -487,25 +487,29 @@
                    const int64_t* __restrict__ o1, const int32_t* __restrict__ l1,
                    const int32_t* __restrict__ c2, const int64_t* __restrict__ o2,
                    const int32_t* __restrict__ l2, const int32_t* __restrict__ len,
-                   const int64_t* __restrict__ off, int32_t* __restrict__ cov) {
+                   const int64_t* __restrict__ off, int32_t* __restrict__ cov,
+                   const unsigned long long* __restrict__ w0, const unsigned long long* __restrict__ w1,
+                   const unsigned long long* __restrict__ w2) {
     const int64_t r = blockIdx.x;
     if (len[r] == 0) return;
     int32_t* dst = cov + off[r];
     const int a = l0[r], b = l1[r], c = l2[r];
-    for (int i = threadIdx.x; i < a; i += CTA) dst[i] = c0[o0[r] + i];
-    for (int i = threadIdx.x; i < b; i += CTA) dst[a + i] = c1[o1[r] + i];
-    for (int i = threadIdx.x; i < c; i += CTA) dst[a + b + i] = c2[o2[r] + i];
+    const bool n0 = cov_narrow(w0), n1 = cov_narrow(w1), n2 = cov_narrow(w2);
+    for (int i = threadIdx.x; i < a; i += CTA) dst[i] = cov_at(c0, o0[r] + i, n0);
+    for (int i = threadIdx.x; i < b; i += CTA) dst[a + i] = cov_at(c1, o1[r] + i, n1);
+    for (int i = threadIdx.x; i < c; i += CTA) dst[a + b + i] = cov_at(c2, o2[r] + i, n2);
 }
 
 __global__ void __launch_bounds__(CTA)
 pack_kernel(const int32_t* __restrict__ cov, const int64_t* __restrict__ off,
             const int32_t* __restrict__ len, const int64_t* __restrict__ packed_off,
-            int64_t first, int32_t* __restrict__ out) {
+            int64_t first, int32_t* __restrict__ out, const unsigned long long* __restrict__ bound) {
     const int64_t r = first + blockIdx.x;
     const int L = len[r];
-    const int32_t* src = cov + off[r];
+    const bool narrow = cov_narrow(bound);
+    const int64_t o = off[r];
     int32_t* dst = out + packed_off[blockIdx.x];
-    for (int i = threadIdx.x; i < L; i += CTA) dst[i] = src[i];
+    for (int i = threadIdx.x; i < L; i += CTA) dst[i] = cov_at(cov, o + i, narrow);
 }
 
 __global__ void __launch_bounds__(CTA)
@@ -517,13 +521,16 @@
 
 __global__ void __launch_bounds__(CTA)
 rle_count_kernel(const int32_t* __restrict__ cov, const int64_t* __restrict__ off,
-                 const int32_t* __restrict__ len, int64_t first, int64_t* __restrict__ n_runs) {
+                 const int32_t* __restrict__ len, int64_t first, int64_t* __restrict__ n_runs,
+                 const unsigned long long* __restrict__ bound) {
     __shared__ int wsum[WARPS];
     const int64_t r = first + blockIdx.x;
     const int L = len[r];
-    const int32_t* x = cov + off[r];
+    const bool narrow = cov_narrow(bound);
+    const int64_t o = off[r];
     int c = 0;
-    for (int i = threadIdx.x; i < L; i += CTA) c += (i == 0) || (x[i] != x[i - 1]);
+    for (int i = threadIdx.x; i < L; i += CTA)
+        c += (i == 0) || (cov_at(cov, o + i, narrow) != cov_at(cov, o + i - 1, narrow));
     for (int d = 16; d > 0; d >>= 1) c += __shfl_xor_sync(0xffffffffu, c, d);
     if ((threadIdx.x & 31) == 0) wsum[threadIdx.x >> 5] = c;
     __syncthreads();
@@ -538,12 +545,13 @@
 rle_write_kernel(const int32_t* __restrict__ cov, const int64_t* __restrict__ off,
                  const int32_t* __restrict__ len, int64_t first,
                  const int64_t* __restrict__ run_ptr, int32_t* __restrict__ values,
-                 int32_t* __restrict__ starts) {
+                 int32_t* __restrict__ starts, const unsigned long long* __restrict__ bound) {
     __shared__ int wsum[WARPS];
     __shared__ int carry_s;
     const int64_t r = first + blockIdx.x;
     const int L = len[r];
-    const int32_t* x = cov + off[r];
+    const bool narrow = cov_narrow(bound);
+    const int64_t o = off[r];
     const int64_t base = run_ptr[blockIdx.x];
     const int lane = threadIdx.x & 31, warp = threadIdx.x >> 5;
     if (threadIdx.x == 0) carry_s = 0;
@@ -553,8 +561,8 @@
         int v = 0;
         bool head = false;
         if (i < L) {
-            v = x[i];
-            head = (i == 0) || (v != x[i - 1]);
+            v = cov_at(cov, o + i, narrow);
+            head = (i == 0) || (v != cov_at(cov, o + i - 1, narrow));
         }
         const unsigned bal = __ballot_sync(0xffffffffu, head);
         if (lane == 0) wsum[warp] = __popc(bal);
@@ -695,6 +703,7 @@
     dfree(c.len);
     dfree(c.is_null);
     dfree(c.d_stats);
+    c.d_bound = nullptr;
     c.stats_pending = false;
 }
 
@@ -703,14 +712,14 @@
 na_rule_kernel(int64_t R, const int32_t* __restrict__ chrom, const int8_t* __restrict__ strand,
                const uint8_t* __restrict__ len_na, int n_chrom, const int64_t* __restrict__ off,
                int32_t* __restrict__ len, uint8_t* __restrict__ is_null, const int32_t* __restrict__ cov,
-               const int64_t* __restrict__ end_pos) {
+               const int64_t* __restrict__ end_pos, const unsigned long long* __restrict__ bound) {
     const int64_t r = (int64_t)blockIdx.x * CTA + threadIdx.x;
     if (r >= R) return;
     const int32_t L = len[r];
     const int c = chrom[r];
     if (L <= 0 || c < 0 || c >= n_chrom || !len_na[c]) return;
     const int64_t idx = end_pos ? end_pos[r] : ((strand && strand[r] < 0) ? 0 : (int64_t)L - 1);
-    if (idx < 0 || idx >= L || cov[off[r] + idx] == 0) {
+    if (idx < 0 || idx >= L || cov_at(cov, off[r] + idx, cov_narrow(bound)) == 0) {
         len[r] = 0;
         is_null[r] = 1;
     }
@@ -746,7 +755,7 @@
     const unsigned long long h[4] = {0ull, 0ull, 0ull, (unsigned long long)cv.candidates};
     RCP_CUDA(cudaMemcpyAsync(cv.d_stats, h, 32, cudaMemcpyHostToDevice, g_ctx.stream));
     na_rule_kernel<<<blocks_for(R, CTA), CTA, 0, g_ctx.stream>>>(R, d_chrom, d_strand, rd.d_len_na, rd.n_chrom, cv.off,
-                                                               cv.len, cv.is_null, cv.cov, d_end_pos);
+                                                               cv.len, cv.is_null, cv.cov, d_end_pos, cv.d_bound);
     RCP_LAUNCHED();
     len_stats_kernel<<<blocks_for(R, CTA), CTA, 0, g_ctx.stream>>>(R, cv.len, cv.d_stats);
     RCP_LAUNCHED();
@@ -954,7 +963,8 @@
     if (R > 0) {
         concat_copy_kernel<<<(unsigned)R, CTA, 0, g_ctx.stream>>>(a.cov, a.off, a.len, b.cov, b.off,
                                                                  b.len, c.cov, c.off, c.len,
-                                                                 cv->len, cv->off, cv->cov);
+                                                                 cv->len, cv->off, cv->cov, a.d_bound,
+                                                                 b.d_bound, c.d_bound);
         RCP_LAUNCHED();
     }
     dfree(padded);
@@ -986,7 +996,7 @@
         rc = dalloc(&packed, (size_t)total);
         if (rc == RCP_OK) {
             pack_kernel<<<(unsigned)count, CTA, 0, g_ctx.stream>>>(cv.cov, cv.off, cv.len, poff,
-                                                                  first, packed);
+                                                                  first, packed, cv.d_bound);
             g_ctx.launches++;
             cudaError_t e = cudaMemcpyAsync(out, packed, (size_t)total * 4, cudaMemcpyDeviceToHost,
                                             g_ctx.stream);
@@ -1011,7 +1021,7 @@
     int64_t *n_runs = nullptr, *d_ptr = nullptr;
     RCP_TRY(dalloc(&n_runs, (size_t)count));
     RCP_TRY(dalloc(&d_ptr, (size_t)count + 1));
-    rle_count_kernel<<<(unsigned)count, CTA, 0, g_ctx.stream>>>(cv.cov, cv.off, cv.len, first, n_runs);
+    rle_count_kernel<<<(unsigned)count, CTA, 0, g_ctx.stream>>>(cv.cov, cv.off, cv.len, first, n_runs, cv.d_bound);
     RCP_LAUNCHED();
     RCP_TRY(exclusive_scan_i64(n_runs, d_ptr, count, d_ptr + count));
     RCP_CUDA(cudaMemcpyAsync(run_ptr, d_ptr, ((size_t)count + 1) * 8, cudaMemcpyDeviceToHost,
@@ -1031,7 +1041,7 @@
             if (rc == RCP_OK) rc = dalloc(&d_len, (size_t)total);
             if (rc == RCP_OK) {
                 rle_write_kernel<<<(unsigned)count, CTA, 0, g_ctx.stream>>>(cv.cov, cv.off, cv.len, first,
-                                                                           d_ptr, d_val, d_start);
+                                                                           d_ptr, d_val, d_start, cv.d_bound);
                 g_ctx.launches++;
                 rle_lengths_kernel<<<(unsigned)count, CTA, 0, g_ctx.stream>>>(cv.len, first, d_ptr,
                                                                              d_start, d_len);
diff --git a/recoup_b200/csrc/coverage_split.cu b/recoup_b200/csrc/coverage_split.cu
--- a/recoup_b200/csrc/coverage_split.cu
+++ b/recoup_b200/csrc/coverage_split.cu
@@ -55,9 +55,9 @@
                int32_t* __restrict__ plen, uint8_t* __restrict__ flags, int64_t* __restrict__ ntile,
                int64_t* __restrict__ padded, uint32_t* __restrict__ tab, unsigned int* __restrict__ err,
                unsigned long long* __restrict__ pstats ,
-               unsigned long long* __restrict__ zero4 ) {
+               unsigned long long* __restrict__ zero5 ) {
     const int64_t r = (int64_t)blockIdx.x * CTA + threadIdx.x;
-    if (r < 4) zero4[r] = 0ull;
+    if (r < 5) zero5[r] = 0ull;
     unsigned long long my_len = 0;
     if (r < R) {
         const int st = strand ? (int)strand[r] : 0;
@@ -118,8 +118,9 @@
                 uint32_t max_w, uint32_t pmask, const uint32_t* __restrict__ boff, SpDesc* __restrict__ desc,
                 uint32_t* __restrict__ tabs,
                 const uint32_t* __restrict__ lxs, const uint32_t* __restrict__ lmax, uint32_t ln,
-                uint2* __restrict__ lrange) {
+                uint2* __restrict__ lrange, unsigned long long* __restrict__ bound) {
     const int64_t t = (int64_t)blockIdx.x * CTA + threadIdx.x;
+    const unsigned live = __ballot_sync(0xffffffffu, t < T);
     if (t >= T) return;
     const int64_t r = sp_owner_of(off_tile, R, t);
     const int L = plen[r];
@@ -149,6 +150,7 @@
     d.flags = flags[r];
     d.region = (uint32_t)r;
     desc[t] = d;
+    uint32_t most = d.n;
     if (ln) {
         tabs[t] = tstart;
         const uint32_t hi = tstart + tlen - 1u;
@@ -167,6 +169,11 @@
             else b = mid;
         }
         lrange[t] = make_uint2(a, c1);
+        most = most + (c1 - a) < most ? 0xffffffffu : most + (c1 - a);
+    }
+    if (bound) {
+        most = __reduce_max_sync(live, most);
+        if ((threadIdx.x & 31) == 0) atomicMax(bound, (unsigned long long)most);
     }
 }
 
@@ -694,8 +701,8 @@
     return lo < hi;
 }
 
-template <int RPW, bool STORE = true>
-__device__ __forceinline__ void warp_scan_store_fwd(int* diff, int tlen, int32_t* __restrict__ dst) {
+template <int RPW, class O = int32_t>
+__device__ __forceinline__ void warp_scan_store_fwd(int* diff, int tlen, O* __restrict__ dst) {
     const int lane = threadIdx.x & 31;
     int* mine = diff + lane * 4 * RPW;
     int4 v[RPW];
@@ -707,6 +714,7 @@
     }
     const int inc = warp_inclusive_scan(sum);
     int run = inc - sum;
+    if (sizeof(O) == 2) __syncwarp();
 #pragma unroll
     for (int k = 0; k < RPW; k++) {
         int4 o;
@@ -714,13 +722,34 @@
         o.y = (run += v[k].y);
         o.z = (run += v[k].z);
         o.w = (run += v[k].w);
-        *(reinterpret_cast<int4*>(mine) + k) = o;
+        if (sizeof(O) == 2)
+            *(reinterpret_cast<uint2*>(diff) + lane * RPW + k) =
+                make_uint2(((uint32_t)o.x & 0xffffu) | ((uint32_t)o.y << 16), ((uint32_t)o.z & 0xffffu) | ((uint32_t)o.w << 16));
+        else
+            *(reinterpret_cast<int4*>(mine) + k) = o;
     }
     __syncwarp();
-    if (STORE && lane == 0) {
+    if (lane == 0) {
         fence_proxy_async_smem();
-        tma_store_1d(dst, diff, (uint32_t)((tlen + 3) & ~3) * 4u);
+        constexpr int E = 16 / (int)sizeof(O);
+        tma_store_1d(dst, diff, (uint32_t)((tlen + E - 1) & ~(E - 1)) * (uint32_t)sizeof(O));
         tma_store_commit();
+    }
+}
+
+__device__ __forceinline__ void warp_rows_store_u16(const int* diff, int tlen, uint16_t* __restrict__ dst) {
+    const int lane = threadIdx.x & 31;
+    int pre = 0;
+    for (int row = 0; row * ROW < tlen; row++) {
+        const int4 v = *(reinterpret_cast<const int4*>(diff + row * ROW) + lane);
+        const int i0 = v.x, i1 = i0 + v.y, i2 = i1 + v.z, i3 = i2 + v.w;
+        const int inc = warp_inclusive_scan(i3);
+        const int ex = pre + inc - i3;
+        if (row * ROW + lane * 4 < tlen)
+            *reinterpret_cast<uint2*>(dst + row * ROW + lane * 4) =
+                make_uint2(((uint32_t)(ex + i0) & 0xffffu) | ((uint32_t)(ex + i1) << 16),
+                           ((uint32_t)(ex + i2) & 0xffffu) | ((uint32_t)(ex + i3) << 16));
+        pre += __shfl_sync(0xffffffffu, inc, 31);
     }
 }
 
@@ -828,8 +857,10 @@
 __global__ void __launch_bounds__(CTA, RCP_WTILE_OCC)
 sp_wtile_kernel(int64_t T, const SpDesc* __restrict__ desc, const uint32_t* __restrict__ cand, int P,
                 int32_t* __restrict__ cov, uint8_t* __restrict__ region_hit, FusedBins fb, LongIdx lg,
-                const uint32_t* __restrict__ tabs, const uint2* __restrict__ lrange) {
+                const uint32_t* __restrict__ tabs, const uint2* __restrict__ lrange,
+                const unsigned long long* __restrict__ bound) {
     extern __shared__ __align__(16) unsigned char wt_smem[];
+    const bool narrow = !FUSED && cov_narrow(bound);
     const int warp = threadIdx.x >> 5;
     const uint32_t lane = threadIdx.x & 31;
     int* diff = reinterpret_cast<int*>(wt_smem) + warp * WT_ONE;
@@ -945,6 +976,18 @@
                     default: prefixed = warp_scan_prefix2<8>(diff); break;
                 }
                 tile_to_bins(diff, d, fb, prefixed);
+            }
+        } else if (narrow) {
+            uint16_t* dst = reinterpret_cast<uint16_t*>(cov) + d.out;
+            switch (rows) {
+                case 1: warp_scan_store_fwd<1>(diff, d.tlen, dst); break;
+                case 2: warp_scan_store_fwd<2>(diff, d.tlen, dst); break;
+                case 3: warp_scan_store_fwd<3>(diff, d.tlen, dst); break;
+                case 4: warp_scan_store_fwd<4>(diff, d.tlen, dst); break;
+                case 5: warp_scan_store_fwd<5>(diff, d.tlen, dst); break;
+                case 6: warp_scan_store_fwd<6>(diff, d.tlen, dst); break;
+                case 7: warp_scan_store_fwd<7>(diff, d.tlen, dst); break;
+                default: warp_rows_store_u16(diff, d.tlen, dst); break;
             }
         } else {
             int32_t* dst = cov + d.out;
@@ -1481,7 +1524,7 @@
     RCP_TRY(dalloc(&cv->off, r + 1));
     RCP_TRY(dalloc(&cv->len, r));
     RCP_TRY(dalloc(&cv->is_null, r));
-    RCP_TRY(dalloc(&cv->d_stats, 4));
+    RCP_TRY(dalloc(&cv->d_stats, 5));
     auto give_up = [&]() {
         dfree(cv->off);
         dfree(cv->len);
@@ -1492,7 +1535,7 @@
     {
         StageTimer t(ST_SP_PLAN);
         RCP_CUDA(cudaMemsetAsync(A.base, 0, zero_bytes, g_ctx.stream));
-        if (R == 0) RCP_CUDA(cudaMemsetAsync(cv->d_stats, 0, 32, g_ctx.stream));
+        if (R == 0) RCP_CUDA(cudaMemsetAsync(cv->d_stats, 0, 40, g_ctx.stream));
         if (R > 0) {
             sp_plan_kernel<<<blocks_for(R, CTA), CTA, 0, g_ctx.stream>>>(
                 R, d_chrom.ptr, d_start.ptr, d_end.ptr, d_strand.ptr, rd.d_chrom_off, rd.d_chrom_len,
@@ -1566,7 +1609,9 @@
         cv->n_null = 0;
         cv->stats_pending = true;
         RCP_TRY(dalloc(&cv->cov, (size_t)h.total_padded));
-    }
+        if (getenv("RCP_COVERAGE_WIDE") == nullptr) cv->d_bound = cv->d_stats + 4;
+    }
+    unsigned long long* bound = cv->d_bound ? cv->d_stats + 4 : nullptr;
 
     bool words_stranded = stranded;
     if (have_index) {
@@ -1591,7 +1636,7 @@
         sp_tiles_kernel<<<blocks_for(T, CTA), CTA, 0, g_ctx.stream>>>(R, T, off_tile, gs, plen, flags,
                                                                      fz ? nullptr : cv->off, fb.edge, fb.n, max_w, pmask, boff,
                                                                      desc, tabs,
-                                                                     lg.xs, lg.maxe1, lg.n, lrange);
+                                                                     lg.xs, lg.maxe1, lg.n, lrange, bound);
         RCP_LAUNCHED();
     }
     if (T > 0) {
@@ -1605,7 +1650,7 @@
                 per_sm = std::max(per_sm, 1);
                 kern<<<(unsigned)std::min<int64_t>(want, (int64_t)g_ctx.sm_count * per_sm), CTA, WTILE_SMEM,
                        g_ctx.stream>>>(
-                    T, desc, cand, P, cv->cov, region_hit, fb, lg, tabs, lrange);
+                    T, desc, cand, P, cv->cov, region_hit, fb, lg, tabs, lrange, bound);
                 RCP_LAUNCHED();
                 return RCP_OK;
             };
diff --git a/recoup_b200/csrc/profile.cu b/recoup_b200/csrc/profile.cu
--- a/recoup_b200/csrc/profile.cu
+++ b/recoup_b200/csrc/profile.cu
@@ -58,6 +58,36 @@
     else return (double)k;
 }
 
+template <class S>
+constexpr int LOG_PER16 = sizeof(S) == 2 ? 3 : 2;
+template <class S>
+using Word = typename std::conditional<sizeof(S) == 2, uint16_t, uint32_t>::type;
+template <class V, class S>
+__device__ __forceinline__ typename Val<V>::Sum unit_sum(uint4 x) {
+    if constexpr (sizeof(S) == 2) {
+        return (long long)(((x.x & 0xffffu) + (x.x >> 16)) + ((x.y & 0xffffu) + (x.y >> 16)) +
+                           ((x.z & 0xffffu) + (x.z >> 16)) + ((x.w & 0xffffu) + (x.w >> 16)));
+    } else {
+        return (word_sum<V>(x.x) + word_sum<V>(x.y)) + (word_sum<V>(x.z) + word_sum<V>(x.w));
+    }
+}
+template <class S>
+using Raw4 = typename std::conditional<sizeof(S) == 2, uint2, int4>::type;
+__device__ __forceinline__ int4 widen4(int4 v) { return v; }
+__device__ __forceinline__ int4 widen4(uint2 u) {
+    return make_int4((int)(u.x & 0xffffu), (int)(u.x >> 16), (int)(u.y & 0xffffu), (int)(u.y >> 16));
+}
+template <class S>
+__device__ __forceinline__ Raw4<S> load4_cs(const S* p) {
+    return __ldcs(reinterpret_cast<const Raw4<S>*>(p));
+}
+template <class S>
+__device__ __forceinline__ int4 load4_g(const S* p) {
+    return widen4(__ldg(reinterpret_cast<const Raw4<S>*>(p)));
+}
+template <class S>
+constexpr int ROWS_IN_FLIGHT = sizeof(S) == 2 ? 8 : 4;
+
 struct Seg {
     int a, b;
 };
@@ -78,6 +108,7 @@
 
 struct BinArgs {
     const int32_t* cov;
+    const unsigned long long* bound;
     const int64_t* off;
     const int32_t* len;
     const uint8_t* is_null;
@@ -115,13 +146,17 @@
     return s;
 }
 
-template <class V>
-__global__ void __launch_bounds__(CTA) bin_median_kernel(BinArgs p) {
+struct MedianSmem {
+    int wcount[WARPS];
+    int chunk_carry;
+};
+template <class V, class S>
+__device__ __forceinline__ void bin_median_run(const BinArgs& p, MedianSmem& sm) {
     using K = typename Val<V>::Key;
     extern __shared__ __align__(16) int sh[];
     int* edges = sh;
-    __shared__ int wcount[WARPS];
-    __shared__ int chunk_carry;
+    auto& wcount = sm.wcount;
+    auto& chunk_carry = sm.chunk_carry;
     const int tid = threadIdx.x, warp = tid >> 5, lane = tid & 31;
     const int64_t r = blockIdx.x;
     const int n = p.n;
@@ -167,7 +202,7 @@
         if (tid == 0) edges[n] = sg.b;
         __syncthreads();
     }
-    const int32_t* src = p.cov + p.off[r];
+    const S* src = reinterpret_cast<const S*>(p.cov) + p.off[r];
     int g = 1;
     while (g < 32 && g < bsz) g <<= 1;
     const int per_warp = 32 / g;
@@ -213,6 +248,15 @@
     }
 }
 
+template <class V>
+__global__ void __launch_bounds__(CTA) bin_median_kernel(BinArgs p) {
+    __shared__ MedianSmem sm;
+    if constexpr (std::is_same<V, int32_t>::value) {
+        if (cov_narrow(p.bound)) return bin_median_run<V, uint16_t>(p, sm);
+    }
+    bin_median_run<V, int32_t>(p, sm);
+}
+
 __device__ __forceinline__ uint32_t smem_u32(const void* p) {
     return (uint32_t)__cvta_generic_to_shared(p);
 }
@@ -260,9 +304,12 @@
 bin_desc_kernel(int64_t R, const int64_t* __restrict__ off, const int32_t* __restrict__ len,
                 const uint8_t* __restrict__ is_null, int where, int f1, int f2, int n,
                 int buf_ints, BinDesc* __restrict__ desc, int32_t* __restrict__ long_list,
-                unsigned int* __restrict__ long_count) {
+                unsigned int* __restrict__ long_count, const unsigned long long* __restrict__ bound) {
     const int64_t r = (int64_t)blockIdx.x * CTA + threadIdx.x;
     if (r >= R) return;
+    const bool narrow = cov_narrow(bound);
+    const int sh = narrow ? 3 : 2;
+    const int cap = narrow ? (buf_ints >> 1) & ~3 : buf_ints;
     Seg sg;
     sg.a = sg.b = 0;
     if (!is_null[r]) sg = segment_of(len[r], where, f1, f2);
@@ -275,11 +322,11 @@
     const int Ls = sg.b - sg.a;
     d.bsz = Ls >= n ? Ls / n : 0;
     d.dif = Ls >= n ? Ls - d.bsz * n : 0;
-    d.lo_al = sg.a & ~3;
+    d.lo_al = sg.a & ~((1 << sh) - 1);
     d.nvec = 0;
     if (d.bsz > 0 && d.bsz < STAGE_MAX_BIN) {
-        const int nvec = (sg.b - d.lo_al + 3) >> 2;
-        if (nvec * 4 <= buf_ints) d.nvec = nvec;
+        const int nvec = (sg.b - d.lo_al + (1 << sh) - 1) >> sh;
+        if (nvec * 4 <= cap) d.nvec = nvec;
     }
     if (d.bsz >= STAGE_MAX_BIN && Ls >= LONG_REGION_MIN) {
         d.nvec = -1;
@@ -299,17 +346,28 @@
 
 constexpr int NBUF_MAX = 8;
 
-template <class V>
-__global__ void __launch_bounds__(BT)
-bin_mean_kernel(BinArgs p, const BinDesc* __restrict__ desc, int64_t R, int buf_ints, int nbuf) {
+struct MeanSmem {
+    int wcount[BWARPS];
+    int chunk_carry;
+    __align__(8) uint64_t full_bar[NBUF_MAX];
+    BinDesc ring[NBUF_MAX];
+};
+template <class V, class ST>
+__device__ __forceinline__ void bin_mean_run(const BinArgs& p, const BinDesc* __restrict__ desc, int64_t R,
+                                             int buf_ints, int nbuf, MeanSmem& sm) {
     using S = typename Val<V>::Sum;
+    constexpr int ESH = LOG_PER16<ST>, E = 1 << ESH;
+    if (sizeof(ST) == 2) {
+        buf_ints = (buf_ints >> 1) & ~3;
+        nbuf = min(2 * nbuf, NBUF_MAX);
+    }
     extern __shared__ __align__(16) int sh[];
     int* edges = sh;
     uint32_t* bufs = reinterpret_cast<uint32_t*>(sh + ((p.n + 1 + 3) & ~3));
-    __shared__ int wcount[BWARPS];
-    __shared__ int chunk_carry;
-    __shared__ __align__(8) uint64_t full_bar[NBUF_MAX];
-    __shared__ BinDesc ring[NBUF_MAX];
+    auto& wcount = sm.wcount;
+    auto& chunk_carry = sm.chunk_carry;
+    auto& full_bar = sm.full_bar;
+    auto& ring = sm.ring;
     const int tid = threadIdx.x, warp = tid >> 5, lane = tid & 31;
     const int n = p.n;
     const int64_t step = gridDim.x;
@@ -324,7 +382,7 @@
     none.off_lo = none.off_hi = none.a = none.b = none.bsz = none.dif = none.lo_al = none.nvec = 0;
 
     auto src_of = [&](const BinDesc& d) {
-        return p.cov + (int64_t)(((uint64_t)(uint32_t)d.off_hi << 32) | (uint32_t)d.off_lo);
+        return reinterpret_cast<const ST*>(p.cov) + (int64_t)(((uint64_t)(uint32_t)d.off_hi << 32) | (uint32_t)d.off_lo);
     };
     auto issue = [&](const BinDesc& d, int which) {
         if (tid != 0) return;
@@ -386,14 +444,15 @@
                 __syncthreads();
             }
             auto edge = [&](int i) { return equal ? d.a + i * bsz : edges[i]; };
-            const int32_t* src = src_of(d);
+            const ST* src = src_of(d);
+            const Word<ST>* staged = reinterpret_cast<const Word<ST>*>(stage);
             if (bsz < STAGE_MAX_BIN) {
                 const bool preloaded = d.nvec > 0;
-                const int bins_per_chunk = preloaded ? n : max(1, (buf_ints - 4) / (bsz + 1));
+                const int bins_per_chunk = preloaded ? n : max(1, ((buf_ints << (ESH - 2)) - E) / (bsz + 1));
                 for (int bin0 = 0; bin0 < n; bin0 += bins_per_chunk) {
                     const int bin1 = min(n, bin0 + bins_per_chunk);
-                    const int lo_al = preloaded ? d.lo_al : (edge(bin0) & ~3);
-                    const int nvec = preloaded ? d.nvec : ((edge(bin1) - lo_al + 3) >> 2);
+                    const int lo_al = preloaded ? d.lo_al : (edge(bin0) & ~(E - 1));
+                    const int nvec = preloaded ? d.nvec : ((edge(bin1) - lo_al + E - 1) >> ESH);
                     if (!preloaded) {
                         __syncthreads();
                         const int4* gsrc = reinterpret_cast<const int4*>(src + lo_al);
@@ -416,12 +475,9 @@
                             const int share = (blen + g - 1) / g;
                             int q = eb0 - lo_al + part * share;
                             const int qe = min(q + share, eb1 - lo_al);
-                            while (q < qe && (q & 3)) s64 += word_sum<V>(stage[q++]);
-                            for (; q + 4 <= qe; q += 4) {
-                                const uint4 x = *reinterpret_cast<const uint4*>(stage + q);
-                                s64 += (word_sum<V>(x.x) + word_sum<V>(x.y)) + (word_sum<V>(x.z) + word_sum<V>(x.w));
-                            }
-                            while (q < qe) s64 += word_sum<V>(stage[q++]);
+                            while (q < qe && (q & (E - 1))) s64 += word_sum<V>(staged[q++]);
+                            for (; q + E <= qe; q += E) s64 += unit_sum<V, ST>(*reinterpret_cast<const uint4*>(staged + q));
+                            while (q < qe) s64 += word_sum<V>(staged[q++]);
                         }
                         for (int dd = g >> 1; dd > 0; dd >>= 1) s64 += __shfl_xor_sync(0xffffffffu, s64, dd);
                         if (b < bin1 && part == 0)
@@ -435,22 +491,23 @@
                     const int lo = edge(i0), hi = edge(i1);
                     int k = i0, nxt = edge(i0 + 1);
                     S acc = 0;
-                    constexpr int UW = 4;
+                    constexpr int UW = ROWS_IN_FLIGHT<ST>;
                     for (int q0 = lo & ~3; q0 < hi; q0 += 128 * UW) {
-                        int4 x[UW];
+                        Raw4<ST> x[UW];
 #pragma unroll
                         for (int u = 0; u < UW; u++) {
                             const int q = q0 + u * 128 + lane * 4;
-                            x[u] = make_int4(0, 0, 0, 0);
-                            if (q < hi) x[u] = __ldcs(reinterpret_cast<const int4*>(src + q));
+                            x[u] = Raw4<ST>{};
+                            if (q < hi) x[u] = load4_cs(src + q);
                         }
 #pragma unroll
                         for (int u = 0; u < UW; u++) {
                             const int row = q0 + u * 128;
                             if (row >= hi) break;
                             const int q = row + lane * 4;
-                            auto a0 = word_val<V>(x[u].x), a1 = word_val<V>(x[u].y), a2 = word_val<V>(x[u].z),
-                                 a3 = word_val<V>(x[u].w);
+                            const int4 xu = widen4(x[u]);
+                            auto a0 = word_val<V>(xu.x), a1 = word_val<V>(xu.y), a2 = word_val<V>(xu.z),
+                                 a3 = word_val<V>(xu.w);
                             if (row < lo || row + 128 > hi) {
                                 a0 = (q >= lo && q < hi) ? a0 : 0;
                                 a1 = (q + 1 >= lo && q + 1 < hi) ? a1 : 0;
@@ -484,12 +541,22 @@
     }
 }
 
+template <class V>
+__global__ void __launch_bounds__(BT)
+bin_mean_kernel(BinArgs p, const BinDesc* __restrict__ desc, int64_t R, int buf_ints, int nbuf) {
+    __shared__ MeanSmem sm;
+    if constexpr (std::is_same<V, int32_t>::value) {
+        if (cov_narrow(p.bound)) return bin_mean_run<V, uint16_t>(p, desc, R, buf_ints, nbuf, sm);
+    }
+    bin_mean_run<V, int32_t>(p, desc, R, buf_ints, nbuf, sm);
+}
+
 constexpr int WIDE_RUN = 16;
 
-template <class V>
-__global__ void __launch_bounds__(BT, 3)
-bin_wide_kernel(BinArgs p, const BinDesc* __restrict__ desc, const int32_t* __restrict__ long_list,
-                unsigned int* __restrict__ long_count) {
+template <class V, class ST>
+__device__ __forceinline__ void bin_wide_run(const BinArgs& p, const BinDesc* __restrict__ desc,
+                                             const int32_t* __restrict__ long_list,
+                                             unsigned int* __restrict__ long_count) {
     using S = typename Val<V>::Sum;
     const int lane = threadIdx.x & 31;
     const int n = p.n;
@@ -515,20 +582,20 @@
         }
         const int lo = d.a + i0 * bsz + pre;
         const int hi = lo + (i1 - i0) * bsz + __popc(extra);
-        const int32_t* src = p.cov + (int64_t)(((uint64_t)(uint32_t)d.off_hi << 32) | (uint32_t)d.off_lo);
+        const ST* src = reinterpret_cast<const ST*>(p.cov) + (int64_t)(((uint64_t)(uint32_t)d.off_hi << 32) | (uint32_t)d.off_lo);
         double* out = p.out + r;
         int k = i0, b0 = lo, nxt = lo + bsz + (int)(extra & 1u);
         S acc = 0;
-        constexpr int UW = 4;
-        auto fetch = [&](int q0, int4* x) {
+        constexpr int UW = ROWS_IN_FLIGHT<ST>;
+        auto fetch = [&](int q0, Raw4<ST>* x) {
 #pragma unroll
             for (int v = 0; v < UW; v++) {
                 const int q = q0 + v * 128 + lane * 4;
-                x[v] = make_int4(0, 0, 0, 0);
-                if (q < hi) x[v] = __ldcs(reinterpret_cast<const int4*>(src + q));
+                x[v] = Raw4<ST>{};
+                if (q < hi) x[v] = load4_cs(src + q);
             }
         };
-        int4 x[UW], y[UW];
+        Raw4<ST> x[UW], y[UW];
         fetch(lo & ~3, x);
         for (int q0 = lo & ~3; q0 < hi; q0 += 128 * UW) {
             if (q0 + 128 * UW < hi) fetch(q0 + 128 * UW, y);
@@ -537,8 +604,9 @@
                 const int row = q0 + v * 128;
                 if (row >= hi) break;
                 const int q = row + lane * 4;
-                auto a0 = word_val<V>(x[v].x), a1 = word_val<V>(x[v].y), a2 = word_val<V>(x[v].z),
-                     a3 = word_val<V>(x[v].w);
+                const int4 xv = widen4(x[v]);
+                auto a0 = word_val<V>(xv.x), a1 = word_val<V>(xv.y), a2 = word_val<V>(xv.z),
+                     a3 = word_val<V>(xv.w);
                 if (row < lo || row + 128 > hi) {
                     a0 = (q >= lo && q < hi) ? a0 : 0;
                     a1 = (q + 1 >= lo && q + 1 < hi) ? a1 : 0;
@@ -568,8 +636,19 @@
     }
 }
 
+template <class V>
+__global__ void __launch_bounds__(BT, 3)
+bin_wide_kernel(BinArgs p, const BinDesc* __restrict__ desc, const int32_t* __restrict__ long_list,
+                unsigned int* __restrict__ long_count) {
+    if constexpr (std::is_same<V, int32_t>::value) {
+        if (cov_narrow(p.bound)) return bin_wide_run<V, uint16_t>(p, desc, long_list, long_count);
+    }
+    bin_wide_run<V, int32_t>(p, desc, long_list, long_count);
+}
+
 struct InterpArgs {
     const int32_t* cov;
+    const unsigned long long* bound;
     const int64_t* off;
     const int32_t* len;
     int where, f1, f2, n;
@@ -581,8 +660,9 @@
     const unsigned int* short_count;
 };
 
-template <class V>
-__global__ void __launch_bounds__(32) interp_kernel(InterpArgs p) {
+template <class V, class ST>
+__device__ __forceinline__ void interp_run(const InterpArgs& p) {
+    using E = typename std::conditional<sizeof(ST) == 2, uint16_t, V>::type;
     extern __shared__ double shd[];
     const int n = p.n;
     double* y = shd;
@@ -599,7 +679,7 @@
         const int L_all = p.len[r];
         const Seg sg = segment_of(L_all, p.where, p.f1, p.f2);
         const int L = sg.b - sg.a;
-        const V* src = reinterpret_cast<const V*>(p.cov) + p.off[r] + sg.a;
+        const E* src = reinterpret_cast<const E*>(p.cov) + p.off[r] + sg.a;
         double* out = p.out + r;
         __syncwarp();
         bool neighborhood = p.interp == RCP_INTERP_NEIGHBORHOOD;
@@ -713,8 +793,17 @@
     }
 }
 
+template <class V>
+__global__ void __launch_bounds__(32) interp_kernel(InterpArgs p) {
+    if constexpr (std::is_same<V, int32_t>::value) {
+        if (cov_narrow(p.bound)) return interp_run<V, uint16_t>(p);
+    }
+    interp_run<V, int32_t>(p);
+}
+
 struct BaseArgs {
     const int32_t* cov;
+    const unsigned long long* bound;
     const int64_t* off;
     const int32_t* len;
     const uint8_t* is_null;
@@ -725,11 +814,17 @@
     int64_t ld;
 };
 
-template <class V>
-__global__ void __launch_bounds__(256) base_matrix_kernel(BaseArgs p) {
-    __shared__ int tile[32][33];
-    __shared__ int64_t r_off[32];
-    __shared__ int r_a[32], r_b[32];
+struct BaseSmem {
+    int tile[32][33];
+    int64_t r_off[32];
+    int r_a[32], r_b[32];
+};
+template <class V, class S>
+__device__ __forceinline__ void base_matrix_run(const BaseArgs& p, BaseSmem& sm) {
+    auto& tile = sm.tile;
+    auto& r_off = sm.r_off;
+    auto& r_a = sm.r_a;
+    auto& r_b = sm.r_b;
     const int tx = threadIdx.x, ty = threadIdx.y;
     const int64_t r0 = (int64_t)blockIdx.y * 32, k0 = (int64_t)blockIdx.x * 32;
     if (ty == 0) {
@@ -751,7 +846,7 @@
         const int64_t k = k0 + tx;
         const int q = r_a[jj] + (int)k;
         int v = 0;
-        if (k < p.n_cols && q < r_b[jj]) v = __ldg(p.cov + r_off[jj] + q);
+        if (k < p.n_cols && q < r_b[jj]) v = __ldg(reinterpret_cast<const S*>(p.cov) + r_off[jj] + q);
         tile[jj][tx] = v;
     }
     __syncthreads();
@@ -761,14 +856,29 @@
     }
 }
 
+template <class V>
+__global__ void __launch_bounds__(256) base_matrix_kernel(BaseArgs p) {
+    __shared__ BaseSmem sm;
+    if constexpr (std::is_same<V, int32_t>::value) {
+        if (cov_narrow(p.bound)) return base_matrix_run<V, uint16_t>(p, sm);
+    }
+    base_matrix_run<V, int32_t>(p, sm);
+}
+
 constexpr int BW_ROWS = 32, BW_COLS = 256;
 
-template <class V>
-__global__ void __launch_bounds__(256) base_matrix_wide_kernel(BaseArgs p, int64_t col_tiles,
-                                                               int vec_store) {
-    __shared__ int tile[BW_ROWS][BW_COLS + 1];
-    __shared__ int64_t r_off[BW_ROWS];
-    __shared__ int r_a[BW_ROWS], r_b[BW_ROWS];
+struct BaseWideSmem {
+    int tile[BW_ROWS][BW_COLS + 1];
+    int64_t r_off[BW_ROWS];
+    int r_a[BW_ROWS], r_b[BW_ROWS];
+};
+template <class V, class S>
+__device__ __forceinline__ void base_matrix_wide_run(const BaseArgs& p, int64_t col_tiles, int vec_store,
+                                                     BaseWideSmem& sm) {
+    auto& tile = sm.tile;
+    auto& r_off = sm.r_off;
+    auto& r_a = sm.r_a;
+    auto& r_b = sm.r_b;
     const int tid = threadIdx.x, warp = tid >> 5, lane = tid & 31;
     const int64_t r0 = ((int64_t)blockIdx.x / col_tiles) * BW_ROWS;
     const int64_t k0 = ((int64_t)blockIdx.x % col_tiles) * BW_COLS;
@@ -789,14 +899,14 @@
     __syncthreads();
     for (int jj = warp; jj < BW_ROWS; jj += 8) {
         const int a = r_a[jj], b = r_b[jj];
-        const int32_t* src = p.cov + r_off[jj] + a + k0;
+        const S* src = reinterpret_cast<const S*>(p.cov) + r_off[jj] + a + k0;
         const int avail = (int)min((int64_t)(b - a) - k0, (int64_t)BW_COLS);
 #pragma unroll
         for (int h = 0; h < BW_COLS / 128; h++) {
             const int c = h * 128 + lane * 4;
             int4 v = make_int4(0, 0, 0, 0);
             if ((a & 3) == 0 && c + 3 < avail) {
-                v = __ldg(reinterpret_cast<const int4*>(src + c));
+                v = load4_g(src + c);
             } else {
                 if (c < avail) v.x = __ldg(src + c);
                 if (c + 1 < avail) v.y = __ldg(src + c + 1);
@@ -822,6 +932,15 @@
         if (r < p.R)
             for (int c = warp; c < ncol; c += 8) p.out[(k0 + c) * p.ld + r] = p.scale * word_double<V>(tile[lane][c]);
     }
+}
+
+template <class V>
+__global__ void __launch_bounds__(256) base_matrix_wide_kernel(BaseArgs p, int64_t col_tiles, int vec_store) {
+    __shared__ BaseWideSmem sm;
+    if constexpr (std::is_same<V, int32_t>::value) {
+        if (cov_narrow(p.bound)) return base_matrix_wide_run<V, uint16_t>(p, col_tiles, vec_store, sm);
+    }
+    base_matrix_wide_run<V, int32_t>(p, col_tiles, vec_store, sm);
 }
 
 template <class V>
@@ -848,6 +967,7 @@
     RCP_CUDA(cudaMemsetAsync(short_count, 0, sizeof(unsigned int), g_ctx.stream));
     BinArgs a;
     a.cov = cv.cov;
+    a.bound = cv.d_bound;
     a.off = cv.off;
     a.len = cv.len;
     a.is_null = cv.is_null;
@@ -881,7 +1001,7 @@
         if (where == RCP_WHERE_UPSTREAM) seg_max = std::min<int64_t>(seg_max, f1);
         else if (where == RCP_WHERE_DOWNSTREAM) seg_max = std::min<int64_t>(seg_max, f2);
         else if (where == RCP_WHERE_CENTER) seg_max = std::max<int64_t>(seg_max - f1 - f2, 0);
-        int buf_ints = (int)std::min<int64_t>(STAGE_INTS, ((seg_max + 10) & ~(int64_t)3));
+        int buf_ints = (int)std::min<int64_t>(STAGE_INTS, ((seg_max + 18) & ~(int64_t)3));
         int per_sm = 4;
         {
             const int64_t live = std::max<int64_t>(R - cv.n_null, 1);
@@ -898,7 +1018,8 @@
         RCP_TRY(dalloc(&long_count, 4));
         RCP_CUDA(cudaMemsetAsync(long_count, 0, 4 * sizeof(unsigned int), g_ctx.stream));
         bin_desc_kernel<<<(unsigned)((R + CTA - 1) / CTA), CTA, 0, g_ctx.stream>>>(
-            R, cv.off, cv.len, cv.is_null, where, f1, f2, n_bins, buf_ints, d_desc, long_list, long_count);
+            R, cv.off, cv.len, cv.is_null, where, f1, f2, n_bins, buf_ints, d_desc, long_list, long_count,
+            cv.d_bound);
         RCP_LAUNCHED();
         int nbuf = 2;
         if (const char* e = getenv("RCP_BIN_CTAS")) per_sm = std::max(1, atoi(e));
@@ -919,6 +1040,7 @@
     }
     InterpArgs ia;
     ia.cov = cv.cov;
+    ia.bound = cv.d_bound;
     ia.off = cv.off;
     ia.len = cv.len;
     ia.where = where;
@@ -962,6 +1084,7 @@
     if (R == 0 || n_cols == 0) return RCP_OK;
     BaseArgs a;
     a.cov = cv.cov;
+    a.bound = cv.d_bound;
     a.off = cv.off;
     a.len = cv.len;
     a.is_null = cv.is_null;
diff --git a/recoup_b200/csrc/rcp_internal.cuh b/recoup_b200/csrc/rcp_internal.cuh
--- a/recoup_b200/csrc/rcp_internal.cuh
+++ b/recoup_b200/csrc/rcp_internal.cuh
@@ -249,6 +249,7 @@
     bool stats_pending = false;
     double scale = 1.0;
     int value_type = RCP_VALUE_INT32;
+    const unsigned long long* d_bound = nullptr;
     int32_t* cov = nullptr;
     int64_t* off = nullptr;
     int32_t* len = nullptr;
@@ -256,6 +257,14 @@
 };
 void coverage_release(Coverage& c);
 int coverage_resolve_stats(Coverage& c);
+
+constexpr unsigned long long NARROW_MAX = 0xffffull;
+__device__ __forceinline__ bool cov_narrow(const unsigned long long* bound) {
+    return bound != nullptr && *bound <= NARROW_MAX;
+}
+__device__ __forceinline__ int32_t cov_at(const int32_t* cov, int64_t i, bool narrow) {
+    return narrow ? (int32_t)reinterpret_cast<const uint16_t*>(cov)[i] : cov[i];
+}
 int coverage_na_rule(const ReadsIdx& rd, Coverage& cv, int64_t R, const int32_t* d_chrom, const int8_t* d_strand,
                      const int64_t* d_end_pos);
 
```

Result: faster. 52.05 billion (median of 6 runs) (+6.5%).
